# calmiLovesAI/ComputerVision.pytorch

Hardware: AMD Instinct MI355X
Metric: images/sec 640x640 YOLOv8-n train step (higher is better)
Workload: dtype f16; 1 GPU; YOLOv8-n train step (fwd + v8 loss + bwd + Adam), batch 32/GPU, 640x640, nc=80, random init; global_batch=32, parallelism=dp1, launch=eager, exchange=none (1 rank), gpu_max_hw_queues=4

## Files before the change

__graft_entry__.py:

```python
import os
import subprocess
import sys

ROOT = os.path.dirname(os.path.abspath(__file__))
CSRC = os.path.join(ROOT, "computervision.pytorch_amd", "csrc")
LIBDIR = os.path.join(ROOT, "computervision.pytorch_amd", "lib")
LIB = os.path.join(LIBDIR, "libcvx_engine.so")
SOURCES = ["conv_igemm.hip", "conv_igemm_dma.hip", "conv_halo.hip", "conv_tile.hip", "conv_tile_k1.hip", "conv_tile_k2.hip", "conv_gemm.hip", "conv_stem7.hip", "conv_pw.hip", "conv_wgrad.hip", "conv_wgrad_gemm.hip", "conv_wgrad_halo.hip", "conv_wgrad_stream.hip", "conv_wgrad_k3.hip", "bn_act.hip", "stem.hip", "unit_ops.hip", "misc_ops.hip", "loss_v8.hip", "loss_seg.hip", "loss_centernet.hip", "loss_multibox.hip", "loss_yolov7.hip", "preprocess.hip", "augment.hip", "seg_pipeline.hip", "det_eval.hip", "coco_eval.hip", "nms.hip", "centernet_decode.hip", "render.hip", "tiles.hip", "seg_tiles.hip", "seg_tta.hip", "det_tta.hip", "track.hip", "optim.hip", "comm.hip", "engine.hip"]


def _stale(out, deps):
    if not os.path.exists(out):
        return True
    t = os.path.getmtime(out)
    return any(os.path.getmtime(d) > t for d in deps)


def build(force: bool = False) -> None:
    os.makedirs(LIBDIR, exist_ok=True)
    objdir = os.path.join(ROOT, "build", "obj")
    os.makedirs(objdir, exist_ok=True)
    headers = [os.path.join(CSRC, f) for f in os.listdir(CSRC) if f.endswith(".h")] + [os.path.join(ROOT, "include", "cvx_engine.h")]
    hipcc = os.environ.get("HIPCC", "/opt/rocm/bin/hipcc")
    objs, procs = [], []
    for src in SOURCES:
        s = os.path.join(CSRC, src)
        o = os.path.join(objdir, src.replace(".hip", ".o"))
        objs.append(o)
        if force or _stale(o, [s] + headers):
            cmd = [hipcc, "--offload-arch=gfx950", "-O3", "-std=c++17", "-fPIC", "-c", s, "-o", o]
            procs.append((src, subprocess.Popen(cmd, stdout=subprocess.PIPE, stderr=subprocess.STDOUT, text=True)))
    for src, p in procs:
        out, _ = p.communicate()
        if p.returncode != 0:
            raise RuntimeError(f"hipcc failed on {src}:\n{out}")
    if force or procs or _stale(LIB, objs):
        cmd = [hipcc, "--offload-arch=gfx950", "-shared", "-fPIC", "-o", LIB] + objs
        r = subprocess.run(cmd, stdout=subprocess.PIPE, stderr=subprocess.STDOUT, text=True)
        if r.returncode != 0:
            raise RuntimeError("link failed:\n" + r.stdout)
    if ROOT not in sys.path:
        sys.path.insert(0, ROOT)
    import computervision.pytorch_amd as pkg
    pkg._lib.load()


def smoke() -> None:
    if ROOT not in sys.path:
        sys.path.insert(0, ROOT)
    import numpy as np
    import torch
    from computervision.pytorch_amd.model import Yolo8
    from computervision.pytorch_amd.train import FlatAdam, FusedTrainStep, V8DetectionLoss
    from computervision.pytorch_amd import engine as E
    from configs import Yolo8DetConfig
    from oracle import nms_ref, synth
    from oracle import yolov8_ref as O

    assert torch.cuda.is_available(), "smoke() needs the MI355X"
    dev = torch.device("cuda:0")
    cfg = Yolo8DetConfig()
    torch.manual_seed(0)
    model = Yolo8("n", 80).to(dev).train()
    crit = V8DetectionLoss(cfg, model)
    step = FusedTrainStep(model, crit, FlatAdam(model, lr=1e-3))
    x, batch = synth.images(2, 128, 128, seed=1), synth.targets(2, seed=2)
    items = step(x.to(dev), batch).cpu()
    sd = O.init_state_dict("n", 80, seed=0)
    loss_ref, items_ref, _, _ = O.train_step(sd, x, batch, {})
    rel = float((items - items_ref).abs().max() / items_ref.abs().max())
    assert rel < 3e-2, f"loss items differ from the oracle: {items} vs {items_ref}"
    w = model.state_dict()["model.22.cv3.0.2.bias"].cpu()
    assert torch.allclose(w, sd["model.22.cv3.0.2.bias"], atol=2e-3), "post-Adam bias differs from the oracle"
    pred = synth.nms_pred(7, b=1)
    rows, index, counts = E.nms(torch.from_numpy(pred).to(dev), 0.25, 0.7, 300)
    ref_rows, ref_keep = nms_ref.non_max_suppression(pred, 0.25, 0.7, 300)[0]
    k = int(counts[0])
    assert k == len(ref_keep) and np.array_equal(index[0, :k].cpu().numpy().astype(np.int64), ref_keep), "NMS indices differ"
    print(f"smoke ok: loss items {items.tolist()} (oracle {items_ref.tolist()}), nms kept {k}")


if __name__ == "__main__":
    build(force="--force" in sys.argv)
    print("built", LIB)
    if "--smoke" in sys.argv:
        smoke()
```

computervision.pytorch_amd/_lib.py:

```python
from __future__ import annotations

import ctypes as C
import os

import numpy as np

_HERE = os.path.dirname(os.path.abspath(__file__))
LIB_PATH = os.environ.get("CVX_LIB") or os.path.join(_HERE, "lib", "libcvx_engine.so")
ABI_VERSION = 5
SEG_OPTS_KEY_OFFSET = 4096


class CvxError(RuntimeError):
    pass


class BufDesc(C.Structure):
    _fields_ = [("h", C.c_int32), ("w", C.c_int32), ("c", C.c_int32), ("kind", C.c_int32)]


class View(C.Structure):
    _fields_ = [("buf", C.c_int32), ("coff", C.c_int32), ("c", C.c_int32), ("pix_off", C.c_int32)]


class OpDesc(C.Structure):
    _fields_ = [
        ("type", C.c_int32),
        ("in_", View), ("out", View), ("res", View),
        ("ih", C.c_int32), ("iw", C.c_int32), ("oh", C.c_int32), ("ow", C.c_int32),
        ("k", C.c_int32), ("stride", C.c_int32), ("pad", C.c_int32), ("dil", C.c_int32),
        ("act", C.c_int32), ("needs_dgrad", C.c_int32), ("w_cin", C.c_int32),
        ("w_off", C.c_int64), ("gamma_off", C.c_int64), ("beta_off", C.c_int64), ("bias_off", C.c_int64),
        ("rmean_off", C.c_int64), ("rvar_off", C.c_int64),
        ("lane", C.c_int32), ("flags", C.c_int32),
    ]


class SegDims(C.Structure):
    _fields_ = [(k, C.c_int32) for k in ("ld", "batch", "nc", "ih", "iw", "oh", "ow")]


class SegCriterion(C.Structure):
    _fields_ = [("base", C.c_int32), ("focal_alpha", C.c_float), ("focal_gamma", C.c_float), ("class_weight", C.c_void_p),
                ("label_smoothing", C.c_float), ("ignore_index", C.c_int64), ("ohem_theta", C.c_float), ("ohem_min_kept", C.c_int64),
                ("region", C.c_int32), ("base_weight", C.c_double), ("weight", C.c_double), ("alpha", C.c_double), ("beta", C.c_double),
                ("gamma", C.c_double), ("smooth", C.c_double), ("per_image", C.c_int32), ("skip_absent", C.c_int32),
                ("region_class_weight", C.c_void_p)]


BUF_ACT_F16, BUF_PRED_F32 = 0, 1
OP_CONV, OP_MAXPOOL5, OP_UPSAMPLE2, OP_MAXPOOL2, OP_DWCONVT, OP_COPY, OP_MAXPOOL3S2, OP_AVGPOOL, OP_RESIZE, OP_MAXPOOL3S1, OP_L2NORM = 1, 2, 3, 4, 5, 6, 7, 8, 9, 10, 11
OP_DROPOUT = 12
ACT_BN_SILU, ACT_BIAS, ACT_BN_RELU, ACT_BN_LINEAR, ACT_BIAS_RELU, ACT_BIAS_LINEAR = 1, 2, 3, 4, 5, 6
OPF_RES_PRE_ACT = 1
OPF_CONV_BIAS = 2
OPF_RAW_F16 = 4

_P, _I32, _I64, _F, _U64 = C.c_void_p, C.c_int32, C.c_int64, C.c_float, C.c_uint64

EXPERIMENTAL_PROTOTYPES = {
    "cvx_chain_pair_unit": (_I32, [_P, _I32, _I32, _I32, _I32, _P, _P, _P, _P, _P, _P, _I32, _P, _I32, _I32, _I32, C.POINTER(_F), _P]),
    "cvx_chain_conv_unit": (_I32, [_P, _I32, _I32, _I32, _I32, _P, _I32, _I32, _I32, _I32, _P, _P, _I32, _P, _I32, _I32, _I32, C.POINTER(_F), _P]),
    "cvx_chain_detect_unit": (_I32, [_P, _I32, _I32, _I32, _I32, _I32, _I32, _I32, _P, _P, _P, _P, _P, _P, _P, _P, _P, _P, _P, _I32, _I32, _I32,
                                     _I32, _I32, C.POINTER(_F), _P]),
    "cvx_wgrad_time_unit": (_I32, [_P, _P, _I32, _I32, _I32, _I32, _I32, _I32, _I32, _I32, _I32, _I32, _P, _I64, C.POINTER(_F), C.POINTER(_I32), _P]),
}

PROTOTYPES = {
    "cvx_last_error": (C.c_char_p, []),
    "cvx_abi_version": (_I32, []),
    "cvx_engine_create": (_I32, [C.POINTER(_P), C.POINTER(BufDesc), _I32, C.POINTER(OpDesc), _I32, _I32, _I32, _I32, _P]),
    "cvx_engine_destroy": (_I32, [_P]),
    "cvx_engine_bind": (_I32, [_P, _P, _P, _I64, _P, _I64]),
    "cvx_engine_set_bn": (_I32, [_P, _F, _F]),
    "cvx_engine_forward": (_I32, [_P, _P, _I32, _I32, _P]),
    "cvx_engine_backward": (_I32, [_P, _P, _F]),
    "cvx_engine_backward_begin": (_I32, [_P, _P, _F]),
    "cvx_engine_backward_range": (_I32, [_P, _I32, _I32]),
    "cvx_engine_grads_ready": (_I32, [_P, _I32, _I32, _P]),
    "cvx_engine_backward_end": (_I32, [_P]),
    "cvx_engine_workspace_bytes": (_I64, [_P]),
    "cvx_engine_plan_generation": (_I64, [_P]),
    "cvx_engine_debug_copy": (_I32, [_P, _I32, _I32, _P, _I64]),
    "cvx_engine_profile": (_I32, [_P, _I32]),
    "cvx_engine_profile_read": (_I32, [_P, _I32, C.POINTER(C.c_double), C.POINTER(C.c_double), C.POINTER(C.c_double),
                                       C.POINTER(_I64)]),
    "cvx_debug_clock_buffer": (_I32, [_P]),
    "cvx_debug_conv_tile_plan": (_I32, [_I32, _I32, _I32, _I32, _I32, _P]),
    "cvx_debug_conv_dma_plan": (_I32, [_I64, _I32, _I32, _I32, _P]),
    "cvx_debug_conv_halo_plan": (_I32, [_I32, _I32, _I32, _I32, _I32, _P]),
    "cvx_debug_conv_pw_plan": (_I32, [_I64, _I32, _I32, _P]),
    "cvx_debug_conv_grid_div": (_I32, [_I32]),
    "cvx_engine_profile_dump": (_I32, [_P, C.c_char_p]),
    "cvx_pred_level_to_nchw": (_I32, [_P, _I32, _I32, _I32, _I32, _I32, _I32, _P, _P]),
    "cvx_nchw_grad_to_dpred": (_I32, [_P, _I32, _I32, _I32, _I32, _I32, _I32, _F, _P, _P]),
    "cvx_loss_v8_workspace_bytes": (_I64, [_I32, _I32, _I32, _I32]),
    "cvx_loss_v8": (_I32, [_P, _I32, _I32, _I32, _P, _I32, _I32, C.POINTER(_I32), C.POINTER(_F), _I32, _F, _F, _F, _F, _P, _P, _P,
                           _I64, _P]),
    "cvx_loss_v8_strided": (_I32, [_P, _I32, _I32, _I32, _I32, _P, _I32, _I32, C.POINTER(_I32), C.POINTER(_F), _I32, _F, _F, _F, _F, _P, _P, _P,
                                   _I64, _P]),
    "cvx_loss_v8_assignment": (_I32, [_P, _I32, _I32, _I32, _P, _P, _P]),
    "cvx_pack_targets": (_I32, [_P, _P, _P, _I32, _P, _P]),
    "cvx_decode_strided": (_I32, [_P, _I32, _I32, _I32, _I32, C.POINTER(_I32), C.POINTER(_F), _I32, _P, _P]),
    "cvx_adam_step": (_I32, [_P, _P, _P, _P, _I64, _F, _F, _F, _F, _I32, _P, _I32, _P]),
    "cvx_check_finite": (_I32, [_P, _I64, _P, _P]),
    "cvx_adam_step_dev": (_I32, [_P, _P, _P, _P, _I64, _F, _F, _F, _P, _P, _I32, _F, _P]),
    "cvx_ema_update": (_I32, [_P, _P, _I64, _F, _F, _P]),
    "cvx_adam_ema_step_dev": (_I32, [_P, _P, _P, _P, _I64, _F, _F, _F, _P, _P, _I32, _F, _P, _F, _F, _P]),
    "cvx_optim_step": (_I32, [_I32, _P, _P, _P, _P, _I64, _P, _P, _I32, _P, _F, _F, _F, _P, _I32, _F, _P, _P, _F, _F, _P]),
    "cvx_grad_norm_workspace": (_I64, [_I64]),
    "cvx_grad_norm": (_I32, [_P, _I64, _P, _P, _I32, _F, _F, _P, _P, _P, _I64, _P]),
    "cvx_engine_set_stream": (_I32, [_P, _P]),
    "cvx_engine_exchange_stream": (_P, [_P]),
    "cvx_decode": (_I32, [_P, _I32, _I32, _I32, C.POINTER(_I32), C.POINTER(_F), _I32, _P, _P]),
    "cvx_yolo7_decode": (_I32, [_P, _I32, _I32, _I32, _P, _P, _I32, _I32, _I32, _P, _P, _P]),
    "cvx_ssd_decode": (_I32, [_P, _P, _P, _I32, _I32, _I32, _F, _F, _P, _P, _P]),
    "cvx_ssd_decode_max": (_I32, [_P, _P, _P, _I32, _I32, _I32, _F, _F, _P, _P, _P, _P]),
    "cvx_pred_cols_to_nchw": (_I32, [_P, _I32, _I32, _I32, _I32, _I32, _I32, _I32, _P, _I64, _I64, _P]),
    "cvx_nms_workspace_bytes": (_I64, [_I32, _I32]),
    "cvx_nms": (_I32, [_P, _I32, _I32, _I32, _F, _F, _I32, _P, _P, _P, _P, _I64, _P]),
    "cvx_nms_variant": (_I32, [_P, _I32, _I32, _I32, _F, _F, _I32, _I32, _P, _P, _P, _P, _I64, _P]),
    "cvx_centernet_decode_workspace_bytes": (_I64, [_I32, _I32, _I32, _I32]),
    "cvx_centernet_decode": (_I32, [_P, _I32, _I32, _I32, _I32, _I32, _I32, _I32, _I32, _F, _F, _I32, _P, _P, _P, _P, _P, _P, _P, _I64, _P]),
    "cvx_conv2d_nhwc": (_I32, [_P, _I32, _I32, _I32, _I32, _P, _I32, _I32, _I32, _I32, _I32, _I32, _P, _P, _P, _P]),
    "cvx_conv2d_dgrad_nhwc": (_I32, [_P, _I32, _I32, _I32, _I32, _P, _I32, _I32, _I32, _I32, _I32, _P, _P]),
    "cvx_conv2d_wgrad_workspace_bytes": (_I64, [_I32, _I32, _I32, _I32, _I32, _I32]),
    "cvx_conv2d_wgrad_nhwc": (_I32, [_P, _P, _I32, _I32, _I32, _I32, _I32, _I32, _I32, _I32, _I32, _P, _P, _I64, _P]),
    "cvx_bn_silu_train_nhwc": (_I32, [_P, _I32, _I32, _I32, _P, _P, _F, _F, _P, _P, _P, _P, _P, _P, _P, _P]),
    "cvx_bn_silu_bwd_nhwc": (_I32, [_P, _P, _I32, _I32, _I32, _P, _P, _P, _F, _P, _P, _P, _P, _I32, _P]),
    "cvx_letterbox_geometry": (_I32, [_I32, _I32, _I32, _I32, _P, _P, _P, _P, _P]),
    "cvx_letterbox_u8_to_nchw": (_I32, [_P, _I32, _I32, _I32, _I32, _P, _I32, _I32, _P]),
    "cvx_letterbox_batch_u8_to_nchw": (_I32, [_P, _I32, _I32, _I32, _P, _I32, _I32, _P]),
    "cvx_det_to_image": (_I32, [_P, _P, _I32, _I32, _I32, _P, _P, _P, _P, _P]),
    "cvx_draw_detections": (_I32, [_P, _I32, _I32, _I32, _P, _P, _I32, _P, _I32, _I32, _I32, _P]),
    "cvx_seg_overlay": (_I32, [_P, _I32, _I32, _I32, _P, _I32, _I32, _I32, _I32, _I32, _I32, _P, _I32, _P]),
    "cvx_tiles_u8_to_nchw": (_I32, [_P, _I32, _I32, _P, _I32, _I32, _P]),
    "cvx_det_merge_workspace_bytes": (_I64, [_I32]),
    "cvx_det_merge_tiles": (_I32, [_P, _P, _I32, _I32, _P, _P, _I32, _I32, _F, _I32, _I32, _P, _P, _P, _P, _P, _I64, _P]),
    "cvx_track_state_bytes": (_I64, [_I32]),
    "cvx_track_update": (_I32, [_P, _P, _I32, _I32, _P, _I32, _P, _P, _P, _P, _P]),
    "cvx_draw_tracks": (_I32, [_P, _I32, _I32, _I32, _P, _P, _I32, _P, _P, _I32, _I32, _I32, _P]),
    "cvx_seg_stitch": (_I32, [_P, _I32, _I32, _I32, _I32, _I32, _I32, _I32, _P, _P, _I32, _P, _I32, _I32, _I32, _P, _P, _P, _P, _I32, _I32, _I32, _P]),
    "cvx_seg_tta_inputs": (_I32, [_P, _I32, _I32, _I32, _I32, _I32, _I32, _I32, _P, _P]),
    "cvx_seg_fuse": (_I32, [_P, _I32, _I32, _I32, _I32, _I32, _I32, _I32, _P, _P, _P, _P, _P]),
    "cvx_det_tta_inputs": (_I32, [_P, _I32, _I32, _I32, _P, _I32, _F, _P, _P]),
    "cvx_det_fuse_views": (_I32, [_P, _P, _I32, _P, _P, _I32, _I32, _F, _I32, _I32, _I32, _I32, _P, _P, _P, _P, _P, _P, _I64, _P]),
    "cvx_aug_images": (_I32, [_P, _P, _P, _I32, _P, _I32, _I32, _P]),
    "cvx_aug_boxes": (_I32, [_P, _P, _I32, _P, _I32, _I32, _I32, _P, _P, _P]),
    "cvx_aug_images_plain": (_I32, [_P, _P, _I32, _P, _I32, _I32, _P]),
    "cvx_aug_boxes_padded": (_I32, [_P, _P, _P, _I32, _P, _I32, _I32, _I32, _I32, _P, _P, _P, _P]),
    "cvx_aug_warp_mix": (_I32, [_P, _P, _I32, _P, _I32, _I32, _P]),
    "cvx_aug_boxes_warp": (_I32, [_P, _P, _I32, _P, _I32, _I32, _I32, _F, _F, _F, _I32, _P, _I32, _P, _P, _P]),
    "cvx_engine_set_seed": (_I32, [_P, _U64]),
    "cvx_engine_keep_shadows": (_I32, [_P]),
    "cvx_engine_set_fusion": (_I32, [_P, _I32]),
    "cvx_engine_fused_groups": (_I32, [_P]),
    "cvx_centernet_loss_workspace_bytes": (_I64, [_I32, _I32]),
    "cvx_centernet_loss": (_I32, [_P, _I32, _I32, _I32, _I32, _I32, _I32, _P, _P, _P, _P, _P, _I32, _F, _F, _F, _F, _P, _P, _P, _P, _P]),
    "cvx_yolo7_loss_workspace_bytes": (_I64, [_I32, _I32, _I32, _I32]),
    "cvx_yolo7_loss": (_I32, [_P, _I32, _I32, _I32, _P, _P, _P, _P, _I32, _F, _F, _F, _F, _F, _F, _P, _P, _P, _P, _P]),
    "cvx_debug_yolo7_loss_layout": (_I32, [_I32, _I32, _I32, _I32, _P]),
    "cvx_centernet_draw_targets": (_I32, [_P, _P, _I32, _I32, _I32, _I32, _I32, _P, _P, _P, _P, _P, _P]),
    "cvx_ssd_encode_targets": (_I32, [_P, _P, _I32, _I32, _P, _I32, _I32, _F, _F, _F, _P, _P, _P]),
    "cvx_multibox_loss_workspace_bytes": (_I64, [_I32, _I32]),
    "cvx_multibox_loss": (_I32, [_P, _P, _P, _I32, _I32, _I32, _F, _F, _F, _P, _P, _P, _P, _P]),
    "cvx_seg_criterion_workspace_bytes": (_I64, [C.POINTER(SegDims), C.POINTER(SegCriterion), _I32]),
    "cvx_seg_criterion_loss": (_I32, [_P, C.POINTER(SegDims), _P, C.POINTER(SegCriterion), _F, _P, _P, _P, _P, _P, _P, _P]),
    "cvx_seg_criterion_eval": (_I32, [_P, C.POINTER(SegDims), _P, C.POINTER(SegCriterion), _P, _P, _P, _P, _P]),
    "cvx_det_match": (_I32, [_P, _P, _I32, _I32, _I32, _P, _P, _P, _I32, _I32, C.c_double, _I32, _P, _P, _P, _I64, _P, _P, _P]),
    "cvx_det_ap": (_I32, [_P, _P, _P, _P, _I32, C.c_double, _I32, _P, _P, _P, _P]),
    "cvx_coco_match": (_I32, [_P, _P, _I32, _I32, _I32, _P, _I32, _I32, _P, _P, _I32, _I32, _P, _P, _P, _P, _P, _P, _I64, _P, _P, _P]),
    "cvx_coco_accumulate": (_I32, [_P, _P, _P, _P, _P, _I32, _P, _P, _P, _P]),
    "cvx_coco_summarize": (_I32, [_P, _P, _I32, _P, _P]),
    "cvx_seg_pipeline": (_I32, [_P, _I32, _P, _I32, _I32, C.POINTER(_F), C.POINTER(_F), _P, _P, _I32, _I32, _P]),
    "cvx_seg_pipeline_aug": (_I32, [_P, _I32, _P, _I32, _I32, _I32, _I32, C.POINTER(_F), C.POINTER(_F), C.POINTER(_F), _P, _P, _I32, _I32, _P]),
    "cvx_resize_bilinear_nchw_grad_to_rows": (_I32, [_P, _I32, _I32, _I32, _I32, _I32, _I32, _F, _P, _I32, _P]),
    "cvx_maxpool3_train_nhwc": (_I32, [_P, _I32, _I32, _I32, _I32, _I32, _P, _P, _P]),
    "cvx_maxpool3_bwd_nhwc": (_I32, [_P, _P, _I32, _I32, _I32, _I32, _I32, _P, _I32, _P]),
    "cvx_l2norm_bwd_nhwc": (_I32, [_P, _P, _P, _I32, _I32, _I32, _F, _P, _P, _I32, _P]),
    "cvx_nchw_cols_grad_to_pred": (_I32, [_P, _I64, _I64, _I32, _I32, _I32, _I32, _I32, _F, _P, _I32, _I32, _P]),
    "cvx_dwconvt_nhwc": (_I32, [_P, _I32, _I32, _I32, _I32, _I32, _P, _P, _P]),
    "cvx_dwconvt_bwd_nhwc": (_I32, [_P, _P, _I32, _I32, _I32, _I32, _I32, _P, _P, _I32, _P, _F, _P]),
    "cvx_maxpool2_bwd_nhwc": (_I32, [_P, _P, _I32, _I32, _I32, _I32, _I32, _P, _I32, _P]),
    "cvx_avgpool_global_bwd_nhwc": (_I32, [_P, _I32, _I32, _I32, _P, _I32, _P]),
    "cvx_resize_bilinear_bwd_nhwc": (_I32, [_P, _I32, _I32, _I32, _I32, _I32, _I32, _P, _I32, _P]),
    "cvx_dropout_nhwc": (_I32, [_P, _I32, _I32, _I32, _F, _U64, _P, _I32, _P]),
    "cvx_bn_act_train_nhwc": (_I32, [_P, _I32, _I32, _I32, _P, _P, _F, _F, _P, _P, _P, _I32, _I32, _P, _P, _P, _P, _P]),
    "cvx_bn_act_bwd_nhwc": (_I32, [_P, _P, _P, _I32, _I32, _I32, _P, _P, _P, _I32, _I32, _F, _P, _P, _P, _P, _I32, _P]),
    "cvx_maxpool5_nhwc": (_I32, [_P, _I32, _I32, _I32, _I32, _P, _P, _P]),
    "cvx_maxpool5_bwd_nhwc": (_I32, [_P, _P, _I32, _I32, _I32, _I32, _P, _I32, _P]),
    "cvx_resize_bilinear_rows_to_nchw": (_I32, [_P, _I32, _I32, _I32, _I32, _I32, _I32, _I32, _P, _P]),
    "cvx_maxpool_nhwc": (_I32, [_P, _I32, _I32, _I32, _I32, _I32, _I32, _I32, _P, _P]),
    "cvx_avgpool_global_nhwc": (_I32, [_P, _I32, _I32, _I32, _P, _P]),
    "cvx_resize_bilinear_nhwc": (_I32, [_P, _I32, _I32, _I32, _I32, _I32, _I32, _P, _P]),
    "cvx_l2norm_nhwc": (_I32, [_P, _P, _I32, _I32, _I32, _P, _P]),
    "cvx_upsample2_nhwc": (_I32, [_P, _I32, _I32, _I32, _I32, _P, _P]),
    "cvx_upsample2_bwd_nhwc": (_I32, [_P, _I32, _I32, _I32, _I32, _P, _I32, _P]),
    "cvx_stem_train_nchw": (_I32, [_P, _I32, _I32, _I32, _P, _I32, _P, _P, _F, _F, _P, _P, _P, _P, _P, _P, _P]),
    "cvx_stem_eval_nchw": (_I32, [_P, _I32, _I32, _I32, _P, _I32, _P, _P, _P, _P]),
    "cvx_stem_wgrad_nchw": (_I32, [_P, _I32, _I32, _I32, _P, _I32, _P, _P]),
    "cvx_comm_unique_id": (_I32, [_P]),
    "cvx_comm_create": (_I32, [C.POINTER(_P), _P, _I32, _I32, _I32]),
    "cvx_comm_destroy": (_I32, [_P]),
    "cvx_allreduce_f32": (_I32, [_P, _I64, _P, _P]),
    "cvx_allreduce_grads": (_I32, [_P, _P, _P]),
    "cvx_engine_backward_exchange": (_I32, [_P, _P, _F, _P, _P, _I32, _P]),
    "cvx_stem_backward_nchw": (_I32, [_P, _I32, _I32, _I32, _P, _P, _I32, _P, _P, _P, _F, _P, _P, _P, _P]),
    "cvx_stem_backward_recompute_nchw": (_I32, [_P, _I32, _I32, _I32, _P, _P, _I32, _P, _P, _P, _P, _F, _P, _P, _P, _P]),
# ... 49 lines not shown
```

computervision.pytorch_amd/csrc/conv_igemm.h:

```cpp
#pragma once
#include "cvx_common.h"
#include "bn_act.h"
#include "conv_plan.h"

enum {
  CVX_EPI_RAW_STATS = 0,
  CVX_EPI_AFFINE_SILU = 1,
  CVX_EPI_BIAS_F32 = 2,
  CVX_EPI_PLAIN = 3,
};

#define CVX_MAX_TAPS 64

struct ConvParams {
  const half_t* in;
  long long in_bstride;
  int in_ld;
  int IH, IW;
  int Cin;
  const half_t* wt;
  int wt_ld;
  int Cout;
  int B, OH2, OW2;
  int IS;
  int OS, oph, opw;
  int OWr;
  int ntaps;
  const ConvTap* taps;
  int epi;
  int accumulate;
  half_t* out16;
  float* out32;
  long long out_bstride;
  int out_ld;
  const half_t* res;
  long long res_bstride;
  int res_ld;
  const float* scale;
  int act_kind;
  int res_pre;
  const float* shift;
  const float* bias;
  long long* stats;
  int stats_replicas;
  const half_t* zeros;
  int dbg;
  unsigned long long* clk;
  int halo_taps_ok;
  int nphase;
  struct Phase {
    const ConvTap* taps;
    int ntaps, OH2, OW2, oph, opw;
  } phase[4];
  int pointwise;
  unsigned long long halo_pos, halo_wt;
  const half_t* wt_packed;
  int wt_packed_bn, wt_packed_kc;
  int std7x7;
  int std3x3;
  int gemm_variant;
  const half_t* tile_packed;
  int tile_packed_bn;
  int no_tile;
  int ps_cin;
  int raw16;
};

__device__ __forceinline__ void cvx_store_raw4(const ConvParams& p, long long off, const f4& v) {
  if (p.raw16) *reinterpret_cast<h4*>(p.out16 + off) = h4{(half_t)v[0], (half_t)v[1], (half_t)v[2], (half_t)v[3]};
  else *reinterpret_cast<f4*>(p.out32 + off) = v;
}

extern unsigned long long* g_cvx_clk;
extern int g_cvx_grid_div;
int cvx_conv_igemm_launch(const ConvParams& p, hipStream_t stream);
int cvx_conv_igemm_dma_launch(const ConvParams& p, hipStream_t stream);
bool cvx_conv_halo_supported(const ConvParams& p);
int cvx_conv_halo_launch(const ConvParams& p, hipStream_t stream);
bool cvx_conv_stem7_supported(const ConvParams& p);
int cvx_conv_stem7_launch(const ConvParams& p, hipStream_t stream);
struct GemmPackJob {
  const half_t* src;
  half_t* dst;
  const ConvTap* taps;
  int src_ld, rows, Cin, ntaps, BN, kc, nblocks, chunks;
  int blk0, nblk;
};
bool cvx_conv_gemm_plan(const ConvParams& p, GemmPackJob* job, size_t* bytes);
int cvx_conv_gemm_pack_jobs(const GemmPackJob* d_jobs, int njobs, int nblocks, hipStream_t stream);
bool cvx_conv_gemm_shape_ok(const ConvParams& p);
bool cvx_conv_gemm_supported(const ConvParams& p);
int cvx_conv_gemm_launch(const ConvParams& p, hipStream_t stream);
void cvx_conv_gemm_release();
struct TilePackPlan {
  int BN, NB, SPT;
  size_t bytes;
  double cost_us;
};
bool cvx_conv_tile_shape_ok(const ConvParams& p);
bool cvx_conv_tile_supported(const ConvParams& p);
bool cvx_conv_tile_plan(const ConvParams& p, TilePackPlan* out);
int cvx_conv_tile_fill_job(const ConvParams& p, const TilePackPlan& tp, half_t* dst, int blk0, void* job_out);
size_t cvx_conv_tile_job_bytes();
int cvx_conv_tile_pack_jobs(const void* d_jobs, int njobs, int nblocks, hipStream_t stream);
int cvx_conv_tile_launch(const ConvParams& p, hipStream_t stream);
void cvx_conv_tile_release();
bool cvx_conv_pw_supported(const ConvParams& p);
int cvx_conv_pw_launch(const ConvParams& p, hipStream_t stream);

struct WgradParams {
  const half_t* x;
  long long x_bstride;
  int x_ld;
  int IH, IW, Cin;
  const half_t* dy;
  long long dy_bstride;
  int dy_ld;
  int Cout;
  int B, OH, OW;
  int stride;
  int ntaps;
  const ConvTap* taps;
  float* slabs;
  int nsplit;
  int cin_pad16;
  int std3x3;
};
int cvx_conv_wgrad_launch(const WgradParams& p, hipStream_t stream);
void cvx_conv_wgrad_tile(int cout, int jtot, int* co_b, int* j_b);
bool cvx_conv_wgrad_gemm_supported(const WgradParams& p);
void cvx_conv_wgrad_gemm_tile(int cout, int jtot, int* co_b, int* j_b);
int cvx_conv_wgrad_gemm_launch(const WgradParams& p, hipStream_t stream);
bool cvx_conv_wgrad_halo_supported(const WgradParams& p);
void cvx_conv_wgrad_halo_grid(int cout, int cin, int* gx, int* gy);
int cvx_conv_wgrad_halo_tiles(int B, int OH, int OW);
int cvx_conv_wgrad_halo_launch(const WgradParams& p, hipStream_t stream);
bool cvx_conv_wgrad_stream_supported(const WgradParams& p);
int cvx_conv_wgrad_stream_nsplit(const WgradParams& p);
int cvx_conv_wgrad_stream_launch(const WgradParams& p, hipStream_t stream);
bool cvx_conv_wgrad_k3_supported(const WgradParams& p);
int cvx_conv_wgrad_k3_nsplit(const WgradParams& p, bool wide = false);
int cvx_conv_wgrad_k3_launch(const WgradParams& p, hipStream_t stream);
```

computervision.pytorch_amd/csrc/conv_igemm.hip:

```cpp
#include "conv_igemm.h"

unsigned long long* g_cvx_clk = nullptr;
int g_cvx_grid_div = 1;

extern "C" int cvx_debug_conv_grid_div(int32_t div) {
  CVX_CHECK(div >= 1, "the grid divisor is at least 1");
  const int prev = g_cvx_grid_div;
  g_cvx_grid_div = div;
  return prev;
}

int cvx_conv_igemm_launch(const ConvParams& p_in, hipStream_t stream) {
  ConvParams p = p_in;
  p.clk = g_cvx_clk;
  CVX_CHECK(p.Cin % 8 == 0 && p.in_ld % 8 == 0 && p.wt_ld % 8 == 0, "conv: channel counts must be multiples of 8");
  CVX_CHECK(p.Cout % 4 == 0 && p.out_ld % 4 == 0, "conv: Cout/out_ld must be multiples of 4");
  CVX_CHECK(p.ntaps >= 1 && p.ntaps <= CVX_MAX_TAPS, "conv: bad tap count");
  CVX_CHECK(((uintptr_t)p.in % 16) == 0 && ((uintptr_t)p.wt % 16) == 0, "conv: operands must be 16-byte aligned");
  CVX_CHECK(p.zeros && ((uintptr_t)p.zeros % 16) == 0, "conv: needs a 16-byte aligned zero page (padding source of the LDS DMA)");
  CVX_CHECK((long long)p.B * p.OH2 * p.OW2 > 0, "conv: empty output");
  if (p.ps_cin > 0) {
    CVX_CHECK(p.epi == CVX_EPI_PLAIN && p.nphase <= 1 && p.OS == 2 && p.oph == 0 && p.opw == 0 && p.ps_cin % 8 == 0 && p.Cout == 4 * p.ps_cin &&
                  cvx_conv_gemm_shape_ok(p),
              "conv: pixel-shuffle data gradient needs the GEMM-shaped kernel (plain epilogue, 4 phases of ps_cin channels, output stride 2)");
    return cvx_conv_gemm_launch(p, stream);
  }
  if (p.nphase > 1) return cvx_conv_igemm_dma_launch(p, stream);
  if (cvx_conv_stem7_supported(p)) return cvx_conv_stem7_launch(p, stream);
  if (cvx_conv_tile_supported(p)) return cvx_conv_tile_launch(p, stream);
  if (cvx_conv_gemm_supported(p)) return cvx_conv_gemm_launch(p, stream);
  if (cvx_conv_pw_supported(p)) return cvx_conv_pw_launch(p, stream);
  if (cvx_conv_halo_supported(p)) return cvx_conv_halo_launch(p, stream);
  return cvx_conv_igemm_dma_launch(p, stream);
}
```

computervision.pytorch_amd/csrc/conv_tile.h:

```cpp
#pragma once
#include "conv_tile_common.h"

namespace cvx_tile_k {
using namespace cvx_tile;

typedef __attribute__((address_space(3))) void* lds_ptr_t;

constexpr int kTileWaves = 8;

struct TileArgs {
  int TR, tiles_per_img, ntiles, NB;
  int P, pow2, logP, sh, swmask, phmask;
  int SPT, NSTEPS, KSC, NCH, R;
  int CP, PW;
  int PP, PPW;
  int units, Wp;
  unsigned magic_wp, magic_w, magic_p;
  int wring_off, CB, stat_off;
  unsigned in_records;
  const half_t* wpk;
  int dbg;
};

template <int OFF>
__device__ __forceinline__ h8 lds_frag(unsigned a) {
  h8 v;
  asm volatile("ds_read_b128 %0, %1 offset:%2" : "=v"(v) : "v"(a), "n"(OFF));
  return v;
}
template <int NTW>
__device__ __forceinline__ void frag_load_w(h8 (&w)[NTW], unsigned a) {
  if constexpr (NTW >= 1) w[0] = lds_frag<0>(a);
  if constexpr (NTW >= 2) w[1] = lds_frag<1024>(a);
  if constexpr (NTW >= 3) w[2] = lds_frag<2048>(a);
  if constexpr (NTW >= 4) w[3] = lds_frag<3072>(a);
  if constexpr (NTW >= 5) w[4] = lds_frag<4096>(a);
  if constexpr (NTW >= 6) w[5] = lds_frag<5120>(a);
  if constexpr (NTW >= 7) w[6] = lds_frag<6144>(a);
  if constexpr (NTW >= 8) w[7] = lds_frag<7168>(a);
  if constexpr (NTW >= 9) w[8] = lds_frag<8192>(a);
}

__device__ __forceinline__ void wait_vmcnt_dyn(int n) {
#define CVX_WV(N) else if (n == N) wait_vmcnt<N>();
  if (n <= 0 || n > 20) wait_vmcnt<0>();
  CVX_WV(1) CVX_WV(2) CVX_WV(3) CVX_WV(4) CVX_WV(5) CVX_WV(6) CVX_WV(7) CVX_WV(8) CVX_WV(9) CVX_WV(10)
  CVX_WV(11) CVX_WV(12) CVX_WV(13) CVX_WV(14) CVX_WV(15) CVX_WV(16) CVX_WV(17) CVX_WV(18) CVX_WV(19) CVX_WV(20)
#undef CVX_WV
}

}

int cvx_conv_tile_launch_k1(int MT, int NTW, const ConvParams& p, const cvx_tile_k::TileArgs& a, int lds, hipStream_t st);
int cvx_conv_tile_launch_k2(int MT, int NTW, const ConvParams& p, const cvx_tile_k::TileArgs& a, int lds, hipStream_t st);
```

computervision.pytorch_amd/csrc/conv_tile.hip:

```cpp
#include <algorithm>
#include <cstring>
#include <map>
#include <mutex>
#include <vector>

#include "conv_tile.h"

namespace {
using namespace cvx_tile_k;

struct TilePackJob {
  const half_t* src;
  half_t* dst;
  unsigned long long wt_pack;
  int src_ld, rows, Cin, BN, NB, SPT;
  int blk0, nblk;
};
constexpr int TPACK_UNITS = 256 * 8;
__device__ __forceinline__ void tile_pack_units(const TilePackJob& a, long long u0, long long u1) {
  const int nsteps = 9 * a.SPT;
  for (long long u = u0 + threadIdx.x; u < u1; u += blockDim.x) {
    const int sp = (int)(u & 3);
    const long long r0 = u >> 2;
    const int r = (int)(r0 % a.BN);
    const long long r1 = r0 / a.BN;
    const int n = (int)(r1 % nsteps);
    const int nb = (int)(r1 / nsteps);
    const int g = sp ^ ((r >> 1) & 3);
    const int tap = n / a.SPT, s = n - tap * a.SPT;
    const int k = s * 32 + g * 8;
    const int row = nb * a.BN + r;
    h8 v = {0, 0, 0, 0, 0, 0, 0, 0};
    if (row < a.rows && k < a.Cin) v = *reinterpret_cast<const h8*>(a.src + (long long)row * a.src_ld + (int)((a.wt_pack >> (4 * tap)) & 15) * a.Cin + k);
    *reinterpret_cast<h8*>(a.dst + u * 8) = v;
  }
}
__global__ __launch_bounds__(256) void tile_pack_kernel(const TilePackJob a) {
  const long long total = (long long)a.NB * 9 * a.SPT * a.BN * 4;
  const long long u0 = (long long)blockIdx.x * TPACK_UNITS;
  if (u0 < total) tile_pack_units(a, u0, u0 + TPACK_UNITS < total ? u0 + TPACK_UNITS : total);
}
__global__ __launch_bounds__(256) void tile_pack_jobs_kernel(const TilePackJob* jobs, int njobs) {
  int lo = 0, hi = njobs - 1;
  while (lo < hi) {
    const int mid = (lo + hi + 1) >> 1;
    if (jobs[mid].blk0 <= (int)blockIdx.x)
      lo = mid;
    else
      hi = mid - 1;
  }
  const TilePackJob a = jobs[lo];
  const long long total = (long long)a.NB * 9 * a.SPT * a.BN * 4;
  const long long u0 = (long long)((int)blockIdx.x - a.blk0) * TPACK_UNITS;
  if (u0 < total) tile_pack_units(a, u0, u0 + TPACK_UNITS < total ? u0 + TPACK_UNITS : total);
}

constexpr int kMaxMT = 4;
const int kNtwMenu[] = {1, 2, 3, 4, 5, 6, 9};

unsigned magic_of(int d) { return (unsigned)((0x100000000ULL + (unsigned long long)d - 1) / (unsigned long long)d); }

struct Plan {
  int MT, NTW, TR, NB, KSC, NCH, R, SPT, lds, ntiles, tpi, PP, units, CB, wring_off, stat_off;
  double cost;
};

bool plan_tile(const ConvParams& p, Plan* best) {
  const int H = p.IH, W = p.IW, Cin = p.Cin;
  const int P = Cin / 8, SPT = (Cin + 31) / 32, NSTEPS = 9 * SPT;
  const int ctiles = (p.Cout + 15) / 16;
  static const int force_tr = cvx_tune_int("CVX_TILE_TR", 0), force_ntw = cvx_tune_int("CVX_TILE_NTW", 0);
  bool found = false;
  for (int NTW : kNtwMenu) {
    if (force_ntw && NTW != force_ntw) continue;
    if (NTW > ctiles && NTW != kNtwMenu[0]) {
      bool smaller_fits = false;
      for (int q : kNtwMenu) smaller_fits |= q >= ctiles && q < NTW;
      if (smaller_fits) continue;
    }
    const int NB = (ctiles + NTW - 1) / NTW;
    if ((NB - 1) * NTW >= ctiles) continue;
    for (int TR = 1; TR <= H; ++TR) {
      if (force_tr && TR != force_tr) continue;
      const int G = (TR * W + 15) / 16;
      const int MT = (G + kTileWaves - 1) / kTileWaves;
      if (MT > kMaxMT) break;
      if (MT > 4 || MT * NTW * 4 + 3 * (MT + NTW) * 4 > 216) continue;
      const int tpi = (H + TR - 1) / TR;
      const int units = (TR + 2) * (W + 2) * P;
      const int PP = (units + 63) / 64;
      const int patch_bytes = PP * 1024;
      const int stat_bytes = kTileWaves * 16 * NTW * 2 * 4;
      const int budget = 160 * 1024 - patch_bytes - stat_bytes;
      int KSC = 0, R = 0;
      if (NSTEPS * NTW * 1024 <= budget && (NSTEPS * NTW + kTileWaves - 1) / kTileWaves + (PP + kTileWaves - 1) / kTileWaves <= 60) {
        KSC = NSTEPS;
        R = 2;
      } else {
        for (int k = SPT; k >= 1 && !KSC; --k) {
          if (SPT % k) continue;
          const int r = budget / (k * NTW * 1024);
          if (r >= 3 && (k * NTW + kTileWaves - 1) / kTileWaves <= 20) {
            KSC = k;
            R = r > 4 ? 4 : r;
          }
        }
      }
      if (!KSC) continue;
      const int CB = KSC * NTW * 1024;
      const int nslots = R > NSTEPS / KSC ? NSTEPS / KSC : R;
      const int stage_bytes = kTileWaves * MT * 16 * (16 * NTW * 4 + 16);
      const int lds = std::max(patch_bytes + nslots * CB + stat_bytes, stage_bytes);
      if (lds > 160 * 1024) continue;
      const long long wgs = (long long)tpi * p.B * NB;
      const double rounds = (double)((wgs + 255) / 256);
      const double mfma_cyc = (double)NSTEPS * MT * NTW * 16.0 * (kTileWaves / 4);
      const double lds_cyc = (double)NSTEPS * kTileWaves * (MT + NTW) * 6.0;
      const double valu_cyc = (double)NSTEPS * (MT * 3 + NTW * 4 + 8) * 4.0;
      const double loop_us = std::max(std::max(mfma_cyc * 1.15, lds_cyc), valu_cyc + mfma_cyc * 0.5) / 1900.0;
      const double wbytes = (double)NSTEPS * NTW * 1024.0;
      const double load_us = (patch_bytes + CB) / 60e3 + std::max(0.0, (wbytes - CB) / 60e3 - loop_us);
      const double epi_us = 0.6 + MT * NTW * 0.02;
      const double t = rounds * (1.2 + load_us + loop_us + epi_us) + 1.0;
      if (!found || t < best->cost) {
        found = true;
        *best = Plan{MT, NTW, TR, NB, KSC, NSTEPS / KSC, R, SPT, lds, tpi * p.B, tpi, PP, units, CB, patch_bytes, patch_bytes + nslots * CB, t};
      }
    }
  }
  return found;
}

struct PackSlot {
  half_t* buf = nullptr;
  size_t bytes = 0;
};
std::mutex g_pack_mu;
std::map<std::pair<const void*, unsigned long long>, PackSlot> g_pack;

}

bool cvx_conv_tile_shape_ok(const ConvParams& p) {
  if (!p.zeros || !p.halo_taps_ok || p.ntaps != 9) return false;
  if (p.IS != 1 || p.OS != 1 || p.oph != 0 || p.opw != 0) return false;
  if (p.OH2 != p.IH || p.OW2 != p.IW || p.OWr != p.IW) return false;
  if (p.Cin % 8 != 0 || p.Cin < 32 || p.Cin > 512 || p.in_ld % 8 != 0) return false;
  if (p.Cout % 8 != 0 || p.out_ld % 8 != 0 || (p.res && p.res_ld % 8 != 0)) return false;
  if (p.IW > 4000 || p.IH > 4000 || p.IW < 2) return false;
  const long long extent = ((long long)(p.B - 1) * p.in_bstride + ((long long)p.IH * p.IW - 1) * p.in_ld + p.Cin) * 2;
  if (extent >= (1LL << 32) - 65536) return false;
  Plan pl;
  return plan_tile(p, &pl);
}

bool cvx_conv_tile_supported(const ConvParams& p) {
  static const bool off = cvx_tune_set("CVX_NO_TILE");
  if (off || p.no_tile) return false;
  static const int max_w = cvx_tune_int("CVX_TILE_MAXW", 40), max_c = cvx_tune_int("CVX_TILE_MAXC", 144);
  if (p.IW > max_w || p.IH > max_w || p.Cin > max_c) return false;
  return cvx_conv_tile_shape_ok(p);
}

bool cvx_conv_tile_plan(const ConvParams& p, TilePackPlan* out) {
  if (!cvx_conv_tile_shape_ok(p)) return false;
  Plan pl;
  if (!plan_tile(p, &pl)) return false;
  out->BN = 16 * pl.NTW;
  out->NB = pl.NB;
  out->SPT = pl.SPT;
  out->bytes = (size_t)pl.NB * 9 * pl.SPT * pl.NTW * 1024;
  out->cost_us = pl.cost;
  return true;
}

int cvx_conv_tile_pack_jobs(const void* d_jobs, int njobs, int nblocks, hipStream_t stream) {
  if (njobs <= 0 || nblocks <= 0) return 0;
  hipLaunchKernelGGL(tile_pack_jobs_kernel, dim3(nblocks), dim3(256), 0, stream, (const TilePackJob*)d_jobs, njobs);
  CVX_HIP(hipGetLastError());
  return 0;
}

int cvx_conv_tile_fill_job(const ConvParams& p, const TilePackPlan& tp, half_t* dst, int blk0, void* job_out) {
  TilePackJob j;
  memset(&j, 0, sizeof(j));
  j.src = p.wt;
  j.dst = dst;
  j.wt_pack = p.halo_wt;
  j.src_ld = p.wt_ld;
  j.rows = p.Cout;
  j.Cin = p.Cin;
  j.BN = tp.BN;
  j.NB = tp.NB;
  j.SPT = tp.SPT;
  j.blk0 = blk0;
  const long long units = (long long)tp.NB * 9 * tp.SPT * tp.BN * 4;
  j.nblk = (int)((units + TPACK_UNITS - 1) / TPACK_UNITS);
  memcpy(job_out, &j, sizeof(j));
  return j.nblk;
}
size_t cvx_conv_tile_job_bytes() { return sizeof(TilePackJob); }

int cvx_conv_tile_launch(const ConvParams& p, hipStream_t stream) {
  Plan pl;
  CVX_CHECK(plan_tile(p, &pl), "conv_tile: no tiling for this shape");
  const half_t* packed = (p.tile_packed && p.tile_packed_bn == 16 * pl.NTW) ? p.tile_packed : nullptr;
  if (!packed) {
    TilePackPlan tp{16 * pl.NTW, pl.NB, pl.SPT, (size_t)pl.NB * 9 * pl.SPT * pl.NTW * 1024, 0.0};
    half_t* buf = nullptr;
    {
      std::lock_guard<std::mutex> lk(g_pack_mu);
      PackSlot& ps = g_pack[{p.wt, p.halo_wt ^ ((unsigned long long)tp.BN << 52)}];
      if (ps.bytes < tp.bytes) {
        hipStreamCaptureStatus cs = hipStreamCaptureStatusNone;
        (void)hipStreamIsCapturing(stream, &cs);
        CVX_CHECK(cs == hipStreamCaptureStatusNone, "conv_tile: the packed-weight buffer cannot be allocated while the stream is capturing");
        if (ps.buf) CVX_HIP(hipFree(ps.buf));
        CVX_HIP(hipMalloc((void**)&ps.buf, tp.bytes));
        ps.bytes = tp.bytes;
      }
      buf = ps.buf;
    }
    TilePackJob j;
    const int nblk = cvx_conv_tile_fill_job(p, tp, buf, 0, &j);
    hipLaunchKernelGGL(tile_pack_kernel, dim3(nblk), dim3(256), 0, stream, j);
    packed = buf;
  }
  TileArgs a;
  memset(&a, 0, sizeof(a));
  a.TR = pl.TR;
  a.tiles_per_img = pl.tpi;
  a.ntiles = pl.ntiles;
  a.NB = pl.NB;
  a.P = p.Cin / 8;
  a.pow2 = (a.P & (a.P - 1)) == 0 ? 1 : 0;
  a.logP = 0;
  while ((1 << a.logP) < a.P) ++a.logP;
  a.sh = a.P == 4 ? 2 : (a.P == 8 ? 1 : 0);
  a.swmask = a.pow2 ? (a.P >= 16 ? 15 : a.P - 1) : 0;
  a.phmask = a.pow2 ? a.P - 1 : -1;
  a.SPT = pl.SPT;
  a.NSTEPS = 9 * pl.SPT;
  a.KSC = pl.KSC;
  a.NCH = pl.NCH;
  a.R = pl.R;
  a.CP = pl.KSC * pl.NTW;
  a.PW = (a.CP + kTileWaves - 1) / kTileWaves;
  a.PP = pl.PP;
  a.PPW = (pl.PP + kTileWaves - 1) / kTileWaves;
  a.units = pl.units;
  a.Wp = p.IW + 2;
  a.magic_wp = magic_of(a.Wp);
  a.magic_w = magic_of(p.IW);
  a.magic_p = magic_of(a.P);
  a.wring_off = pl.wring_off;
  a.CB = pl.CB;
  a.stat_off = pl.stat_off;
  a.in_records = (unsigned)(((long long)(p.B - 1) * p.in_bstride + ((long long)p.IH * p.IW - 1) * p.in_ld + p.Cin) * 2);
  a.wpk = packed;
  static const int dbg = cvx_tune_int("CVX_TILE_DBG", 0);
  a.dbg = dbg;
  int rc;
  if (pl.MT <= 2)
    rc = cvx_conv_tile_launch_k1(pl.MT, pl.NTW, p, a, pl.lds, stream);
  else
    rc = cvx_conv_tile_launch_k2(pl.MT, pl.NTW, p, a, pl.lds, stream);
  CVX_TRY(rc);
  CVX_HIP(hipGetLastError());
  return 0;
}

extern "C" int cvx_debug_conv_tile_plan(int32_t batch, int32_t h, int32_t w, int32_t cin, int32_t cout, int32_t* out8) {
  CVX_CHECK(out8 && batch > 0 && h > 0 && w > 0, "bad arguments");
  ConvParams p;
  memset(&p, 0, sizeof(p));
  static half_t dummy_zero[8];
  p.zeros = dummy_zero;
  p.halo_taps_ok = 1;
  p.ntaps = 9;
  p.IS = p.OS = 1;
  p.B = batch;
  p.IH = p.OH2 = h;
  p.IW = p.OW2 = p.OWr = w;
  p.Cin = p.in_ld = cin;
  p.in_bstride = (long long)h * w * cin;
  p.Cout = cout;
  if (!cvx_conv_tile_shape_ok(p)) return -1;
  Plan pl;
  if (!plan_tile(p, &pl)) return -1;
  out8[0] = pl.TR;
  out8[1] = pl.MT;
  out8[2] = pl.NTW;
  out8[3] = pl.NB;
  out8[4] = pl.ntiles * pl.NB;
  out8[5] = pl.KSC;
  out8[6] = pl.lds;
  out8[7] = (int)(pl.cost * 100.0);
  return 0;
}

void cvx_conv_tile_release() {
  std::lock_guard<std::mutex> lk(g_pack_mu);
  for (auto& kv : g_pack)
    if (kv.second.buf) (void)hipFree(kv.second.buf);
  g_pack.clear();
}
```

computervision.pytorch_amd/csrc/conv_tile_kernel.inc.h:

```cpp
#include "conv_tile.h"

namespace {
using namespace cvx_tile_k;

template <int MT, int NTW>
__global__ __launch_bounds__(64 * kTileWaves) void conv_tile_kernel(const ConvParams p, const TileArgs a) {
#if defined(__HIP_DEVICE_COMPILE__)
  constexpr int BN = 16 * NTW;
  extern __shared__ __attribute__((aligned(16))) unsigned char smem[];
  const int tid = threadIdx.x;
  const int wave = __builtin_amdgcn_readfirstlane(tid >> 6), lane = tid & 63;
  const int fr = lane & 15, fq = lane >> 4;
  const int xcd = blockIdx.x & 7, seq = blockIdx.x >> 3;
  const int nblk = seq % a.NB;
  const int tile = (seq / a.NB) * 8 + xcd;
  if (tile >= a.ntiles) return;
  clk_mark(p, 0);
  const int b = tile / a.tiles_per_img;
  const int y0 = (tile - b * a.tiles_per_img) * a.TR;
  const int H = p.IH, W = p.IW, Wp = a.Wp, P = a.P;

  const __amdgpu_buffer_rsrc_t rsrc_in = __builtin_amdgcn_make_buffer_rsrc(const_cast<half_t*>(p.in), (short)0, (int)a.in_records, 0x00020000);
  const half_t* wblk = a.wpk + (long long)nblk * a.NSTEPS * (BN * 32);
  const __amdgpu_buffer_rsrc_t rsrc_w = __builtin_amdgcn_make_buffer_rsrc(const_cast<half_t*>(wblk), (short)0, a.NSTEPS * BN * 64, 0x00020000);

  {
    const unsigned img_off = (unsigned)((long long)b * p.in_bstride * 2);
    for (int k = 0; k < a.PPW; ++k) {
      int piece = k * kTileWaves + wave;
      piece = piece < a.PP ? piece : a.PP - 1;
      const unsigned u = (unsigned)(piece * 64 + lane);
      const unsigned q = __umulhi(u, a.magic_p);
      const unsigned phys = u - q * (unsigned)P;
      const unsigned pr = __umulhi(q, a.magic_wp);
      const unsigned pc = q - pr * (unsigned)Wp;
      const unsigned c = phys ^ ((pc >> a.sh) & (unsigned)a.swmask);
      const int y = y0 - 1 + (int)pr, x = (int)pc - 1;
      const bool ok = u < (unsigned)a.units && (unsigned)y < (unsigned)H && (unsigned)x < (unsigned)W;
      const unsigned vo = ok ? img_off + (unsigned)(((y * W + x) * p.in_ld + (int)c * 8) * 2) : 0xffffffffu;
      __builtin_amdgcn_raw_ptr_buffer_load_lds(rsrc_in, (lds_ptr_t)(smem + piece * 1024), 16, vo, 0, 0, 0);
    }
  }
  const unsigned vb = (unsigned)(lane * 16);
  auto issue_chunk = [&](int c, int slot) __attribute__((always_inline)) {
    unsigned char* sb = smem + a.wring_off + slot * a.CB;
    const int base = c * a.CB;
    for (int k = 0; k < a.PW; ++k) {
      int piece = k * kTileWaves + wave;
      piece = piece < a.CP ? piece : a.CP - 1;
      __builtin_amdgcn_raw_ptr_buffer_load_lds(rsrc_w, (lds_ptr_t)(sb + piece * 1024), 16, vb, base + piece * 1024, 0, 0);
    }
  };
  const int npre = a.NCH < a.R - 1 ? a.NCH : a.R - 1;
  for (int c = 0; c < npre; ++c) issue_chunk(c, c);
  clk_mark(p, 1);

  const int rows_here = H - y0 < a.TR ? H - y0 : a.TR;
  const int npix = rows_here * W;
  unsigned S0[MT], S1[MT], S2[MT];
  bool pvalid[MT];
  const unsigned rowpitch = (unsigned)(Wp * P * 16);
#pragma unroll
  for (int i = 0; i < MT; ++i) {
    const int m = (wave * MT + i) * 16 + fr;
    pvalid[i] = m < npix;
    const unsigned mm = pvalid[i] ? (unsigned)m : 0u;
    const unsigned pr = __umulhi(mm, a.magic_w);
    const unsigned pc = mm - pr * (unsigned)W;
    auto s_of = [&](unsigned col) -> unsigned {
      const unsigned sw = (col >> a.sh) & (unsigned)a.swmask;
      const unsigned ph = ((unsigned)fq ^ sw) & (unsigned)a.phmask;
      return (pr + 1u) * rowpitch + ((col * (unsigned)P + ph) << 4);
    };
    S0[i] = s_of(pc);
    S1[i] = s_of(pc + 1u);
    S2[i] = s_of(pc + 2u);
  }

  f4 acc[MT][NTW];
#pragma unroll
  for (int i = 0; i < MT; ++i)
#pragma unroll
    for (int j = 0; j < NTW; ++j) acc[i][j] = f4{0.f, 0.f, 0.f, 0.f};

  const unsigned long long pos_pack = p.halo_pos;
  const unsigned xk_mask = a.pow2 ? 0xffffffffu : 0u, np2_mask = ~xk_mask;
  auto step_xk = [&](int s) -> unsigned { return (unsigned)(s << 6) & xk_mask; };
  auto step_ak = [&](int dh, int s) -> unsigned {
    int c = 4 * s + fq;
    c = c < P ? c : P - 1;
    return (unsigned)(dh * (int)rowpitch) + ((unsigned)((c - fq) << 4) & np2_mask);
  };

#pragma unroll
  for (int i = 0; i < MT; ++i) asm volatile("" ::"v"(S0[i]), "v"(S1[i]), "v"(S2[i]));
#pragma unroll
  for (int i = 0; i < MT; ++i)
#pragma unroll
    for (int j = 0; j < NTW; ++j) asm volatile("" ::"v"(acc[i][j]));
  if (npre <= 1 || (a.dbg & 1)) wait_vmcnt<0>();
  else wait_vmcnt_dyn((npre - 1) * a.PW);
  workgroup_barrier();
  clk_mark(p, 2);
#ifdef CVX_TUNING
  if ((a.dbg & 8) && p.clk) {
    wait_vmcnt<0>();
    workgroup_barrier();
    if (blockIdx.x == 0)
      for (int o = tid * 4; o < a.stat_off; o += 1024) reinterpret_cast<unsigned*>(p.clk)[o >> 2] = *reinterpret_cast<const unsigned*>(smem + o);
    return;
  }
#endif

  h8 xs[3][MT], ws[3][NTW];
  unsigned SC[MT];
  const unsigned lds0 = (unsigned)(unsigned long long)(const __attribute__((address_space(3))) void*)smem;
  const int NSTEPS = a.NSTEPS, SPT = a.SPT, KSC = a.KSC, NCH = a.NCH, CB = a.CB, R = a.R, PWc = a.PW;
  const unsigned wfrag0 = lds0 + (unsigned)a.wring_off + (unsigned)(lds_row_off(fr, fq) * 2);
  int c_tap = 0, c_st = 0, c_inc = 0, c_chunk = 0, c_slot = 0, c_n = 0;
  int dh_cur;
  unsigned xk_c, ak_c, w_c;
  auto set_tap = [&](int t) __attribute__((always_inline)) -> int {
    const int code = (int)(pos_pack >> (4 * t)) & 15;
    const int dwi = code & 3;
    const unsigned m0 = dwi == 0 ? 0xffffffffu : 0u, m1 = dwi == 1 ? 0xffffffffu : 0u, m2 = dwi == 2 ? 0xffffffffu : 0u;
#pragma unroll
    for (int i = 0; i < MT; ++i) SC[i] = (S0[i] & m0) | (S1[i] & m1) | (S2[i] & m2);
    return (code >> 2) - 1;
  };
  dh_cur = set_tap(0);
  xk_c = step_xk(0);
  ak_c = step_ak(dh_cur, 0) + lds0;
  w_c = wfrag0;
  auto advance = [&]() __attribute__((always_inline)) {
    if (c_n + 1 < NSTEPS) {
      ++c_n;
      if (++c_st == SPT) {
        c_st = 0;
        ++c_tap;
        dh_cur = set_tap(c_tap);
      }
      xk_c = step_xk(c_st);
      ak_c = step_ak(dh_cur, c_st) + lds0;
      if (++c_inc == KSC) {
        c_inc = 0;
        const int issued = NCH < c_chunk + R - 1 ? NCH : c_chunk + R - 1;
        if (issued - c_chunk - 2 <= 0) wait_vmcnt<0>();
        else wait_vmcnt_dyn((issued - c_chunk - 2) * PWc);
        workgroup_barrier();
        if (c_chunk + R - 1 < NCH) issue_chunk(c_chunk + R - 1, c_slot == 0 ? R - 1 : c_slot - 1);
        ++c_chunk;
        c_slot = c_slot == R - 1 ? 0 : c_slot + 1;
      }
      w_c = wfrag0 + (unsigned)(c_slot * CB + c_inc * (NTW * 1024));
    }
  };
  frag_load_w<NTW>(ws[0], w_c);
#pragma unroll
  for (int i = 0; i < MT; ++i) xs[0][i] = lds_frag<0>((SC[i] ^ xk_c) + ak_c);
  advance();
  frag_load_w<NTW>(ws[1], w_c);
#pragma unroll
  for (int i = 0; i < MT; ++i) xs[1][i] = lds_frag<0>((SC[i] ^ xk_c) + ak_c);
  asm volatile("s_waitcnt lgkmcnt(0)" ::: "memory");
  constexpr int LW = (MT + NTW) > 15 ? 15 : (MT + NTW);
#if defined(CVX_TILE_ABL)
#define CVX_TILE_DBG_BIT(b) (((CVX_TILE_ABL) & (b)) != 0)
#else
#define CVX_TILE_DBG_BIT(b) false
#endif
#define CVX_TILE_BODY(K, LAST)                                                                                          \
  {                                                                                                                     \
    advance();                                                                                                          \
    if (!CVX_TILE_DBG_BIT(128)) frag_load_w<NTW>(ws[((K) + 2) % 3], w_c);                                                \
    _Pragma("unroll") for (int i = 0; i < MT; ++i) {                                                                    \
      __builtin_amdgcn_sched_barrier(0);                                                                                \
      _Pragma("unroll") for (int j = 0; j < NTW; ++j)                                                                   \
          acc[i][j] = __builtin_amdgcn_mfma_f32_16x16x32_f16(ws[K][j], xs[K][i], acc[i][j], 0, 0, 0);                   \
      if (!CVX_TILE_DBG_BIT(64)) xs[((K) + 2) % 3][i] = lds_frag<0>((SC[i] ^ xk_c) + ak_c);                              \
    }                                                                                                                   \
    __builtin_amdgcn_sched_barrier(0);                                                                                  \
    if (LAST) {                                                                                                         \
      asm volatile("s_waitcnt lgkmcnt(0)" ::: "memory");                                                                \
    } else {                                                                                                            \
      asm volatile("s_waitcnt lgkmcnt(%0)" ::"n"(LW) : "memory");                                                       \
    }                                                                                                                   \
    __builtin_amdgcn_sched_barrier(0);                                                                                  \
  }
  clk_mark(p, 7);
  for (int n = 0; n < NSTEPS; n += 3) {
    CVX_TILE_BODY(0, false)
    CVX_TILE_BODY(1, false)
    CVX_TILE_BODY(2, true)
  }
#undef CVX_TILE_BODY
  clk_mark(p, 3);

  constexpr int RS = BN * 4 + 16;
  constexpr int CPR = BN / 8;
  constexpr int RPI = 64 / CPR;
  constexpr int ROWS = MT * 16;
  const int epi = p.epi;
  f4 st1[NTW], st2[NTW];
  if (epi == CVX_EPI_RAW_STATS) {
#pragma unroll
    for (int j = 0; j < NTW; ++j) {
      st1[j] = st2[j] = f4{0.f, 0.f, 0.f, 0.f};
#pragma unroll
      for (int i = 0; i < MT; ++i)
        if (pvalid[i]) {
#pragma unroll
          for (int r = 0; r < 4; ++r) {
            st1[j][r] += acc[i][j][r];
            st2[j][r] += acc[i][j][r] * acc[i][j][r];
          }
        }
    }
  }
  if (epi == CVX_EPI_RAW_STATS) {
#pragma unroll
    for (int i = 0; i < MT; ++i) {
      if (!pvalid[i]) continue;
      const unsigned m = (unsigned)((wave * MT + i) * 16 + fr);
      const unsigned pr = __umulhi(m, a.magic_w);
      const unsigned pc = m - pr * (unsigned)W;
      const long long dst = (long long)b * p.out_bstride + ((long long)(y0 + (int)pr) * W + (int)pc) * p.out_ld + nblk * BN + fq * 4;
#pragma unroll
      for (int j = 0; j < NTW; ++j)
        if (nblk * BN + j * 16 + fq * 4 < p.Cout) cvx_store_raw4(p, dst + j * 16, acc[i][j]);
    }
  } else {
  __syncthreads();
    unsigned char* wreg = smem + wave * (ROWS * RS);
#pragma unroll
    for (int i = 0; i < MT; ++i)
#pragma unroll
      for (int j = 0; j < NTW; ++j) *reinterpret_cast<f4*>(wreg + (i * 16 + fr) * RS + (j * 16 + fq * 4) * 4) = acc[i][j];
    {
      const int q = lane % CPR, r0 = lane / CPR;
      const int n = nblk * BN + q * 8;
      const bool lane_on = r0 < RPI && n < p.Cout;
      const int act_kind = p.act_kind, res_pre = p.res_pre, accumulate = p.accumulate;
      const half_t* res = p.res;
      float c0[8], c1[8];
#pragma unroll
      for (int k = 0; k < 8; ++k) {
        c0[k] = 1.f;
        c1[k] = 0.f;
      }
      if (lane_on && epi == CVX_EPI_AFFINE_SILU) {
#pragma unroll
        for (int k = 0; k < 8; ++k) {
          c0[k] = p.scale[n + k];
          c1[k] = p.shift[n + k];
        }
      }
      if (lane_on && epi == CVX_EPI_BIAS_F32) {
#pragma unroll
        for (int k = 0; k < 8; ++k) c1[k] = p.bias[n + k];
      }
      const int m_wave = wave * ROWS;
      for (int r = r0; r < ROWS; r += RPI) {
        const int m = m_wave + r;
        if (!lane_on || m >= npix) continue;
        const unsigned pr = __umulhi((unsigned)m, a.magic_w);
        const unsigned pc = (unsigned)m - pr * (unsigned)W;
        const long long pix = (long long)(y0 + (int)pr) * W + (int)pc;
        const f4 lo = *reinterpret_cast<const f4*>(wreg + r * RS + q * 32);
        const f4 hi = *reinterpret_cast<const f4*>(wreg + r * RS + q * 32 + 16);
        float v[8] = {lo[0], lo[1], lo[2], lo[3], hi[0], hi[1], hi[2], hi[3]};
        if (epi == CVX_EPI_BIAS_F32) {
          float* dst = p.out32 + (long long)b * p.out_bstride + pix * p.out_ld + n;
          *reinterpret_cast<f4*>(dst) = f4{v[0] + c1[0], v[1] + c1[1], v[2] + c1[2], v[3] + c1[3]};
          *reinterpret_cast<f4*>(dst + 4) = f4{v[4] + c1[4], v[5] + c1[5], v[6] + c1[6], v[7] + c1[7]};
          continue;
        }
        half_t* dst = p.out16 + (long long)b * p.out_bstride + pix * p.out_ld + n;
        if (epi == CVX_EPI_AFFINE_SILU) {
          float rv[8] = {0.f, 0.f, 0.f, 0.f, 0.f, 0.f, 0.f, 0.f};
          if (res) {
            const h8 rr = *reinterpret_cast<const h8*>(res + (long long)b * p.res_bstride + pix * p.res_ld + n);
#pragma unroll
            for (int k = 0; k < 8; ++k) rv[k] = (float)rr[k];
          }
#pragma unroll
          for (int k = 0; k < 8; ++k) {
            float t = v[k] * c0[k] + c1[k];
            if (res_pre) t += rv[k];
            if (act_kind == 0) t = cvx_silu(t);
            else if (act_kind == 1) t = fmaxf(t, 0.f);
            if (!res_pre) t += rv[k];
            v[k] = t;
          }
        } else if (accumulate) {
          const h8 old = *reinterpret_cast<const h8*>(dst);
#pragma unroll
          for (int k = 0; k < 8; ++k) v[k] += (float)old[k];
        }
        *reinterpret_cast<h8*>(dst) = h8{(half_t)v[0], (half_t)v[1], (half_t)v[2], (half_t)v[3], (half_t)v[4], (half_t)v[5], (half_t)v[6], (half_t)v[7]};
      }
    }
  }
  if (epi == CVX_EPI_RAW_STATS) {
    __syncthreads();
    float* sStat = reinterpret_cast<float*>(smem);
#pragma unroll
    for (int j = 0; j < NTW; ++j)
#pragma unroll
      for (int r = 0; r < 4; ++r) {
        const float s1 = cvx_wave_sum16(st1[j][r]), s2 = cvx_wave_sum16(st2[j][r]);
        if (fr == 0) {
          sStat[(wave * BN + j * 16 + fq * 4 + r) * 2 + 0] = s1;
          sStat[(wave * BN + j * 16 + fq * 4 + r) * 2 + 1] = s2;
        }
      }
    __syncthreads();
    for (int t = tid; t < BN * 2; t += 64 * kTileWaves) {
      const int ch = t >> 1, which = t & 1, nn = nblk * BN + ch;
      if (nn < p.Cout) {
        float v = 0.f;
#pragma unroll
        for (int w = 0; w < kTileWaves; ++w) v += sStat[(w * BN + ch) * 2 + which];
        cvx_fix_atomic_add(p.stats, ((long long)(blockIdx.x % p.stats_replicas) * p.Cout + nn) * 2 + which, v);
      }
    }
  }
  clk_mark(p, 4);
#endif
}


template <int MT, int NTW>
int launch_tile(const ConvParams& p, const TileArgs& a, int lds, hipStream_t stream) {
  static unsigned long long optin_mask = 0;
  CVX_TRY(cvx_lds_optin((const void*)conv_tile_kernel<MT, NTW>, 160 * 1024, &optin_mask));
  const int blocks = ((a.ntiles + 7) / 8) * 8 * a.NB;
  hipLaunchKernelGGL((conv_tile_kernel<MT, NTW>), dim3(blocks), dim3(64 * kTileWaves), lds, stream, p, a);
  return 0;
}
template <int MT>
int launch_tile_n(int NTW, const ConvParams& p, const TileArgs& a, int lds, hipStream_t st) {
  switch (NTW) {
    case 1: return launch_tile<MT, 1>(p, a, lds, st);
    case 2: return launch_tile<MT, 2>(p, a, lds, st);
    case 3: return launch_tile<MT, 3>(p, a, lds, st);
    case 4: return launch_tile<MT, 4>(p, a, lds, st);
    case 5: return launch_tile<MT, 5>(p, a, lds, st);
    case 6: return launch_tile<MT, 6>(p, a, lds, st);
    default: return launch_tile<MT, 9>(p, a, lds, st);
  }
}
}

int CVX_TILE_LAUNCH_FN(int MT, int NTW, const ConvParams& p, const cvx_tile_k::TileArgs& a, int lds, hipStream_t st) {
  if (MT == CVX_TILE_MT_A) return launch_tile_n<CVX_TILE_MT_A>(NTW, p, a, lds, st);
  return launch_tile_n<CVX_TILE_MT_B>(NTW, p, a, lds, st);
}
```

computervision.pytorch_amd/csrc/engine.hip:

```cpp
#include <algorithm>
#include <atomic>
#include <cstdlib>
#include <cstdio>
#include <cstring>
#include <vector>

#include "../../include/cvx_engine.h"
#ifdef CVX_WITH_CHAIN
#include "conv_chain.h"
#endif
#include "bn_act.h"
#include "conv_igemm.h"
#include <map>
#include <mutex>

#include "misc_ops.h"
#include "stem.h"

static unsigned cvx_event_flags() {
  static const bool sysfence = cvx_tune_set("CVX_EVENT_SYSFENCE");
  return hipEventDisableTiming | (sysfence ? 0u : hipEventDisableSystemFence);
}

static thread_local std::string g_last_error;
void cvx_set_error(const std::string& msg) { g_last_error = msg; }
extern "C" const char* cvx_last_error(void) { return g_last_error.c_str(); }
extern "C" int cvx_abi_version(void) { return CVX_ABI_VERSION; }

namespace {

struct PhaseRt {
  const ConvTap* taps = nullptr;
  TapTraits tr;
  int ntaps = 0, oph = 0, opw = 0, OH2 = 0, OW2 = 0;
};
PhaseRt make_phase(const DgradPhase& d, const ConvTap* dev_taps) {
  PhaseRt r;
  r.taps = dev_taps;
  r.tr = cvx_tap_traits(d.taps);
  r.ntaps = (int)d.taps.size();
  r.oph = d.oph;
  r.opw = d.opw;
  r.OH2 = d.OH2;
  r.OW2 = d.OW2;
  return r;
}

struct DgClass {
  PhaseRt ph;
  const half_t* gemm_pk = nullptr;
  int gemm_bn = 0, gemm_kc = 0;
  const half_t* tile_pk = nullptr;
  int tile_bn = 0;
};

struct ConvRt {
  ConvTap* taps_fwd = nullptr;
  TapTraits tr;
  int ntaps = 0;
  DgClass dg[16];
  int ndg = 0;
  long long sh_fwd = 0, sh_dg = -1;
  int cin_g = 0;
  int cin_pad16 = 0;
  int in_accum = 0, res_accum = 0;
  long long sh_ps = -1;
  PsPackDesc ps_desc;
  ConvTap* ps_taps = nullptr;
  bool ps_on = false;
  const half_t* ps_pk = nullptr;
  int ps_bn = 0, ps_kc = 0;
  int slab_blk0 = 0, slab_blk1 = 0;
  bool raw16 = false;
  bool stem = false;
  half_t* ybuf = nullptr;
  half_t* dybuf = nullptr;
  float *mean = nullptr, *invstd = nullptr, *scale = nullptr, *shift = nullptr;
  long long *stat_fwd = nullptr, *stat_bwd = nullptr;
  hipEvent_t ev_dy = nullptr;
  long long slab_off = 0;
  int nsplit = 1;
  const half_t* gemm_fwd = nullptr;
  int gemm_fwd_bn = 0, gemm_fwd_kc = 0;
  const half_t* tile_fwd = nullptr;
  int tile_fwd_bn = 0;
};

struct PoolRt {
  uint8_t* idx = nullptr;
  int in_accum = 0;
};

struct Buf {
  cvx_buf_desc d;
  half_t* act = nullptr;
  half_t* grad = nullptr;
};

}

struct cvx_engine {
  int device = 0;
  hipStream_t stream = nullptr;
  std::vector<Buf> bufs;
  std::vector<cvx_op_desc> ops;
  std::vector<ConvRt> conv;
  std::vector<PoolRt> pool;
  int image_buf = -1, pred_buf = -1;
  float* params = nullptr;
  float* grads = nullptr;
  float* stats = nullptr;
  int64_t n_params = 0, n_stats = 0;
  float bn_eps = 1e-3f, bn_momentum = 0.03f;
  std::vector<void*> static_allocs;
  half_t* shadow = nullptr;
  long long shadow_elems = 0;
  half_t* zero_page = nullptr;
  PackDesc* d_pack = nullptr;
  BlockRef* d_pack_blocks = nullptr;
  int n_pack_blocks = 0;
  int planned_batch = 0;
  bool planned_train = false;
  std::vector<void*> batch_allocs;
  int64_t batch_bytes = 0, static_bytes = 0;
  long long* stat_region = nullptr;
  long long stat_half = 0;
  hipStream_t side = nullptr;
  hipStream_t red = nullptr;
  hipStream_t lane = nullptr;
  hipEvent_t ev_lane_fork = nullptr, ev_lane_join = nullptr, ev_pack = nullptr;
  bool use_lanes = false;
  hipEvent_t ev_head[3] = {nullptr, nullptr, nullptr};
  int head_producer[3] = {-1, -1, -1};
  int head_join_op[3] = {-1, -1, -1};
  bool head_overlap = false;
  float* ytmp_lane = nullptr;
  hipEvent_t ev_red = nullptr;
  hipEvent_t ev_fork = nullptr, ev_join = nullptr;
  bool image_nhwc = false;
  float* ytmp = nullptr;
  const float* last_images = nullptr;
  bool inference_only = false;
  int64_t plan_generation = 0;
  float* slabs = nullptr;
  SlabDesc* d_slab = nullptr;
  BlockRef* d_slab_blocks = nullptr;
  int n_slab_blocks = 0;
  ColsumDesc* d_colsum = nullptr;
  ColsumBlock* d_colsum_blocks = nullptr;
  int n_colsum = 0, n_colsum_blocks = 0, colsum_max_c = 0;
  BnFoldDesc* d_fold = nullptr;
  int n_fold = 0;
  int slab_tail_blocks = 0;
  int slab_tail_op = -1;
  hipEvent_t ev_mid = nullptr;
  hipEvent_t ev_seg[8] = {nullptr, nullptr, nullptr, nullptr, nullptr, nullptr, nullptr, nullptr};
  int ev_seg_next = 0;
  unsigned long long seed = 0, train_pass = 0;
  bool has_bias_act = false;
  bool fwd_train_done = false;
  bool keep_shadows_once = false;
  int shadows_gen = -1;
  bool shadows_train = false;
  bool bwd_slabs_clean = false;
  int last_batch = 0;
  float* last_pred = nullptr;
  bool profile = false;
  std::vector<hipEvent_t> ev_pool;
// ... 20 lines not shown
  half_t* gemm_arena = nullptr;
  GemmPackJob* d_gemm_jobs = nullptr;
  int n_gemm_jobs = 0, n_gemm_fwd_jobs = 0, gemm_blocks = 0, gemm_fwd_blocks = 0;
  half_t* tile_arena = nullptr;
  void* d_tile_jobs = nullptr;
  int n_tile_jobs = 0, n_tile_fwd_jobs = 0, tile_blocks = 0, tile_fwd_blocks = 0;
  struct cvx_bw_state* bw = nullptr;
  std::vector<ProfRec> prof_recs;
};

void cvx_engine_free_bw(cvx_engine* e);

namespace {

int dev_alloc(cvx_engine* e, std::vector<void*>& pool, int64_t& counter, void** out, long long bytes) {
  if (bytes <= 0) bytes = 16;
  bytes = (bytes + 255) & ~255LL;
  CVX_HIP(hipMalloc(out, (size_t)bytes));
  pool.push_back(*out);
  counter += bytes;
  return 0;
}
template <typename T>
int upload(cvx_engine* e, std::vector<void*>& pool, int64_t& counter, T** out, const std::vector<T>& host) {
  void* p = nullptr;
  CVX_TRY(dev_alloc(e, pool, counter, &p, (long long)(host.size() * sizeof(T))));
  if (!host.empty()) CVX_HIP(hipMemcpy(p, host.data(), host.size() * sizeof(T), hipMemcpyHostToDevice));
  *out = (T*)p;
  return 0;
}
void free_pool(std::vector<void*>& pool) {
  for (void* p : pool) (void)hipFree(p);
  pool.clear();
}

inline int round_up(int x, int m) { return (x + m - 1) / m * m; }

enum { PROF_CONV_FWD = 0, PROF_CONV_DGRAD = 1, PROF_CONV_WGRAD = 2, PROF_BN_FWD = 3, PROF_BN_BWD = 4, PROF_MISC = 5, PROF_SLAB_REDUCE = 6 };

struct ProfScope {
  cvx_engine* e;
  hipStream_t st;
  ProfScope(cvx_engine* eng, int cls, double flops, double bytes, hipStream_t stream = nullptr)
      : e(eng->profile ? eng : nullptr), st(stream ? stream : eng->stream) {
    if (!e) return;
    while (e->ev_pool.size() < e->ev_used + 2) {
      hipEvent_t ev;
      if (hipEventCreate(&ev) != hipSuccess) {
        e = nullptr;
        return;
      }
      e->ev_pool.push_back(ev);
    }
    e->prof_recs.push_back({cls, flops, bytes, e->cur_op});
    slot = e->ev_used;
    e->ev_used += 2;
    (void)hipEventRecord(e->ev_pool[slot], st);
  }
  size_t slot = 0;
  ~ProfScope() {
    if (!e) return;
    (void)hipEventRecord(e->ev_pool[slot + 1], st);
  }
};

double conv_flops(const cvx_op_desc& o, int B) { return 2.0 * B * o.oh * o.ow * o.out.c * (double)(o.k * o.k * o.w_cin); }
double conv_bytes(const cvx_op_desc& o, int B) {
  return 2.0 * B * ((double)o.ih * o.iw * o.w_cin + (double)o.oh * o.ow * o.out.c) + 2.0 * o.out.c * o.k * o.k * o.w_cin;
}

ViewDesc make_view(const cvx_engine* e, const cvx_view& v, bool grad) {
  ViewDesc r{nullptr, 0, 0};
  if (v.buf < 0) return r;
  const Buf& b = e->bufs[v.buf];
  half_t* base = grad ? b.grad : b.act;
  r.ld = b.d.c;
  r.bstride = (long long)b.d.h * b.d.w * b.d.c;
  r.p = base + (long long)v.pix_off * b.d.c + v.coff;
  return r;
}

int act_kind(const cvx_op_desc& o) { return o.act == CVX_ACT_BN_SILU ? 0 : ((o.act == CVX_ACT_BN_LINEAR || o.act == CVX_ACT_BIAS_LINEAR) ? 2 : 1); }
float dropout_p(const cvx_op_desc& o) { return (float)o.k / 65536.f; }
unsigned long long dropout_seed(const cvx_engine* e, int op) {
  return e->seed * 0x9E3779B97F4A7C15ULL + (unsigned long long)e->train_pass * 1000003ULL + (unsigned long long)op;
}

struct ConvGeom {
  int B, ih, iw, cin, oh, ow, cout, stride, ntaps;
};
ConvGeom geom_of(const cvx_op_desc& o, int B) { return ConvGeom{B, o.ih, o.iw, o.in.c, o.oh, o.ow, o.out.c, o.stride, o.k * o.k}; }

void fill_conv_fwd(const ConvGeom& g, ViewDesc in, const half_t* wt, const ConvTap* taps, const TapTraits& tr, const half_t* zeros, ConvParams* cp) {
  memset(cp, 0, sizeof(*cp));
  cp->in = in.p;
  cp->in_bstride = in.bstride;
  cp->in_ld = in.ld;
  cp->IH = g.ih;
  cp->IW = g.iw;
  cp->Cin = g.cin;
  cp->wt = wt;
  cp->wt_ld = g.ntaps * g.cin;
  cp->Cout = g.cout;
  cp->B = g.B;
  cp->OH2 = g.oh;
  cp->OW2 = g.ow;
  cp->IS = g.stride;
  cp->OS = 1;
  cp->OWr = g.ow;
  cp->ntaps = g.ntaps;
  cp->taps = taps;
  cp->zeros = zeros;
  cp->halo_taps_ok = tr.halo_ok ? 1 : 0;
  cp->pointwise = tr.pointwise;
  cp->halo_pos = tr.halo_pos;
  cp->halo_wt = tr.halo_wt;
  cp->std7x7 = tr.std7x7;
  cp->std3x3 = tr.std3x3;
}

void fill_conv_dgrad(const ConvGeom& g, const PhaseRt& ph, ViewDesc dy, ViewDesc gin, const half_t* wt_t, const half_t* zeros, int accumulate, ConvParams* cp) {
  memset(cp, 0, sizeof(*cp));
  cp->in = dy.p;
  cp->in_bstride = dy.bstride;
  cp->in_ld = dy.ld;
  cp->IH = g.oh;
  cp->IW = g.ow;
  cp->Cin = g.cout;
  cp->wt = wt_t;
  cp->wt_ld = g.ntaps * g.cout;
  cp->Cout = g.cin;
  cp->B = g.B;
  cp->OH2 = ph.OH2;
  cp->OW2 = ph.OW2;
  cp->IS = 1;
  cp->OS = g.stride;
  cp->oph = ph.oph;
  cp->opw = ph.opw;
  cp->OWr = g.iw;
  cp->ntaps = ph.ntaps;
  cp->taps = ph.taps;
  cp->zeros = zeros;
  cp->halo_taps_ok = ph.tr.halo_ok ? 1 : 0;
  cp->pointwise = ph.tr.pointwise;
  cp->halo_pos = ph.tr.halo_pos;
  cp->halo_wt = ph.tr.halo_wt;
  cp->epi = CVX_EPI_PLAIN;
  cp->accumulate = accumulate;
  cp->out16 = gin.p;
  cp->out_ld = gin.ld;
  cp->out_bstride = gin.bstride;
}
bool phases_mergeable(const DgClass* dg, int n) {
  if (n < 2 || n > 4) return false;
  for (int q = 0; q < n; ++q)
    if (dg[q].ph.OH2 <= 0 || dg[q].ph.OW2 <= 0 || dg[q].ph.ntaps <= 0) return false;
  return true;
}
void set_merged_phases(const DgClass* dg, int n, ConvParams* cp) {
  cp->nphase = n;
  for (int z = 0; z < n; ++z) cp->phase[z] = ConvParams::Phase{dg[z].ph.taps, dg[z].ph.ntaps, dg[z].ph.OH2, dg[z].ph.OW2, dg[z].ph.oph, dg[z].ph.opw};
  cp->halo_taps_ok = 0;
  cp->pointwise = 0;
}

void fill_conv_ps(const ConvGeom& g, ViewDesc dy, ViewDesc gin, const half_t* ps_wt, const ConvTap* window_taps, const half_t* zeros, int accumulate, ConvParams* cp) {
  memset(cp, 0, sizeof(*cp));
  cp->in = dy.p;
  cp->in_bstride = dy.bstride;
  cp->in_ld = dy.ld;
  cp->IH = g.oh;
  cp->IW = g.ow;
  cp->Cin = g.cout;
  cp->wt = ps_wt;
  cp->wt_ld = 4 * g.cout;
  cp->Cout = 4 * g.cin;
  cp->B = g.B;
  cp->OH2 = g.oh;
  cp->OW2 = g.ow;
  cp->IS = 1;
  cp->OS = 2;
  cp->OWr = g.iw;
  cp->ntaps = 4;
  cp->taps = window_taps;
  cp->zeros = zeros;
  cp->epi = CVX_EPI_PLAIN;
  cp->ps_cin = g.cin;
  cp->accumulate = accumulate;
  cp->out16 = gin.p;
  cp->out_ld = gin.ld;
  cp->out_bstride = gin.bstride;
}

void fill_wgrad(const ConvGeom& g, ViewDesc x, ViewDesc dy, const ConvTap* taps, int std3x3, float* slabs, int nsplit, WgradParams* wp) {
  memset(wp, 0, sizeof(*wp));
  wp->x = x.p;
  wp->x_bstride = x.bstride;
  wp->x_ld = x.ld;
  wp->IH = g.ih;
  wp->IW = g.iw;
  wp->Cin = g.cin;
  wp->dy = dy.p;
  wp->dy_bstride = dy.bstride;
  wp->dy_ld = dy.ld;
  wp->Cout = g.cout;
  wp->B = g.B;
  wp->OH = g.oh;
  wp->OW = g.ow;
  wp->stride = g.stride;
  wp->ntaps = g.ntaps;
  wp->taps = taps;
  wp->slabs = slabs;
  wp->nsplit = nsplit;
  wp->cin_pad16 = round_up(g.cin, 16);
  wp->std3x3 = std3x3;
}

ViewDesc dense_dy(const cvx_op_desc& o, half_t* p = nullptr) { return ViewDesc{p, (long long)o.oh * o.ow * o.out.c, o.out.c}; }
ViewDesc dy_view(const cvx_engine* e, int i, half_t* dpred) {
  const cvx_op_desc& o = e->ops[i];
  if (o.act != CVX_ACT_BIAS) return dense_dy(o, e->conv[i].dybuf);
  const Buf& pb = e->bufs[e->pred_buf];
  return ViewDesc{dpred ? dpred + (long long)o.out.pix_off * pb.d.c + o.out.coff : nullptr, (long long)pb.d.h * pb.d.w * pb.d.c, pb.d.c};
}
void fill_wgrad(const cvx_engine* e, int i, int B, ViewDesc dy, float* slabs, int nsplit, WgradParams* wp) {
  const ConvRt& c = e->conv[i];
  const ViewDesc x = c.stem ? ViewDesc{nullptr, 0, 0} : make_view(e, e->ops[i].in, false);
  fill_wgrad(geom_of(e->ops[i], B), x, dy, c.taps_fwd, c.tr.std3x3, slabs, nsplit, wp);
}

int build_static(cvx_engine* e) {
  const int nops = (int)e->ops.size();
  e->conv.assign(nops, ConvRt());
  e->pool.assign(nops, PoolRt());
  std::vector<PackDesc> packs;
  std::vector<BlockRef> pblocks;
  long long sh = 0;
  for (int i = 0; i < nops; ++i) {
    const cvx_op_desc& o = e->ops[i];
    CVX_CHECK(o.in.buf >= 0 && o.in.buf < (int)e->bufs.size() && o.out.buf >= 0 && o.out.buf < (int)e->bufs.size(), "op view buffer index");
    CVX_CHECK(o.type >= CVX_OP_CONV && o.type <= CVX_OP_DROPOUT, "unknown op type");
    if (o.type == CVX_OP_CONV && (o.act == CVX_ACT_BIAS_RELU || o.act == CVX_ACT_BIAS_LINEAR) && o.res.buf >= 0) e->inference_only = true;
    if (o.type == CVX_OP_CONV && o.res.buf >= 0 && o.act != CVX_ACT_BIAS) {
      const bool pre = (o.flags & CVX_OPF_RES_PRE_ACT) != 0;
      if (o.act == CVX_ACT_BN_RELU && !pre) e->inference_only = true;
    }
    if (o.type == CVX_OP_DROPOUT) CVX_CHECK(o.k >= 0 && o.k < 65536, "dropout: k = drop probability in units of 2^-16");
    if (o.type == CVX_OP_CONV && (o.act == CVX_ACT_BIAS_RELU || o.act == CVX_ACT_BIAS_LINEAR)) e->has_bias_act = true;
    if (o.type != CVX_OP_CONV) {
      CVX_CHECK(o.in.c % 8 == 0 && o.in.coff % 8 == 0 && o.out.coff % 8 == 0 && o.in.c == o.out.c, "pool / resample / copy views: equal, 8-aligned channel slices");
      continue;
    }
    ConvRt& c = e->conv[i];
    const int T = o.k * o.k;
    CVX_CHECK(T <= CVX_MAX_TAPS, "kernel too large");
    if (o.in.buf == e->image_buf) {
      c.stem = o.w_cin == 3 && o.k == 3 && o.stride == 2 && o.pad == 1 && o.dil == 1 && o.act == CVX_ACT_BN_SILU && !o.needs_dgrad &&
               o.res.buf < 0 && o.out.c % 16 == 0 && o.out.c <= 80 && o.ih % 2 == 0 && o.iw % 2 == 0;
      if (!c.stem) {
        CVX_CHECK(o.w_cin == 3 && !o.needs_dgrad, "an op that reads the image needs 3 stored input channels and no data gradient");
        e->image_nhwc = true;
      }
    }
    CVX_CHECK(o.in.c % 8 == 0 && o.out.c % 8 == 0 && o.in.coff % 8 == 0 && o.out.coff % 8 == 0, "conv views must be 8-channel aligned");
    CVX_CHECK(o.w_cin <= o.in.c && o.w_cin > o.in.c - 8, "w_cin vs view channels");
    CVX_CHECK(o.oh == cvx_conv_out_size(o.ih, o.k, o.stride, o.pad, o.dil) && o.ow == cvx_conv_out_size(o.iw, o.k, o.stride, o.pad, o.dil),
              "conv output size does not follow from (ih, iw, k, stride, pad, dil)");
    c.cin_g = o.in.c;
    c.cin_pad16 = round_up(o.in.c, 16);
    c.ntaps = T;
    const std::vector<ConvTap> taps = cvx_conv_fwd_taps(o.k, o.pad, o.dil);
    CVX_TRY(upload(e, e->static_allocs, e->static_bytes, &c.taps_fwd, taps));
    c.tr = cvx_tap_traits(taps);
    PackDesc pd;
// ... 461 lines not shown
  e->n_colsum = e->n_colsum_blocks = e->colsum_max_c = 0;
  if (training) {
    const Buf& pb = e->bufs[e->pred_buf];
    const long long A = (long long)pb.d.h * pb.d.w;
    std::vector<ColsumDesc> cds;
    std::vector<ColsumBlock> cbs;
    for (size_t i = 0; i < e->ops.size(); ++i) {
      const cvx_op_desc& o = e->ops[i];
      if (o.type != CVX_OP_CONV || o.act != CVX_ACT_BIAS) continue;
      ColsumDesc d;
      d.off = (long long)o.out.pix_off * pb.d.c + o.out.coff;
      d.bstride = A * pb.d.c;
      d.ld = pb.d.c;
      d.hw = o.oh * o.ow;
      d.M = (long long)B * d.hw;
      d.C = o.out.c;
      d.rows_per_block = cvx_stream_rows_per_block(d.M, d.C, 32);
      d.part = e->conv[i].stat_bwd;
      d.dbias_off = o.bias_off;
      const int nb = (int)((d.M + d.rows_per_block - 1) / d.rows_per_block);
      for (int b = 0; b < nb; ++b) cbs.push_back(ColsumBlock{(int)cds.size(), b});
      if (d.C > e->colsum_max_c) e->colsum_max_c = d.C;
      cds.push_back(d);
    }
    CVX_TRY(upload(e, e->batch_allocs, e->batch_bytes, &e->d_colsum, cds));
    CVX_TRY(upload(e, e->batch_allocs, e->batch_bytes, &e->d_colsum_blocks, cbs));
    e->n_colsum = (int)cds.size();
    e->n_colsum_blocks = (int)cbs.size();
  }
  if (training) {
    CVX_TRY(dev_alloc(e, e->batch_allocs, e->batch_bytes, &p, slab_total * 4));
    e->slabs = (float*)p;
    CVX_TRY(upload(e, e->batch_allocs, e->batch_bytes, &e->d_slab, sdescs));
    CVX_TRY(upload(e, e->batch_allocs, e->batch_bytes, &e->d_slab_blocks, sblocks));
    e->n_slab_blocks = (int)sblocks.size();
  }
  e->planned_batch = B;
  e->planned_train = training;
  CVX_TRY(plan_fused_groups(e, B));
  CVX_TRY(plan_gemm_packs(e, B, training));
  CVX_TRY(plan_tile_packs(e, B, training));
  return 0;
}

void fill_conv_fwd(const cvx_engine* e, int i, int B, ConvParams* cp) {
  const ConvRt& c = e->conv[i];
  fill_conv_fwd(geom_of(e->ops[i], B), make_view(e, e->ops[i].in, false), e->shadow + c.sh_fwd, c.taps_fwd, c.tr, e->zero_page, cp);
  cp->wt_packed = c.gemm_fwd;
  cp->wt_packed_bn = c.gemm_fwd_bn;
  cp->wt_packed_kc = c.gemm_fwd_kc;
  cp->tile_packed = c.tile_fwd;
  cp->tile_packed_bn = c.tile_fwd_bn;
}

void free_gemm_packs(cvx_engine* e) {
  if (e->gemm_arena) (void)hipFree(e->gemm_arena);
  if (e->d_gemm_jobs) (void)hipFree(e->d_gemm_jobs);
  e->gemm_arena = nullptr;
  e->d_gemm_jobs = nullptr;
  e->n_gemm_jobs = e->n_gemm_fwd_jobs = e->gemm_blocks = e->gemm_fwd_blocks = 0;
  for (auto& c : e->conv) {
    c.gemm_fwd = nullptr;
    c.gemm_fwd_bn = c.gemm_fwd_kc = 0;
    c.ps_on = false;
    c.ps_pk = nullptr;
    c.ps_bn = c.ps_kc = 0;
    for (auto& d : c.dg) {
      d.gemm_pk = nullptr;
      d.gemm_bn = d.gemm_kc = 0;
    }
  }
}

void fill_conv_dgrad(const cvx_engine* e, int i, int q, int B, ViewDesc dy, ConvParams* cp) {
  const ConvRt& c = e->conv[i];
  const DgClass& dc = c.dg[q];
  fill_conv_dgrad(geom_of(e->ops[i], B), dc.ph, dy, make_view(e, e->ops[i].in, true), e->shadow + c.sh_dg, e->zero_page, c.in_accum, cp);
  cp->wt_packed = dc.gemm_pk;
  cp->wt_packed_bn = dc.gemm_bn;
  cp->wt_packed_kc = dc.gemm_kc;
  cp->tile_packed = dc.tile_pk;
  cp->tile_packed_bn = dc.tile_bn;
}
void fill_conv_ps(const cvx_engine* e, int i, int B, ViewDesc dy, ConvParams* cp) {
  const ConvRt& c = e->conv[i];
  fill_conv_ps(geom_of(e->ops[i], B), dy, make_view(e, e->ops[i].in, true), e->shadow + c.sh_ps, c.ps_taps, e->zero_page, c.in_accum, cp);
  cp->wt_packed = c.ps_pk;
  cp->wt_packed_bn = c.ps_bn;
  cp->wt_packed_kc = c.ps_kc;
}

constexpr int kPsRef = 1000;
int plan_gemm_packs(cvx_engine* e, int B, bool training) {
  free_gemm_packs(e);
  struct Ref {
    int op, q;
  };
  std::vector<GemmPackJob> jobs;
  std::vector<Ref> refs;
  std::vector<size_t> offs;
  size_t total = 0;
  int blocks = 0;
  auto add = [&](const ConvParams& cp, int op, int q) {
    GemmPackJob j;
    size_t bytes = 0;
    if (!cvx_conv_gemm_plan(cp, &j, &bytes)) return;
    j.blk0 = blocks;
    blocks += j.nblk;
    offs.push_back(total);
    total += (bytes + 255) / 256 * 256;
    jobs.push_back(j);
    refs.push_back(Ref{op, q});
  };
  for (size_t i = 0; i < e->ops.size(); ++i) {
    if (e->ops[i].type != CVX_OP_CONV || e->conv[i].stem) continue;
    ConvParams cp;
    fill_conv_fwd(e, (int)i, B, &cp);
    add(cp, (int)i, -1);
  }
  const int n_fwd = (int)jobs.size(), fwd_blocks = blocks;
  if (training) {
    for (size_t i = 0; i < e->ops.size(); ++i) {
      const cvx_op_desc& o = e->ops[i];
      const ConvRt& c = e->conv[i];
      if (o.type != CVX_OP_CONV || c.stem || !o.needs_dgrad || c.sh_dg < 0 || c.ndg != 1) continue;
      if (c.dg[0].ph.OH2 <= 0 || c.dg[0].ph.OW2 <= 0 || c.dg[0].ph.ntaps <= 0) continue;
      ConvParams cp;
      fill_conv_dgrad(e, (int)i, 0, B, dense_dy(e->ops[i]), &cp);
      add(cp, (int)i, 0);
    }
    static const bool ps_off = cvx_tune_set("CVX_NO_PS_DGRAD");
    for (size_t i = 0; i < e->ops.size() && !ps_off; ++i) {
      const cvx_op_desc& o = e->ops[i];
      ConvRt& c = e->conv[i];
      if (o.type != CVX_OP_CONV || c.stem || !o.needs_dgrad || c.sh_ps < 0 || c.ndg != 4) continue;
      ConvParams cp;
      fill_conv_ps(e, (int)i, B, dense_dy(e->ops[i]), &cp);
      if (!cvx_conv_gemm_supported(cp)) continue;
      const size_t before = jobs.size();
      add(cp, (int)i, kPsRef);
      c.ps_on = jobs.size() > before;
    }
  }
  if (jobs.empty()) return 0;
  CVX_HIP(hipMalloc((void**)&e->gemm_arena, total));
  for (size_t k = 0; k < jobs.size(); ++k) {
    jobs[k].dst = reinterpret_cast<half_t*>(reinterpret_cast<char*>(e->gemm_arena) + offs[k]);
    ConvRt& c = e->conv[refs[k].op];
    if (refs[k].q < 0) {
      c.gemm_fwd = jobs[k].dst;
      c.gemm_fwd_bn = jobs[k].BN;
      c.gemm_fwd_kc = jobs[k].kc;
    } else if (refs[k].q == kPsRef) {
      c.ps_pk = jobs[k].dst;
      c.ps_bn = jobs[k].BN;
      c.ps_kc = jobs[k].kc;
    } else {
      c.dg[refs[k].q].gemm_pk = jobs[k].dst;
      c.dg[refs[k].q].gemm_bn = jobs[k].BN;
      c.dg[refs[k].q].gemm_kc = jobs[k].kc;
    }
  }
  CVX_HIP(hipMalloc((void**)&e->d_gemm_jobs, jobs.size() * sizeof(GemmPackJob)));
  CVX_HIP(hipMemcpy(e->d_gemm_jobs, jobs.data(), jobs.size() * sizeof(GemmPackJob), hipMemcpyHostToDevice));
  e->n_gemm_jobs = (int)jobs.size();
  e->n_gemm_fwd_jobs = n_fwd;
  e->gemm_blocks = blocks;
  e->gemm_fwd_blocks = fwd_blocks;
  return 0;
}

void free_tile_packs(cvx_engine* e) {
  if (e->tile_arena) (void)hipFree(e->tile_arena);
  if (e->d_tile_jobs) (void)hipFree(e->d_tile_jobs);
  e->tile_arena = nullptr;
  e->d_tile_jobs = nullptr;
  e->n_tile_jobs = e->n_tile_fwd_jobs = e->tile_blocks = e->tile_fwd_blocks = 0;
  for (auto& c : e->conv) {
    c.tile_fwd = nullptr;
    c.tile_fwd_bn = 0;
    for (auto& d : c.dg) {
      d.tile_pk = nullptr;
      d.tile_bn = 0;
    }
  }
}

int plan_tile_packs(cvx_engine* e, int B, bool training) {
  free_tile_packs(e);
  struct Ref {
    int op, q;
    TilePackPlan tp;
    ConvParams cp;
  };
  std::vector<Ref> refs;
  std::vector<size_t> offs;
  size_t total = 0;
  auto add = [&](const ConvParams& cp, int op, int q) {
    TilePackPlan tp;
    if (!cvx_conv_tile_supported(cp) || !cvx_conv_tile_plan(cp, &tp)) return;
    offs.push_back(total);
    total += (tp.bytes + 255) / 256 * 256;
    refs.push_back(Ref{op, q, tp, cp});
  };
  for (size_t i = 0; i < e->ops.size(); ++i) {
    if (e->ops[i].type != CVX_OP_CONV || e->conv[i].stem) continue;
    ConvParams cp;
    fill_conv_fwd(e, (int)i, B, &cp);
    add(cp, (int)i, -1);
  }
  const int n_fwd = (int)refs.size();
  if (training) {
    for (size_t i = 0; i < e->ops.size(); ++i) {
      const cvx_op_desc& o = e->ops[i];
      const ConvRt& c = e->conv[i];
      if (o.type != CVX_OP_CONV || c.stem || !o.needs_dgrad || c.sh_dg < 0 || c.ndg != 1) continue;
      if (c.dg[0].ph.OH2 <= 0 || c.dg[0].ph.OW2 <= 0 || c.dg[0].ph.ntaps <= 0) continue;
      ConvParams cp;
      fill_conv_dgrad(e, (int)i, 0, B, dense_dy(e->ops[i]), &cp);
      add(cp, (int)i, 0);
    }
  }
  if (refs.empty()) return 0;
  CVX_HIP(hipMalloc((void**)&e->tile_arena, total));
  const size_t jb = cvx_conv_tile_job_bytes();
  std::vector<unsigned char> jobs(refs.size() * jb);
  int blocks = 0, fwd_blocks = 0;
  for (size_t k = 0; k < refs.size(); ++k) {
    half_t* dst = reinterpret_cast<half_t*>(reinterpret_cast<char*>(e->tile_arena) + offs[k]);
    blocks += cvx_conv_tile_fill_job(refs[k].cp, refs[k].tp, dst, blocks, jobs.data() + k * jb);
    if ((int)k + 1 == n_fwd) fwd_blocks = blocks;
    ConvRt& c = e->conv[refs[k].op];
    if (refs[k].q < 0) {
      c.tile_fwd = dst;
      c.tile_fwd_bn = refs[k].tp.BN;
    } else {
      c.dg[refs[k].q].tile_pk = dst;
      c.dg[refs[k].q].tile_bn = refs[k].tp.BN;
    }
  }
  if (n_fwd == 0) fwd_blocks = 0;
  CVX_HIP(hipMalloc(&e->d_tile_jobs, jobs.size()));
  CVX_HIP(hipMemcpy(e->d_tile_jobs, jobs.data(), jobs.size(), hipMemcpyHostToDevice));
  e->n_tile_jobs = (int)refs.size();
  e->n_tile_fwd_jobs = n_fwd;
  e->tile_blocks = blocks;
  e->tile_fwd_blocks = fwd_blocks;
  return 0;
}

}

namespace {
struct AuxStreams {
  hipStream_t side = nullptr, red = nullptr, lane = nullptr, xchg = nullptr;
};
std::mutex g_aux_mu;
std::map<int, AuxStreams> g_aux;
template <typename Make>
hipError_t shared_stream(int device, hipStream_t AuxStreams::*which, hipStream_t* out, Make make) {
  std::lock_guard<std::mutex> lk(g_aux_mu);
  AuxStreams& a = g_aux[device];
  if (!(a.*which)) {
    hipStream_t s = nullptr;
    const hipError_t rc = make(&s);
    if (rc != hipSuccess) return rc;
    a.*which = s;
  }
  *out = a.*which;
  return hipSuccess;
}
}

static std::atomic<int> g_live_engines{0};

extern "C" int cvx_engine_create(cvx_engine** out, const cvx_buf_desc* bufs, int32_t nbufs, const cvx_op_desc* ops, int32_t nops,
                                 int32_t image_buf, int32_t pred_buf, int32_t device, void* hip_stream) {
  CVX_CHECK(out && bufs && ops && nbufs > 0 && nops > 0, "null arguments");
  CVX_HIP(hipSetDevice(device));
  cvx_engine* e = new cvx_engine();
  e->device = device;
  e->stream = (hipStream_t)hip_stream;
  e->bufs.resize(nbufs);
  for (int i = 0; i < nbufs; ++i) e->bufs[i].d = bufs[i];
  e->ops.assign(ops, ops + nops);
  e->image_buf = image_buf;
  e->pred_buf = pred_buf;
  if (!(image_buf >= 0 && image_buf < nbufs && bufs[image_buf].c == 8 && pred_buf >= 0 && pred_buf < nbufs &&
        bufs[pred_buf].kind == CVX_BUF_PRED_F32)) {
    delete e;
    CVX_FAIL("image_buf must be an 8-channel fp16 buffer and pred_buf a PRED_F32 buffer");
  }
  int rc = build_static(e);
  if (rc == 0) {
    static const bool side_prio = cvx_tune_int("CVX_SIDE_PRIO", 1) != 0;
    int prio_least = 0, prio_greatest = 0;
    (void)hipDeviceGetStreamPriorityRange(&prio_least, &prio_greatest);
    hipError_t side_rc;
    static const int side_cus = cvx_tune_int("CVX_SIDE_CUS", 0);
    side_rc = shared_stream(e->device, &AuxStreams::side, &e->side, [&](hipStream_t* s) {
      if (side_cus > 0) {
        uint32_t mask[8] = {0, 0, 0, 0, 0, 0, 0, 0};
        for (int c = 0; c < side_cus && c < 256; ++c) mask[c >> 5] |= 1u << (c & 31);
        return hipExtStreamCreateWithCUMask(s, 8, mask);
      }
      return side_prio ? hipStreamCreateWithPriority(s, hipStreamNonBlocking, prio_least) : hipStreamCreateWithFlags(s, hipStreamNonBlocking);
    });
    static const bool red_own = cvx_tune_int("CVX_RED_OWN_STREAM", 0) != 0;
    if (side_rc == hipSuccess && !red_own) e->red = e->side;
    else if (side_rc == hipSuccess)
      side_rc = shared_stream(e->device, &AuxStreams::red, &e->red, [&](hipStream_t* s) {
        return side_prio ? hipStreamCreateWithPriority(s, hipStreamNonBlocking, prio_least) : hipStreamCreateWithFlags(s, hipStreamNonBlocking);
      });
    if (side_rc != hipSuccess || hipEventCreateWithFlags(&e->ev_red, cvx_event_flags()) != hipSuccess ||
        hipEventCreateWithFlags(&e->ev_fork, cvx_event_flags()) != hipSuccess ||
        hipEventCreateWithFlags(&e->ev_join, cvx_event_flags()) != hipSuccess ||
        hipEventCreateWithFlags(&e->ev_mid, cvx_event_flags()) != hipSuccess) {
      cvx_set_error("cvx_engine_create: could not create the side stream / events");
// ... 375 lines not shown
    if (o.type == CVX_OP_MAXPOOL3S2) {
      ProfScope ps(e, PROF_MISC, 0, 2.0 * B * (o.ih * o.iw + o.oh * o.ow) * o.in.c, st);
      CVX_CHECK(o.oh == (o.ih - 1) / 2 + 1 && o.ow == (o.iw - 1) / 2 + 1, "maxpool3s2: output size must be floor((i - 1) / 2) + 1");
      CVX_TRY(cvx_maxpool3(make_view(e, o.in, false), make_view(e, o.out, false), B, o.ih, o.iw, o.in.c, 2, training ? e->pool[i].idx : nullptr, st));
      continue;
    }
    if (o.type == CVX_OP_MAXPOOL3S1) {
      ProfScope ps(e, PROF_MISC, 0, 4.0 * B * o.ih * o.iw * o.in.c, st);
      CVX_CHECK(o.oh == o.ih && o.ow == o.iw, "maxpool3s1: same-size output");
      CVX_TRY(cvx_maxpool3(make_view(e, o.in, false), make_view(e, o.out, false), B, o.ih, o.iw, o.in.c, 1, training ? e->pool[i].idx : nullptr, st));
      continue;
    }
    if (o.type == CVX_OP_L2NORM) {
      ProfScope ps(e, PROF_MISC, 0, 4.0 * B * o.ih * o.iw * o.in.c, st);
      CVX_TRY(cvx_l2norm(make_view(e, o.in, false), make_view(e, o.out, false), e->params + o.gamma_off, B, o.ih * o.iw, o.in.c, st));
      continue;
    }
    if (o.type == CVX_OP_AVGPOOL) {
      ProfScope ps(e, PROF_MISC, 0, 2.0 * B * o.ih * o.iw * o.in.c, st);
      CVX_CHECK(o.oh == 1 && o.ow == 1, "avgpool: global pooling only (1x1 output)");
      CVX_TRY(cvx_avgpool_global(make_view(e, o.in, false), make_view(e, o.out, false), B, o.ih * o.iw, o.in.c, st));
      continue;
    }
    if (o.type == CVX_OP_RESIZE) {
      ProfScope ps(e, PROF_MISC, 0, 2.0 * B * (o.ih * o.iw + o.oh * o.ow) * o.in.c, st);
      CVX_TRY(cvx_resize_bilinear(make_view(e, o.in, false), make_view(e, o.out, false), B, o.ih, o.iw, o.oh, o.ow, o.in.c, st));
      continue;
    }
    if (o.type == CVX_OP_DROPOUT) {
      ProfScope ps(e, PROF_MISC, 0, 4.0 * B * o.ih * o.iw * o.in.c, st);
      CVX_TRY(cvx_dropout(make_view(e, o.in, false), make_view(e, o.out, false), B, o.ih * o.iw, o.in.c, training ? dropout_p(o) : 0.f,
                          dropout_seed(e, (int)i), 0, st));
      continue;
    }
    ConvRt& c = e->conv[i];
    const long long M = (long long)B * o.oh * o.ow;
    const int C = o.out.c;
    if (c.stem) {
      const StemParams sp{images, B, ib.d.h, ib.d.w, o.oh, o.ow, e->params + o.w_off, C};
      const double img_bytes = 12.0 * B * ib.d.h * ib.d.w;
      ViewDesc outv = make_view(e, o.out, false);
      if (training) {
        {
          ProfScope ps(e, PROF_CONV_FWD, conv_flops(o, B), img_bytes, st);
          CVX_TRY(cvx_stem_stats(sp, c.stat_fwd, st));
        }
        ProfScope ps(e, PROF_CONV_FWD, conv_flops(o, B), img_bytes + 4.0 * M * C, st);
        BnTrainArgs ta{c.stat_fwd,           e->params + o.gamma_off, e->params + o.beta_off, c.mean, c.invstd, e->stats + o.rmean_off,
                       e->stats + o.rvar_off, e->bn_eps,       e->bn_momentum};
        const bool keep_xhat = cvx_stem_keeps_xhat(sp, make_view(e, o.out, true), c.nsplit);
        CVX_TRY(cvx_stem_apply_train(sp, ta, outv, keep_xhat ? c.ybuf : nullptr, st));
      } else {
        ProfScope ps(e, PROF_CONV_FWD, conv_flops(o, B), img_bytes + 2.0 * M * C, st);
        CVX_TRY(cvx_stem_apply_eval(sp, c.scale, c.shift, outv, st));
      }
      continue;
    }
    ConvParams cp;
    fill_conv_fwd(e, (int)i, B, &cp);
    if (o.act == CVX_ACT_BIAS) {
      cp.epi = CVX_EPI_BIAS_F32;
      cp.bias = e->params + o.bias_off;
      cp.out32 = pred + (long long)o.out.pix_off * pb.d.c + o.out.coff;
      cp.out_ld = pb.d.c;
      cp.out_bstride = A * pb.d.c;
      ProfScope ps(e, PROF_CONV_FWD, conv_flops(o, B), conv_bytes(o, B) + 2.0 * M * C, st);
      CVX_TRY(cvx_conv_igemm_launch(cp, st));
      continue;
    }
    ViewDesc outv = make_view(e, o.out, false);
    ViewDesc resv = make_view(e, o.res, false);
    if (training && o.act != CVX_ACT_BIAS_RELU && o.act != CVX_ACT_BIAS_LINEAR) {
      cp.epi = CVX_EPI_RAW_STATS;
      cp.out32 = ytmp;
      cp.out_ld = C;
      cp.out_bstride = (long long)o.oh * o.ow * C;
      if (c.raw16) {
        cp.raw16 = 1;
        cp.out32 = nullptr;
        cp.out16 = c.ybuf;
      }
      cp.stats = c.stat_fwd;
      cp.stats_replicas = cvx_stat_replicas(C);
      {
        ProfScope ps(e, PROF_CONV_FWD, conv_flops(o, B), conv_bytes(o, B) + (c.raw16 ? 0.0 : 2.0 * M * C), st);
        CVX_TRY(cvx_conv_igemm_launch(cp, st));
      }
      ProfScope ps(e, PROF_BN_FWD, 0, (c.raw16 ? 4.0 : resv.p ? 10.0 : 8.0) * M * C, st);
      BnTrainArgs ta{c.stat_fwd,           e->params + o.gamma_off, e->params + o.beta_off, c.mean, c.invstd, e->stats + o.rmean_off,
                     e->stats + o.rvar_off, e->bn_eps,       e->bn_momentum};
      if (o.flags & CVX_OPF_CONV_BIAS) ta.cbias = e->params + o.bias_off;
      if (c.raw16) CVX_TRY(cvx_bn_silu_apply_raw16(c.ybuf, M, C, o.oh * o.ow, ta, outv, st));
      else CVX_TRY(cvx_bn_act_apply(ytmp, M, C, o.oh * o.ow, ta, outv, resv, act_kind(o), (o.flags & CVX_OPF_RES_PRE_ACT) ? 1 : 0, c.ybuf, st));
    } else {
      cp.epi = CVX_EPI_AFFINE_SILU;
      cp.act_kind = act_kind(o);
      cp.res_pre = (o.flags & CVX_OPF_RES_PRE_ACT) ? 1 : 0;
      cp.scale = c.scale;
      cp.shift = c.shift;
      cp.out16 = outv.p;
      cp.out_ld = outv.ld;
      cp.out_bstride = outv.bstride;
      cp.res = resv.p;
      cp.res_ld = resv.ld;
      cp.res_bstride = resv.bstride;
      ProfScope ps(e, PROF_CONV_FWD, conv_flops(o, B), conv_bytes(o, B), st);
      CVX_TRY(cvx_conv_igemm_launch(cp, st));
    }
  }
  if (lane_used) {
    CVX_HIP(hipEventRecord(e->ev_lane_join, e->lane));
    CVX_HIP(hipStreamWaitEvent(main_st, e->ev_lane_join, 0));
  }
  e->cur_op = -1;
  e->fwd_train_done = training != 0;
  e->last_batch = B;
  return 0;
}

struct PendingWgrad {
  WgradParams wp;
  bool stem;
  StemParams sp;
  ViewDesc gout;
  BnCoef coef;
  const long long* part;
  float inv_scale;
  float *dgamma, *dbeta;
  double flops, bytes;
  int op;
  float* dw = nullptr;
};
struct cvx_bw_state {
  half_t* dpred = nullptr;
  float inv_scale = 1.f;
  int B = 0;
  bool active = false;
  int wg_batch = 1;
  int next_op = -1;
  bool lane_pending = false;
  int lane_join_op = -1;
  hipStream_t pending_stream = nullptr;
  std::vector<PendingWgrad> pending;
};
static cvx_bw_state& bw_of(cvx_engine* e) {
  if (!e->bw) e->bw = new cvx_bw_state();
  return *e->bw;
}

namespace {

int flush_wgrads(cvx_engine* e, hipEvent_t ev, hipStream_t producer) {
  cvx_bw_state& w = bw_of(e);
  if (w.pending.empty()) return 0;
  CVX_HIP(hipEventRecord(ev, producer));
  CVX_HIP(hipStreamWaitEvent(e->side, ev, 0));
  for (const PendingWgrad& g : w.pending) {
    e->cur_op = g.op;
    if (g.stem) {
      ProfScope ps(e, PROF_CONV_WGRAD, g.flops, g.bytes, producer);
      CVX_TRY(cvx_stem_backward_fold(g.sp, g.wp.dy , g.gout, g.coef, g.part, g.inv_scale, g.dgamma, g.dbeta, g.dw, g.wp.slabs, g.wp.nsplit, producer));
      continue;
    }
    static const bool skip = cvx_tune_int("CVX_TUNE_SKIP_WGRAD", 0) != 0;
    if (skip) continue;
    ProfScope ps(e, PROF_CONV_WGRAD, g.flops, g.bytes, e->side);
    CVX_TRY(cvx_conv_wgrad_launch(g.wp, e->side));
// ... 123 lines not shown
    }
    if (o.type == CVX_OP_MAXPOOL3S2 || o.type == CVX_OP_MAXPOOL3S1) {
      ProfScope ps(e, PROF_MISC, 0, (2.0 * o.ih * o.iw + 3.0 * o.oh * o.ow) * B * o.in.c, st);
      CVX_TRY(cvx_maxpool3_bwd(make_view(e, o.out, true), make_view(e, o.in, true), B, o.ih, o.iw, o.in.c, o.type == CVX_OP_MAXPOOL3S2 ? 2 : 1,
                               e->pool[i].idx, e->pool[i].in_accum, st));
      return 0;
    }
    if (o.type == CVX_OP_AVGPOOL) {
      ProfScope ps(e, PROF_MISC, 0, (e->pool[i].in_accum ? 4.0 : 2.0) * B * o.ih * o.iw * o.in.c, st);
      CVX_TRY(cvx_avgpool_global_bwd(make_view(e, o.out, true), make_view(e, o.in, true), B, o.ih * o.iw, o.in.c, e->pool[i].in_accum, st));
      return 0;
    }
    if (o.type == CVX_OP_RESIZE) {
      ProfScope ps(e, PROF_MISC, 0, 2.0 * B * (o.ih * o.iw + o.oh * o.ow) * o.in.c, st);
      CVX_TRY(cvx_resize_bilinear_bwd(make_view(e, o.out, true), make_view(e, o.in, true), B, o.ih, o.iw, o.oh, o.ow, o.in.c, e->pool[i].in_accum,
                                      st));
      return 0;
    }
    if (o.type == CVX_OP_DROPOUT) {
      ProfScope ps(e, PROF_MISC, 0, 4.0 * B * o.ih * o.iw * o.in.c, st);
      CVX_TRY(cvx_dropout(make_view(e, o.out, true), make_view(e, o.in, true), B, o.ih * o.iw, o.in.c, dropout_p(o), dropout_seed(e, i),
                          e->pool[i].in_accum, st));
      return 0;
    }
    CVX_CHECK(o.type == CVX_OP_CONV, "op without a backward pass");
    ConvRt& c = e->conv[i];
    const long long M = (long long)B * o.oh * o.ow;
    const int C = o.out.c;
    const int hw = o.oh * o.ow;
    const ViewDesc dyv = dy_view(e, i, w.dpred);
    if (o.act == CVX_ACT_BIAS_RELU || o.act == CVX_ACT_BIAS_LINEAR) {
      ProfScope ps(e, PROF_BN_BWD, 0, 6.0 * M * C, st);
      CVX_TRY(cvx_bias_act_bwd(make_view(e, o.out, true), make_view(e, o.out, false), o.act == CVX_ACT_BIAS_RELU ? 1 : 0, M, C, hw, c.dybuf, c.stat_bwd,
                               w.inv_scale, e->grads + o.bias_off, st));
    } else if (o.act != CVX_ACT_BIAS) {
      ViewDesc gout = make_view(e, o.out, true);
      ViewDesc gres = make_view(e, o.res, true);
      BnCoef k{c.invstd, e->params + o.gamma_off, e->params + o.beta_off, c.raw16 ? c.mean : nullptr};
      const bool pre = (o.flags & CVX_OPF_RES_PRE_ACT) != 0 && o.res.buf >= 0;
      const BnActKind ak{act_kind(o), pre ? 1 : 0, act_kind(o) == 0 && pre ? make_view(e, o.res, false) : ViewDesc{nullptr, 0, 0}};
      ProfScope ps(e, PROF_BN_BWD, 0, (c.stem ? 4.0 : (gres.p ? 14.0 : 10.0)) * M * C, st);
      static const bool tune_skip_reduce = cvx_tune_int("CVX_TUNE_SKIP_BN_REDUCE", 0) != 0;
      int one = 1;
      if (!c.stem && !c.raw16 && st == e->stream && !tune_skip_reduce)
        one = cvx_bn_bwd_fused(c.ybuf, M, C, hw, k, c.stat_bwd, reinterpret_cast<unsigned long long*>(c.stat_bwd + (long long)cvx_stat_replicas(C) * C * CVX_STAT_WORDS),
                               w.inv_scale, e->grads + o.gamma_off, e->grads + o.beta_off, gout, ak, c.dybuf, gres, c.res_accum, st);
      if (one < 0) return one;
      bool stem_onepass = false;
      if (c.stem && e->last_images) {
        const Buf& ib = e->bufs[e->image_buf];
        stem_onepass = cvx_stem_backward_onepass_ok(StemParams{e->last_images, B, ib.d.h, ib.d.w, o.oh, o.ow, e->params + o.w_off, C}, c.ybuf, gout, c.nsplit);
      }
      if (one == 1 && !tune_skip_reduce && !stem_onepass) CVX_TRY(cvx_bn_bwd_reduce(c.ybuf, M, C, hw, k, gout, ak, c.stat_bwd, st));
      if (one == 1 && !c.stem)
        CVX_TRY(cvx_bn_bwd_apply(c.ybuf, M, C, hw, k, c.stat_bwd, w.inv_scale, e->grads + o.gamma_off, e->grads + o.beta_off, gout, ak, c.dybuf,
                                 gres, c.res_accum, st));
    }
    auto queue_wgrad = [&]() -> int {
      WgradParams wp;
      fill_wgrad(e, i, B, dyv, e->slabs + c.slab_off, c.nsplit, &wp);
      PendingWgrad pw{wp, c.stem, StemParams{}, ViewDesc{nullptr, 0, 0}, BnCoef{nullptr, nullptr, nullptr}, nullptr, 0.f, nullptr, nullptr,
                      conv_flops(o, B), conv_bytes(o, B) + 4.0 * c.nsplit * C * c.ntaps * c.cin_pad16, i};
      if (c.stem) {
        const Buf& ib = e->bufs[e->image_buf];
        CVX_CHECK(e->last_images, "the stem's weight gradient needs the images of the training forward");
        pw.sp = StemParams{e->last_images, B, ib.d.h, ib.d.w, o.oh, o.ow, e->params + o.w_off, C};
        pw.bytes = 12.0 * B * ib.d.h * ib.d.w + 4.0 * M * C + 4.0 * c.nsplit * C * 144;
        pw.wp.dy = c.ybuf;
        pw.gout = make_view(e, o.out, true);
        pw.coef = BnCoef{c.invstd, e->params + o.gamma_off, e->params + o.beta_off, c.mean};
        pw.part = c.stat_bwd;
        pw.inv_scale = w.inv_scale;
        pw.dgamma = e->grads + o.gamma_off;
        pw.dbeta = e->grads + o.beta_off;
        pw.dw = e->grads + o.w_off;
      }
      w.pending.push_back(pw);
      if ((int)w.pending.size() >= w.wg_batch || i <= e->slab_tail_op || e->slab_tail_op < 0) CVX_TRY(flush_wgrads(e, c.ev_dy, st));
      return 0;
    };
    static const int wgrad_early = cvx_tune_int("CVX_WGRAD_EARLY", 1);
    const bool wgrad_first = !c.stem && (wgrad_early >= 2 || (wgrad_early == 1 && e->slab_tail_op >= 0 && i <= e->slab_tail_op));
    if (wgrad_first) CVX_TRY(queue_wgrad());
    if (o.needs_dgrad) {
      ViewDesc gin = make_view(e, o.in, true);
      static const bool merge_off = cvx_tune_set("CVX_NO_PHASE_MERGE");
      const bool merged = !merge_off && phases_mergeable(c.dg, c.ndg);
      bool empty_phase = false;
      for (int q = 0; q < c.ndg; ++q) empty_phase |= c.dg[q].ph.OH2 > 0 && c.dg[q].ph.OW2 > 0 && c.dg[q].ph.ntaps == 0;
      if (empty_phase && !c.in_accum) CVX_TRY(cvx_zero_slice(gin, B, o.ih * o.iw, o.in.c, st));
      if (c.ps_on) {
        ConvParams cp;
        fill_conv_ps(e, i, B, dyv, &cp);
        const double fl = 2.0 * B * o.oh * o.ow * (double)o.in.c * c.ntaps * C;
        ProfScope ps(e, PROF_CONV_DGRAD, fl, conv_bytes(o, B) + (c.in_accum ? 2.0 * B * o.ih * o.iw * o.in.c : 0.0), st);
        CVX_TRY(cvx_conv_igemm_launch(cp, st));
      }
      for (int q = 0; q < c.ndg && !c.ps_on; ++q) {
        if (merged && q > 0) break;
        const DgClass& dc = c.dg[q];
        if (dc.ph.OH2 <= 0 || dc.ph.OW2 <= 0 || dc.ph.ntaps == 0) continue;
        ConvParams cp;
        fill_conv_dgrad(e, i, q, B, dyv, &cp);
        double fl = 2.0 * B * dc.ph.OH2 * dc.ph.OW2 * (double)o.in.c * dc.ph.ntaps * C;
        double by = (conv_bytes(o, B) + (c.in_accum ? 2.0 * B * o.ih * o.iw * o.in.c : 0.0)) / c.ndg;
        if (merged) {
          set_merged_phases(c.dg, c.ndg, &cp);
          fl = 0;
          for (int z = 0; z < c.ndg; ++z) fl += 2.0 * B * c.dg[z].ph.OH2 * c.dg[z].ph.OW2 * (double)o.in.c * c.dg[z].ph.ntaps * C;
          by *= c.ndg;
        }
        ProfScope ps(e, PROF_CONV_DGRAD, fl, by, st);
        CVX_TRY(cvx_conv_igemm_launch(cp, st));
      }
    }
    if (!wgrad_first) CVX_TRY(queue_wgrad());
  return 0;
}

}

extern "C" int cvx_engine_backward(cvx_engine* e, const void* dpred_f16, float loss_scale) {
  CVX_TRY(backward_begin(e, dpred_f16, loss_scale));
  cvx_bw_state& w = bw_of(e);
  hipStream_t st = e->stream;
  const float inv_scale = w.inv_scale;
  hipStream_t rs = e->red;
  static const int chunk_convs = cvx_tune_int("CVX_SLAB_CHUNK", 6);
  double slab_bytes = 0;
  int chunk_hi = -1, in_chunk = 0;
  auto reduce_chunk = [&](int lo, int hi, bool first, hipStream_t on) -> int {
    const int blk0 = e->conv[lo].slab_blk0, blk1 = e->conv[hi].slab_blk1;
    if (blk1 <= blk0) return 0;
    ProfScope ps(e, PROF_SLAB_REDUCE, 0, first ? slab_bytes + 8.0 * e->n_params : 0.0, on);
    return cvx_reduce_slabs(e->slabs, e->grads, inv_scale, e->d_slab, e->d_slab_blocks + blk0, blk1 - blk0, on);
  };
  for (size_t i = 0; i < e->ops.size(); ++i)
    if (e->ops[i].type == CVX_OP_CONV) slab_bytes += 4.0 * e->conv[i].nsplit * e->ops[i].out.c * e->conv[i].ntaps * e->conv[i].cin_pad16;
  bool first = true;
  int lo_conv = -1;
  for (int i = (int)e->ops.size() - 1; i >= 0; --i) {
    CVX_TRY(backward_op(e, i));
    if (e->ops[i].type != CVX_OP_CONV) continue;
    if (chunk_hi < 0) chunk_hi = i;
    lo_conv = i;
    ++in_chunk;
    if (in_chunk >= chunk_convs && w.pending.empty() && i > 1) {
      if (rs != e->side) {
        CVX_HIP(hipEventRecord(e->ev_mid, e->side));
        CVX_HIP(hipStreamWaitEvent(rs, e->ev_mid, 0));
      }
      CVX_TRY(reduce_chunk(i, chunk_hi, first, rs));
      first = false;
      chunk_hi = -1;
      in_chunk = 0;
    }
  }
  w.active = false;
  CVX_TRY(join_lane(e));
  CVX_TRY(flush_wgrads(e, e->ev_fork, st));
  e->cur_op = -1;
  static const bool tail_on_main = cvx_tune_int("CVX_TAIL_REDUCE_MAIN", 0) != 0;
  if (tail_on_main) {
    CVX_HIP(hipEventRecord(e->ev_red, rs));
    if (rs != e->side) {
      CVX_HIP(hipEventRecord(e->ev_join, e->side));
      CVX_HIP(hipStreamWaitEvent(st, e->ev_join, 0));
    }
    CVX_HIP(hipStreamWaitEvent(st, e->ev_red, 0));
    if (chunk_hi >= 0) CVX_TRY(reduce_chunk(lo_conv, chunk_hi, first, st));
    return 0;
  }
  if (rs != e->side) {
    CVX_HIP(hipEventRecord(e->ev_join, e->side));
    CVX_HIP(hipStreamWaitEvent(rs, e->ev_join, 0));
  }
  if (chunk_hi >= 0) CVX_TRY(reduce_chunk(lo_conv, chunk_hi, first, rs));
  CVX_HIP(hipEventRecord(e->ev_red, rs));
  CVX_HIP(hipStreamWaitEvent(st, e->ev_red, 0));
  return 0;
}
// ... 133 lines not shown
    if (hipEventElapsedTime(&t, e->ev_pool[2 * r], e->ev_pool[2 * r + 1]) != hipSuccess) t = -1.f;
    const auto& rec = e->prof_recs[r];
    fprintf(f, "%d,%d,%.0f,%.0f,%.6f\n", rec.cls, rec.op, rec.flops, rec.bytes, t);
  }
  fclose(f);
  e->ev_used = 0;
  e->prof_recs.clear();
  return 0;
}

extern "C" int cvx_pred_level_to_nchw(const float* pred, int32_t batch, int32_t anchors, int32_t no, int32_t a_off, int32_t h, int32_t w,
                                      float* out_nchw, void* hip_stream) {
  return cvx_pred_to_nchw(pred, batch, anchors, no, a_off, h, w, out_nchw, (hipStream_t)hip_stream);
}
extern "C" int cvx_nchw_grad_to_dpred(const float* grad_nchw, int32_t batch, int32_t anchors, int32_t no, int32_t a_off, int32_t h, int32_t w,
                                      float scale, void* dpred_f16, void* hip_stream) {
  return cvx_nchw_to_pred_f16(grad_nchw, batch, anchors, no, a_off, h, w, scale, (half_t*)dpred_f16, (hipStream_t)hip_stream);
}
extern "C" int cvx_engine_set_stream(cvx_engine* e, void* hip_stream) {
  CVX_CHECK(e, "null engine");
  e->stream = (hipStream_t)hip_stream;
  return 0;
}
extern "C" void* cvx_engine_exchange_stream(cvx_engine* e) {
  if (!e) return nullptr;
  static const bool own = cvx_tune_int("CVX_XCHG_OWN_STREAM", 0) != 0;
  if (!own) return (void*)e->side;
  int prio_least = 0, prio_greatest = 0;
  (void)hipDeviceGetStreamPriorityRange(&prio_least, &prio_greatest);
  hipStream_t s = nullptr;
  if (shared_stream(e->device, &AuxStreams::xchg, &s, [&](hipStream_t* out) { return hipStreamCreateWithPriority(out, hipStreamNonBlocking, prio_least); }) !=
      hipSuccess) {
    (void)hipGetLastError();
    cvx_set_error("cvx_engine_exchange_stream: could not create the stream");
    return nullptr;
  }
  return (void*)s;
}

namespace {
struct DevTemps {
  std::vector<void*> ptrs;
  DevTemps() = default;
  DevTemps(const DevTemps&) = delete;
  DevTemps& operator=(const DevTemps&) = delete;
  ~DevTemps() {
    for (void* p : ptrs) (void)hipFree(p);
  }
  template <typename T>
  int alloc(T** out, size_t bytes) {
    void* p = nullptr;
    CVX_HIP(hipMalloc(&p, bytes));
    ptrs.push_back(p);
    *out = (T*)p;
    return 0;
  }
  int taps(const std::vector<ConvTap>& host, const ConvTap** dev, const half_t** zeros = nullptr) {
    const size_t tb = ((host.size() * sizeof(ConvTap) + 255) / 256) * 256;
    char* p = nullptr;
    CVX_TRY(alloc(&p, tb + 256));
    CVX_HIP(hipMemset(p, 0, tb + 256));
    CVX_HIP(hipMemcpy(p, host.data(), host.size() * sizeof(ConvTap), hipMemcpyHostToDevice));
    *dev = reinterpret_cast<const ConvTap*>(p);
    if (zeros) *zeros = reinterpret_cast<const half_t*>(p + tb);
    return 0;
  }
};
ViewDesc dense_view(const void* p, long long pixels, int c) { return ViewDesc{(half_t*)p, pixels * c, c}; }
long long unit_wgrad_splits(long long M) { return std::min<long long>(std::max<long long>(1, M / 256), 64); }
}

extern "C" int cvx_conv2d_nhwc(const void* x_f16, int32_t batch, int32_t ih, int32_t iw, int32_t cin, const void* w_f16, int32_t cout,
                               int32_t k, int32_t stride, int32_t pad, int32_t dil, int32_t mode, const float* scale_or_bias,
                               const float* shift, void* out, void* hip_stream) {
  CVX_CHECK(x_f16 && w_f16 && out && k * k <= CVX_MAX_TAPS && stride >= 1 && dil >= 1, "bad arguments");
  hipStream_t st = (hipStream_t)hip_stream;
  const bool force_gemm = (mode & 0x100) != 0;
  const int gemm_variant = (mode >> 9) & 15;
  const bool force_tile = (mode & 0x2000) != 0;
  const bool no_tile = (mode & 0x4000) != 0;
  const bool force_dma = (mode & 0x8000) != 0;
  const bool force_halo = (mode & 0x10000) != 0;
  const bool force_pw = (mode & 0x20000) != 0;
  mode &= 0xff;
  const int oh = cvx_conv_out_size(ih, k, stride, pad, dil), ow = cvx_conv_out_size(iw, k, stride, pad, dil);
  const std::vector<ConvTap> taps = cvx_conv_fwd_taps(k, pad, dil);
  DevTemps tmp;
  const ConvTap* dt = nullptr;
  const half_t* zeros = nullptr;
  CVX_TRY(tmp.taps(taps, &dt, &zeros));
  ConvParams cp;
  fill_conv_fwd(ConvGeom{batch, ih, iw, cin, oh, ow, cout, stride, k * k}, dense_view(x_f16, (long long)ih * iw, cin), (const half_t*)w_f16, dt,
                cvx_tap_traits(taps), zeros, &cp);
  cp.out_ld = cout;
  cp.out_bstride = (long long)oh * ow * cout;
  if (mode == 0) {
    cp.epi = CVX_EPI_PLAIN;
    cp.out16 = (half_t*)out;
  } else if (mode == 1) {
    cp.epi = CVX_EPI_AFFINE_SILU;
    cp.scale = scale_or_bias;
    cp.shift = shift;
    cp.out16 = (half_t*)out;
  } else if (mode == 2) {
    cp.epi = CVX_EPI_BIAS_F32;
    cp.bias = scale_or_bias;
    cp.out32 = (float*)out;
  } else {
    CVX_CHECK(shift, "mode 3 needs the statistics slab (cvx_stat_replicas(cout) * cout * 4 64-bit words, zeroed) in `shift`");
    cp.epi = CVX_EPI_RAW_STATS;
    cp.out32 = (float*)out;
    cp.stats = (long long*)shift;
    cp.stats_replicas = cvx_stat_replicas(cout);
  }
  int rc;
  cp.gemm_variant = gemm_variant;
  if (force_gemm) {
    CVX_CHECK(cvx_conv_gemm_shape_ok(cp), "shape outside the GEMM-shaped kernel (cin % 8, cout % 4)");
    rc = cvx_conv_gemm_launch(cp, st);
  } else if (force_tile) {
    CVX_CHECK(cvx_conv_tile_shape_ok(cp), "shape outside the row-band kernel (3x3 stride 1, cin % 8, cin >= 32)");
    cp.clk = g_cvx_clk;
    rc = cvx_conv_tile_launch(cp, st);
  } else if (force_dma) {
    CVX_CHECK(cin % 8 == 0 && cout % 4 == 0 && oh > 0 && ow > 0 && batch > 0, "shape outside the ring kernel (cin % 8, cout % 4, a non-empty output)");
    CVX_CHECK(((uintptr_t)x_f16 % 16) == 0 && ((uintptr_t)w_f16 % 16) == 0, "conv: operands must be 16-byte aligned");
    cp.clk = g_cvx_clk;
    rc = cvx_conv_igemm_dma_launch(cp, st);
  } else if (force_halo || force_pw) {
    CVX_CHECK(cin % 8 == 0 && cout % 4 == 0 && oh > 0 && ow > 0 && batch > 0, "shape outside the kernel (cin % 8, cout % 4, a non-empty output)");
    CVX_CHECK(((uintptr_t)x_f16 % 16) == 0 && ((uintptr_t)w_f16 % 16) == 0, "conv: operands must be 16-byte aligned");
    cp.clk = g_cvx_clk;
    if (force_halo) {
      CVX_CHECK(cvx_conv_halo_supported(cp), "shape outside the halo kernel (3x3, stride 1, pad 1, dilation 1, cin 16 / 32 / 64 / 80 / 128 / 144)");
      rc = cvx_conv_halo_launch(cp, st);
    } else {
      CVX_CHECK(cvx_conv_pw_supported(cp), "shape outside the pointwise kernel (1x1, stride 1, pad 0, cin <= 512)");
      rc = cvx_conv_pw_launch(cp, st);
    }
  } else {
    cp.no_tile = no_tile ? 1 : 0;
    rc = cvx_conv_igemm_launch(cp, st);
  }
  (void)hipStreamSynchronize(st);
  return rc;
}

extern "C" int cvx_conv2d_dgrad_nhwc(const void* dy_f16, int32_t batch, int32_t ih, int32_t iw, int32_t cin, const void* wt_f16, int32_t cout,
                                     int32_t k, int32_t stride, int32_t pad, int32_t dil, void* dx_f16, void* hip_stream) {
  CVX_CHECK(dy_f16 && wt_f16 && dx_f16 && k * k <= CVX_MAX_TAPS && stride >= 1 && stride <= 4, "bad arguments");
  hipStream_t st = (hipStream_t)hip_stream;
  const int oh = cvx_conv_out_size(ih, k, stride, pad, dil), ow = cvx_conv_out_size(iw, k, stride, pad, dil);
  const ConvGeom g{batch, ih, iw, cin, oh, ow, cout, stride, k * k};
  const ViewDesc dy = dense_view(dy_f16, (long long)oh * ow, cout), dx = dense_view(dx_f16, (long long)ih * iw, cin);
  const std::vector<DgradPhase> phases = cvx_conv_dgrad_phases(k, stride, pad, dil, ih, iw);
  const PsDgrad ps = cvx_conv_ps_dgrad(k, stride, pad, dil, ih, iw, phases);
  if (ps.qualifies && cout % 32 == 0 && cin % 8 == 0) {
    DevTemps tmp;
    const ConvTap* dt = nullptr;
    const half_t* zeros = nullptr;
    CVX_TRY(tmp.taps(cvx_conv_ps_window_taps(), &dt, &zeros));
    ConvParams cp;
    fill_conv_ps(g, dy, dx, nullptr, dt, zeros, 0, &cp);
    if (cvx_conv_gemm_supported(cp)) {
      half_t* psw = nullptr;
      CVX_CHECK(tmp.alloc(&psw, (size_t)16 * cin * cout * 2) == 0, "dgrad: out of memory for the pixel-shuffle weights");
      cp.wt = psw;
      PsPackDesc pd{0, 0, cin, k * k, cout, {}};
      for (int q = 0; q < 16; ++q) pd.wtap[q] = ps.wtap[q];
      int rc = cvx_pack_ps_weights((const half_t*)wt_f16, psw, pd, st);
      if (rc == 0) rc = cvx_conv_igemm_launch(cp, st);
      (void)hipStreamSynchronize(st);
      return rc;
    }
  }
  if (phases.size() >= 2 && phases.size() <= 4) {
    DevTemps tmp;
    DgClass dg[4];
    const half_t* zeros = nullptr;
    for (size_t q = 0; q < phases.size(); ++q) {
      const ConvTap* dt = nullptr;
      if (!phases[q].taps.empty()) CVX_TRY(tmp.taps(phases[q].taps, &dt, &zeros));
      dg[q].ph = make_phase(phases[q], dt);
    }
    if (phases_mergeable(dg, (int)phases.size())) {
      ConvParams cp;
      fill_conv_dgrad(g, dg[0].ph, dy, dx, (const half_t*)wt_f16, zeros, 0, &cp);
      set_merged_phases(dg, (int)phases.size(), &cp);
      const int rc = cvx_conv_igemm_launch(cp, st);
      (void)hipStreamSynchronize(st);
      return rc;
    }
  }
  int rc = 0;
  for (size_t q = 0; q < phases.size() && rc == 0; ++q) {
    const DgradPhase& d = phases[q];
    if (d.OH2 <= 0 || d.OW2 <= 0) continue;
    CVX_CHECK(!d.taps.empty(), "dgrad phase without taps");
    DevTemps tmp;
    const ConvTap* dt = nullptr;
    const half_t* zeros = nullptr;
    CVX_TRY(tmp.taps(d.taps, &dt, &zeros));
    ConvParams cp;
    fill_conv_dgrad(g, make_phase(d, dt), dy, dx, (const half_t*)wt_f16, zeros, 0, &cp);
    rc = cvx_conv_igemm_launch(cp, st);
    (void)hipStreamSynchronize(st);
  }
  return rc;
}

extern "C" int64_t cvx_conv2d_wgrad_workspace_bytes(int32_t batch, int32_t oh, int32_t ow, int32_t cin, int32_t cout, int32_t k) {
  return unit_wgrad_splits((long long)batch * oh * ow) * cout * k * k * round_up(cin, 16) * 4 + 4096;
}

extern "C" int cvx_conv2d_wgrad_nhwc(const void* x_f16, const void* dy_f16, int32_t batch, int32_t ih, int32_t iw, int32_t cin, int32_t cout,
                                     int32_t k, int32_t stride, int32_t pad, int32_t dil, float* dw, void* workspace, int64_t workspace_bytes,
                                     void* hip_stream) {
  CVX_CHECK(x_f16 && dy_f16 && dw && workspace && k * k <= CVX_MAX_TAPS, "bad arguments");
  hipStream_t st = (hipStream_t)hip_stream;
  const int oh = cvx_conv_out_size(ih, k, stride, pad, dil), ow = cvx_conv_out_size(iw, k, stride, pad, dil);
  CVX_CHECK(workspace_bytes >= cvx_conv2d_wgrad_workspace_bytes(batch, oh, ow, cin, cout, k), "workspace too small");
  const std::vector<ConvTap> taps = cvx_conv_fwd_taps(k, pad, dil);
  DevTemps tmp;
  const ConvTap* dt = nullptr;
  CVX_TRY(tmp.taps(taps, &dt));
  WgradParams wp;
// ... 61 lines not shown
```

include/cvx_engine.h:

```cpp
#ifndef CVX_ENGINE_H
#define CVX_ENGINE_H
#include <stdint.h>
#ifdef __cplusplus
extern "C" {
#endif

#define CVX_ABI_VERSION 5

const char* cvx_last_error(void);
int cvx_abi_version(void);

enum { CVX_BUF_ACT_F16 = 0, CVX_BUF_PRED_F32 = 1 };
typedef struct {
  int32_t h, w, c;
  int32_t kind;
} cvx_buf_desc;

typedef struct {
  int32_t buf;
  int32_t coff;
  int32_t c;
  int32_t pix_off;
} cvx_view;

enum { CVX_OP_CONV = 1, CVX_OP_MAXPOOL5 = 2, CVX_OP_UPSAMPLE2 = 3,
       CVX_OP_MAXPOOL2 = 4,
       CVX_OP_DWCONVT = 5,
       CVX_OP_COPY = 6,
       CVX_OP_MAXPOOL3S2 = 7,
       CVX_OP_AVGPOOL = 8,
       CVX_OP_RESIZE = 9,
       CVX_OP_MAXPOOL3S1 = 10,
       CVX_OP_L2NORM = 11,
       CVX_OP_DROPOUT = 12 };
enum { CVX_ACT_BN_SILU = 1, CVX_ACT_BIAS = 2,
       CVX_ACT_BN_RELU = 3,
       CVX_ACT_BN_LINEAR = 4,
       CVX_ACT_BIAS_RELU = 5,
       CVX_ACT_BIAS_LINEAR = 6 };
#define CVX_OPF_RES_PRE_ACT 1
#define CVX_OPF_CONV_BIAS 2
#define CVX_OPF_RAW_F16 4

typedef struct {
  int32_t type;
  cvx_view in, out, res;
  int32_t ih, iw, oh, ow;
  int32_t k, stride, pad, dil;
  int32_t act;
  int32_t needs_dgrad;
  int32_t w_cin;
  int64_t w_off;
  int64_t gamma_off, beta_off;
  int64_t bias_off;
  int64_t rmean_off, rvar_off;
  int32_t lane;
  int32_t flags;
} cvx_op_desc;

typedef struct cvx_engine cvx_engine;

int cvx_engine_create(cvx_engine** out, const cvx_buf_desc* bufs, int32_t nbufs, const cvx_op_desc* ops, int32_t nops,
                      int32_t image_buf, int32_t pred_buf, int32_t device, void* hip_stream);
int cvx_engine_destroy(cvx_engine* e);

int cvx_engine_bind(cvx_engine* e, float* params, float* grads, int64_t n_params, float* stats, int64_t n_stats);

int cvx_engine_set_stream(cvx_engine* e, void* hip_stream);
void* cvx_engine_exchange_stream(cvx_engine* e);

int cvx_engine_set_bn(cvx_engine* e, float eps, float momentum);
int cvx_engine_keep_shadows(cvx_engine* e);
int cvx_engine_set_fusion(cvx_engine* e, int32_t enable);
int32_t cvx_engine_fused_groups(const cvx_engine* e);

int cvx_engine_set_seed(cvx_engine* e, uint64_t seed);

int cvx_engine_forward(cvx_engine* e, const float* images, int32_t batch, int32_t training, float* pred);

int cvx_engine_backward(cvx_engine* e, const void* dpred_f16, float loss_scale);

int cvx_engine_debug_copy(cvx_engine* e, int32_t buf, int32_t which, void* dst, int64_t bytes);

int cvx_engine_backward_begin(cvx_engine* e, const void* dpred_f16, float loss_scale);
int cvx_engine_backward_range(cvx_engine* e, int32_t op_hi, int32_t op_lo);
int cvx_engine_grads_ready(cvx_engine* e, int32_t op_hi, int32_t op_lo, void* hip_stream);
int cvx_engine_backward_end(cvx_engine* e);

int cvx_engine_profile(cvx_engine* e, int32_t enable);
int cvx_engine_profile_read(cvx_engine* e, int32_t n_classes, double* ms, double* flops, double* bytes, int64_t* launches);
int cvx_engine_profile_dump(cvx_engine* e, const char* path);

int cvx_debug_clock_buffer(void* buf);

int cvx_debug_conv_tile_plan(int32_t batch, int32_t h, int32_t w, int32_t cin, int32_t cout, int32_t* out8);
int cvx_debug_conv_dma_plan(int64_t pixels, int32_t cin, int32_t cout, int32_t ntaps, int32_t* out4);
int cvx_debug_conv_halo_plan(int32_t batch, int32_t h, int32_t w, int32_t cin, int32_t cout, int32_t* out4);
int cvx_debug_conv_pw_plan(int64_t pixels, int32_t cin, int32_t cout, int32_t* out4);
int cvx_debug_conv_grid_div(int32_t div);

int64_t cvx_engine_workspace_bytes(const cvx_engine* e);
int64_t cvx_engine_plan_generation(const cvx_engine* e);

int cvx_pred_level_to_nchw(const float* pred, int32_t batch, int32_t anchors, int32_t no, int32_t a_off, int32_t h, int32_t w,
                           float* out_nchw, void* hip_stream);
int cvx_nchw_grad_to_dpred(const float* grad_nchw, int32_t batch, int32_t anchors, int32_t no, int32_t a_off, int32_t h, int32_t w,
                           float scale, void* dpred_f16, void* hip_stream);

int64_t cvx_loss_v8_workspace_bytes(int32_t batch, int32_t anchors, int32_t nc, int32_t max_targets_per_image);
int cvx_loss_v8(const float* pred, int32_t batch, int32_t anchors, int32_t nc, const float* targets, int32_t n_targets,
                int32_t max_targets_per_image, const int32_t* level_hw, const float* strides, int32_t n_levels, float gain_box,
                float gain_cls, float gain_dfl, float loss_scale, float* loss_items, void* dpred_f16, void* workspace,
                int64_t workspace_bytes, void* hip_stream);
int cvx_loss_v8_strided(const float* pred, int32_t pred_ld, int32_t batch, int32_t anchors, int32_t nc, const float* targets,
                        int32_t n_targets, int32_t max_targets_per_image, const int32_t* level_hw, const float* strides, int32_t n_levels,
                        float gain_box, float gain_cls, float gain_dfl, float loss_scale, float* loss_items, void* dpred_f16,
                        void* workspace, int64_t workspace_bytes, void* hip_stream);

int cvx_loss_v8_assignment(const void* workspace, int32_t batch, int32_t anchors, int32_t max_targets_per_image, int32_t* gt_index,
                           float* norm_score, void* hip_stream);
int cvx_pack_targets(const float* batch_idx, const float* cls, const float* bboxes, int32_t n, float* rows, void* hip_stream);

int cvx_letterbox_geometry(int32_t h, int32_t w, int32_t H, int32_t W, int32_t* new_h, int32_t* new_w, int32_t* top, int32_t* left, double* scale);
int cvx_letterbox_u8_to_nchw(const uint8_t* image_hwc, int32_t h, int32_t w, int32_t letterbox, int32_t swap_rb, float* out_chw, int32_t H,
                             int32_t W, void* hip_stream);
typedef struct cvx_letterbox_job {
  const uint8_t* src;
  int32_t h, w, out, reserved;
} cvx_letterbox_job;
int cvx_letterbox_batch_u8_to_nchw(const cvx_letterbox_job* jobs, int32_t n_jobs, int32_t letterbox, int32_t swap_rb, float* out_nchw, int32_t H,
                                   int32_t W, void* hip_stream);

int cvx_adam_step(float* params, float* grads, float* exp_avg, float* exp_avg_sq, int64_t n, float lr, float beta1, float beta2,
                  float eps, int32_t step, const int32_t* found_inf, int32_t zero_grad, void* hip_stream);
int cvx_check_finite(const float* grads, int64_t n, int32_t* found_inf, void* hip_stream);
int cvx_adam_step_dev(float* params, float* grads, float* exp_avg, float* exp_avg_sq, int64_t n, float beta1, float beta2, float eps,
                      float* state, const int32_t* found_inf, int32_t zero_grad, float grad_scale, void* hip_stream);

int cvx_ema_update(float* ema, const float* src, int64_t n, float d, float one_minus_d, void* hip_stream);
int cvx_adam_ema_step_dev(float* params, float* grads, float* exp_avg, float* exp_avg_sq, int64_t n, float beta1, float beta2, float eps,
                          float* state, const int32_t* found_inf, int32_t zero_grad, float grad_scale, float* ema, float d, float one_minus_d,
                          void* hip_stream);

enum { CVX_OPTIM_SGD = 0, CVX_OPTIM_ADAM = 1 };
#define CVX_OPTIM_MAX_GROUPS 16
#define CVX_OPTIM_GROUP_FLOATS 8
#define CVX_OPTIM_UNMAPPED 255
int cvx_optim_step(int32_t kind, float* params, float* grads, float* buf1, float* buf2, int64_t n, const uint8_t* group_map, float* group_state,
                   int32_t n_groups, float* state, float beta1, float beta2, float eps, const int32_t* found_inf, int32_t zero_grad,
                   float grad_scale, const float* clip_state, float* ema, float d, float one_minus_d, void* hip_stream);
int64_t cvx_grad_norm_workspace(int64_t n);
int cvx_grad_norm(const float* grads, int64_t n, const uint8_t* group_map, const float* group_state, int32_t n_groups, float grad_scale,
                  float max_norm, float* clip_state, int32_t* found_inf, float* workspace, int64_t workspace_floats, void* hip_stream);

int cvx_decode(const float* pred, int32_t batch, int32_t anchors, int32_t nc, const int32_t* level_hw, const float* strides,
               int32_t n_levels, float* y, void* hip_stream);
int cvx_decode_strided(const float* pred, int32_t pred_ld, int32_t batch, int32_t anchors, int32_t nc, const int32_t* level_hw,
                       const float* strides, int32_t n_levels, float* y, void* hip_stream);
int cvx_ssd_decode(const float* loc, const float* conf, const float* priors, int32_t batch, int32_t anchors, int32_t num_classes_plus_bg,
                   float variance_xy, float variance_wh, float* boxes, float* prob, void* hip_stream);
int cvx_ssd_decode_max(const float* loc, const float* conf, const float* priors, int32_t B, int32_t A, int32_t num_classes_plus_bg,
                       float variance_xy, float variance_wh, float* boxes, float* prob, float* class_max, void* hip_stream);
int cvx_pred_cols_to_nchw(const float* rows, int32_t ld, int32_t col0, int32_t c, int32_t batch, int32_t anchors, int32_t a_off, int32_t hw,
                          float* out, int64_t out_bstride, int64_t out_off, void* hip_stream);
int cvx_yolo7_decode(const float* pred, int32_t pred_ld, int32_t batch, int32_t nc, const int32_t* level_hw, const float* anchors_wh,
                     int32_t n_levels, int32_t input_h, int32_t input_w, float* dec, float* y, void* hip_stream);
enum { CVX_NMS_TV0141_CUDA = 0,
       CVX_NMS_TV0141_CPU = 1,
       CVX_NMS_OFFSET = 2,
       CVX_NMS_VANILLA = 3 };
#define CVX_NMS_BOXES_XYXY 0x100
int64_t cvx_nms_workspace_bytes(int32_t batch, int32_t anchors);
int cvx_nms(const float* y, int32_t batch, int32_t anchors, int32_t nc, float conf_thres, float iou_thres, int32_t max_det,
            float* out_rows, int32_t* out_index, int32_t* counts, void* workspace, int64_t workspace_bytes, void* hip_stream);
int cvx_nms_variant(const float* y, int32_t batch, int32_t anchors, int32_t nc, float conf_thres, float iou_thres, int32_t max_det,
                    int32_t variant, float* out_rows, int32_t* out_index, int32_t* counts, void* workspace, int64_t workspace_bytes,
                    void* hip_stream);

int64_t cvx_centernet_decode_workspace_bytes(int32_t batch, int32_t h, int32_t w, int32_t nc);
int cvx_centernet_decode(const float* pred, int32_t pred_ld, int32_t batch, int32_t h, int32_t w, int32_t nc, int32_t reg_col, int32_t wh_col,
                         int32_t k, float conf, float nms_thr, int32_t use_nms, float* boxes, float* scores, int32_t* classes,
                         int32_t* topk_index, int32_t* keep, int32_t* counts, void* workspace, int64_t workspace_bytes, void* hip_stream);

int cvx_conv2d_nhwc(const void* x_f16, int32_t batch, int32_t ih, int32_t iw, int32_t cin, const void* w_f16, int32_t cout, int32_t k,
                    int32_t stride, int32_t pad, int32_t dil, int32_t mode, const float* scale_or_bias, const float* shift, void* out,
                    void* hip_stream);
int cvx_conv2d_dgrad_nhwc(const void* dy_f16, int32_t batch, int32_t ih, int32_t iw, int32_t cin, const void* wt_f16, int32_t cout,
                          int32_t k, int32_t stride, int32_t pad, int32_t dil, void* dx_f16, void* hip_stream);
int64_t cvx_conv2d_wgrad_workspace_bytes(int32_t batch, int32_t oh, int32_t ow, int32_t cin, int32_t cout, int32_t k);
int cvx_conv2d_wgrad_nhwc(const void* x_f16, const void* dy_f16, int32_t batch, int32_t ih, int32_t iw, int32_t cin, int32_t cout,
                          int32_t k, int32_t stride, int32_t pad, int32_t dil, float* dw, void* workspace, int64_t workspace_bytes,
                          void* hip_stream);


int cvx_bn_silu_train_nhwc(const float* y_f32, int32_t batch, int32_t hw, int32_t c, const float* gamma, const float* beta, float eps,
                           float momentum, float* running_mean, float* running_var, const void* res_f16, void* out_f16, void* xhat_f16,
                           float* mean, float* invstd, void* hip_stream);
int cvx_bn_silu_bwd_nhwc(const void* xhat_f16, const void* gout_f16, int32_t batch, int32_t hw, int32_t c, const float* gamma,
                         const float* beta, const float* invstd, float inv_scale, float* dgamma, float* dbeta, void* dy_f16, void* gres_f16,
                         int32_t res_accumulate, void* hip_stream);
int cvx_bn_act_train_nhwc(const float* y_f32, int32_t batch, int32_t hw, int32_t c, const float* gamma, const float* beta, float eps,
                          float momentum, float* running_mean, float* running_var, const void* res_f16, int32_t act, int32_t res_pre,
                          void* out_f16, void* xhat_f16, float* mean, float* invstd, void* hip_stream);
int cvx_bn_act_bwd_nhwc(const void* xhat_f16, const void* gout_f16, const void* out_f16, int32_t batch, int32_t hw, int32_t c,
                        const float* gamma, const float* beta, const float* invstd, int32_t act, int32_t res_pre, float inv_scale,
                        float* dgamma, float* dbeta, void* dy_f16, void* gres_f16, int32_t res_accumulate, void* hip_stream);
int cvx_maxpool5_nhwc(const void* x_f16, int32_t batch, int32_t h, int32_t w, int32_t c, void* out_f16, uint8_t* argmax, void* hip_stream);
int cvx_maxpool5_bwd_nhwc(const void* gout_f16, const uint8_t* argmax, int32_t batch, int32_t h, int32_t w, int32_t c, void* gin_f16,
                          int32_t accumulate, void* hip_stream);
int cvx_maxpool_nhwc(const void* x_f16, int32_t batch, int32_t h, int32_t w, int32_t c, int32_t kernel, int32_t stride, int32_t ceil_mode,
                     void* out_f16, void* hip_stream);
int cvx_avgpool_global_nhwc(const void* x_f16, int32_t batch, int32_t hw, int32_t c, void* out_f16, void* hip_stream);
int cvx_resize_bilinear_nhwc(const void* x_f16, int32_t batch, int32_t ih, int32_t iw, int32_t c, int32_t oh, int32_t ow, void* out_f16,
                             void* hip_stream);
int cvx_l2norm_nhwc(const void* x_f16, const float* weight, int32_t batch, int32_t hw, int32_t c, void* out_f16, void* hip_stream);
int cvx_resize_bilinear_rows_to_nchw(const float* rows_f32, int32_t ld, int32_t batch, int32_t c, int32_t ih, int32_t iw, int32_t oh, int32_t ow,
                                     float* out_nchw, void* hip_stream);
#define CVX_SEG_OPTS_KEY_OFFSET 4096
#define CVX_SEG_DIMS_BYTES 28
#define CVX_SEG_CRITERION_BYTES 128
typedef struct cvx_seg_dims {
  int32_t ld, batch, nc, ih, iw, oh, ow;
} cvx_seg_dims;
typedef struct cvx_seg_criterion {
  int32_t base;
  float focal_alpha, focal_gamma;
  const float* class_weight;
  float label_smoothing;
  int64_t ignore_index;
  float ohem_theta;
  int64_t ohem_min_kept;
  int32_t region;
  double base_weight, weight, alpha, beta, gamma, smooth;
  int32_t per_image, skip_absent;
  const float* region_class_weight;
} cvx_seg_criterion;
int64_t cvx_seg_criterion_workspace_bytes(const cvx_seg_dims* dims, const cvx_seg_criterion* crit, int32_t for_eval);
int cvx_seg_criterion_loss(const float* rows_f32, const cvx_seg_dims* dims, const int64_t* target, const cvx_seg_criterion* crit, float loss_scale,
                           float* loss_out, void* dpred_f16, int32_t* bad_target, double* stats_out, double* region_stats_out, void* workspace,
                           void* hip_stream);
int cvx_seg_criterion_eval(const float* rows_f32, const cvx_seg_dims* dims, const int64_t* target, const cvx_seg_criterion* crit, int64_t* confusion,
                           float* loss_out, double* region_stats_out, void* workspace, void* hip_stream);
int cvx_det_match(const float* rows, const int32_t* counts, int32_t batch, int32_t max_det, int32_t box_mode, const float* box_map,
                  const int32_t* gt, const int32_t* gt_counts, int32_t max_gt, int32_t nc, double min_overlap, int32_t quantize,
                  float* rec_score, int32_t* rec_class, int32_t* rec_flag, int64_t capacity, int64_t* state, int64_t* gt_per_class,
                  void* hip_stream);
int cvx_det_ap(const float* score, const int32_t* flag, const int64_t* seg_off, const int64_t* gt_per_class, int32_t nc,
               double score_threshold, int32_t quantize, double* prec, double* rec, double* stats, void* hip_stream);
int cvx_coco_match(const float* rows, const int32_t* counts, int32_t batch, int32_t max_det, int32_t box_mode, const float* box_map,
                   int32_t truncate, int32_t quantize, const double* gt, const int32_t* gt_counts, int32_t max_gt, int32_t nc,
                   const double* iou_thrs, float* rec_score, int32_t* rec_class, int32_t* rec_rank, int64_t* rec_matched, int64_t* rec_ignored,
                   int64_t capacity, int64_t* state, int64_t* npig, void* hip_stream);
int cvx_coco_accumulate(const int32_t* rank, const int64_t* matched, const int64_t* ignored, const int64_t* seg_off, const int64_t* npig,
                        int32_t nc, const double* rec_thrs, double* precision, double* recall, void* hip_stream);
int cvx_coco_summarize(const double* precision, const double* recall, int32_t nc, double* stats, void* hip_stream);
int64_t cvx_centernet_loss_workspace_bytes(int32_t batch, int32_t anchors);
int cvx_centernet_loss(const float* rows_f32, int32_t ld, int32_t batch, int32_t anchors, int32_t nc, int32_t col_a, int32_t col_b,
                       const float* heat_true, const float* true_a, const float* true_b, const float* mask, const int64_t* indices,
                       int32_t max_objects, float hm_weight, float a_weight, float b_weight, float loss_scale, float* loss_items, void* dpred_f16,
                       int32_t* bad_index, void* workspace, void* hip_stream);
int64_t cvx_multibox_loss_workspace_bytes(int32_t batch, int32_t anchors);
int cvx_multibox_loss(const float* loc, const float* conf, const float* y_true, int32_t batch, int32_t anchors, int32_t nc1, float neg_pos_ratio,
                      float alpha, float grad_scale, float* loss_items, float* dloc, float* dconf, void* workspace, void* hip_stream);
int64_t cvx_yolo7_loss_workspace_bytes(int32_t batch, int32_t anchors, int32_t ld, int32_t n_targets);
int cvx_yolo7_loss(const float* rows_f32, int32_t ld, int32_t batch, int32_t nc, const int32_t* level_hw, const float* anchors_px, const float* strides,
                   const float* targets, int32_t n_targets, float img_size, float box_ratio, float obj_ratio, float cls_ratio, float label_smoothing,
                   float loss_scale, float* loss_items, void* dpred_f16, int32_t* bad, void* workspace, void* hip_stream);
int cvx_debug_yolo7_loss_layout(int32_t batch, int32_t anchors, int32_t ld, int32_t n_targets, int64_t* offsets);
int cvx_centernet_draw_targets(const float* labels, const int32_t* counts, int32_t batch, int32_t max_boxes, int32_t fh, int32_t fw, int32_t nc,
                               float* heatmap, float* reg, float* wh, float* reg_mask, float* indices, void* hip_stream);
int cvx_ssd_encode_targets(const float* labels, const int32_t* counts, int32_t batch, int32_t max_boxes, const float* priors, int32_t anchors, int32_t nc1,
// ... 177 lines not shown
```

Before: 5660 images/sec.

## Extend row-band tile conv kernel to stride-2 forward and four-phase data gradient

Generalizes the row-band tiled 3x3 convolution kernel with compile-time variants for stride-2 forward and a four-phase stride-2 data gradient. Cost-model gates choose these over the existing ring/DMA and pixel-shuffle GEMM paths when enough pixels are involved. The engine pre-packs weights for the new dgrad path and routes it at backward time. The aim is better patch and weight reuse in LDS for YOLOv8's downsampling convs. The risks are planner heuristics picking a slower route and extra weight-pack memory.

```diff
diff --git a/__graft_entry__.py b/__graft_entry__.py
--- a/__graft_entry__.py
+++ b/__graft_entry__.py
@@ -6,7 +6,7 @@
 CSRC = os.path.join(ROOT, "computervision.pytorch_amd", "csrc")
 LIBDIR = os.path.join(ROOT, "computervision.pytorch_amd", "lib")
 LIB = os.path.join(LIBDIR, "libcvx_engine.so")
-SOURCES = ["conv_igemm.hip", "conv_igemm_dma.hip", "conv_halo.hip", "conv_tile.hip", "conv_tile_k1.hip", "conv_tile_k2.hip", "conv_gemm.hip", "conv_stem7.hip", "conv_pw.hip", "conv_wgrad.hip", "conv_wgrad_gemm.hip", "conv_wgrad_halo.hip", "conv_wgrad_stream.hip", "conv_wgrad_k3.hip", "bn_act.hip", "stem.hip", "unit_ops.hip", "misc_ops.hip", "loss_v8.hip", "loss_seg.hip", "loss_centernet.hip", "loss_multibox.hip", "loss_yolov7.hip", "preprocess.hip", "augment.hip", "seg_pipeline.hip", "det_eval.hip", "coco_eval.hip", "nms.hip", "centernet_decode.hip", "render.hip", "tiles.hip", "seg_tiles.hip", "seg_tta.hip", "det_tta.hip", "track.hip", "optim.hip", "comm.hip", "engine.hip"]
+SOURCES = ["conv_igemm.hip", "conv_igemm_dma.hip", "conv_halo.hip", "conv_tile.hip", "conv_tile_k1.hip", "conv_tile_k2.hip", "conv_tile_s2_k1.hip", "conv_tile_s2_k2.hip", "conv_tile_dg_k1.hip", "conv_tile_dg_k2.hip", "conv_gemm.hip", "conv_stem7.hip", "conv_pw.hip", "conv_wgrad.hip", "conv_wgrad_gemm.hip", "conv_wgrad_halo.hip", "conv_wgrad_stream.hip", "conv_wgrad_k3.hip", "bn_act.hip", "stem.hip", "unit_ops.hip", "misc_ops.hip", "loss_v8.hip", "loss_seg.hip", "loss_centernet.hip", "loss_multibox.hip", "loss_yolov7.hip", "preprocess.hip", "augment.hip", "seg_pipeline.hip", "det_eval.hip", "coco_eval.hip", "nms.hip", "centernet_decode.hip", "render.hip", "tiles.hip", "seg_tiles.hip", "seg_tta.hip", "det_tta.hip", "track.hip", "optim.hip", "comm.hip", "engine.hip"]
 
 
 def _stale(out, deps):
diff --git a/computervision.pytorch_amd/_lib.py b/computervision.pytorch_amd/_lib.py
--- a/computervision.pytorch_amd/_lib.py
+++ b/computervision.pytorch_amd/_lib.py
@@ -7,7 +7,7 @@
 
 _HERE = os.path.dirname(os.path.abspath(__file__))
 LIB_PATH = os.environ.get("CVX_LIB") or os.path.join(_HERE, "lib", "libcvx_engine.so")
-ABI_VERSION = 5
+ABI_VERSION = 6
 SEG_OPTS_KEY_OFFSET = 4096
 
 
@@ -87,6 +87,8 @@
                                        C.POINTER(_I64)]),
     "cvx_debug_clock_buffer": (_I32, [_P]),
     "cvx_debug_conv_tile_plan": (_I32, [_I32, _I32, _I32, _I32, _I32, _P]),
+    "cvx_debug_conv_tile_s2_plan": (_I32, [_I32, _I32, _I32, _I32, _I32, _I32, _P]),
+    "cvx_debug_conv_tile_rows": (_I32, [_I32]),
     "cvx_debug_conv_dma_plan": (_I32, [_I64, _I32, _I32, _I32, _P]),
     "cvx_debug_conv_halo_plan": (_I32, [_I32, _I32, _I32, _I32, _I32, _P]),
     "cvx_debug_conv_pw_plan": (_I32, [_I64, _I32, _I32, _P]),
@@ -124,6 +126,7 @@
     "cvx_centernet_decode": (_I32, [_P, _I32, _I32, _I32, _I32, _I32, _I32, _I32, _I32, _F, _F, _I32, _P, _P, _P, _P, _P, _P, _P, _I64, _P]),
     "cvx_conv2d_nhwc": (_I32, [_P, _I32, _I32, _I32, _I32, _P, _I32, _I32, _I32, _I32, _I32, _I32, _P, _P, _P, _P]),
     "cvx_conv2d_dgrad_nhwc": (_I32, [_P, _I32, _I32, _I32, _I32, _P, _I32, _I32, _I32, _I32, _I32, _P, _P]),
+    "cvx_conv2d_dgrad_mode_nhwc": (_I32, [_P, _I32, _I32, _I32, _I32, _P, _I32, _I32, _I32, _I32, _I32, _I32, _P, _P]),
     "cvx_conv2d_wgrad_workspace_bytes": (_I64, [_I32, _I32, _I32, _I32, _I32, _I32]),
     "cvx_conv2d_wgrad_nhwc": (_I32, [_P, _P, _I32, _I32, _I32, _I32, _I32, _I32, _I32, _I32, _I32, _P, _P, _I64, _P]),
     "cvx_bn_silu_train_nhwc": (_I32, [_P, _I32, _I32, _I32, _P, _P, _F, _F, _P, _P, _P, _P, _P, _P, _P, _P]),
diff --git a/computervision.pytorch_amd/csrc/conv_igemm.h b/computervision.pytorch_amd/csrc/conv_igemm.h
--- a/computervision.pytorch_amd/csrc/conv_igemm.h
+++ b/computervision.pytorch_amd/csrc/conv_igemm.h
@@ -64,6 +64,8 @@
   int no_tile;
   int ps_cin;
   int raw16;
+  int tile_dg, OHr;
+  unsigned tile_dg_taps, tile_dg_phase;
 };
 
 __device__ __forceinline__ void cvx_store_raw4(const ConvParams& p, long long off, const f4& v) {
diff --git a/computervision.pytorch_amd/csrc/conv_igemm.hip b/computervision.pytorch_amd/csrc/conv_igemm.hip
--- a/computervision.pytorch_amd/csrc/conv_igemm.hip
+++ b/computervision.pytorch_amd/csrc/conv_igemm.hip
@@ -25,6 +25,10 @@
               "conv: pixel-shuffle data gradient needs the GEMM-shaped kernel (plain epilogue, 4 phases of ps_cin channels, output stride 2)");
     return cvx_conv_gemm_launch(p, stream);
   }
+  if (p.tile_dg) {
+    CVX_CHECK(p.epi == CVX_EPI_PLAIN && p.nphase <= 1 && cvx_conv_tile_shape_ok(p), "conv: the four-phase data gradient needs the row-band kernel (3x3 / stride 2 / pad 1, plain epilogue)");
+    return cvx_conv_tile_launch(p, stream);
+  }
   if (p.nphase > 1) return cvx_conv_igemm_dma_launch(p, stream);
   if (cvx_conv_stem7_supported(p)) return cvx_conv_stem7_launch(p, stream);
   if (cvx_conv_tile_supported(p)) return cvx_conv_tile_launch(p, stream);
diff --git a/computervision.pytorch_amd/csrc/conv_tile.h b/computervision.pytorch_amd/csrc/conv_tile.h
--- a/computervision.pytorch_amd/csrc/conv_tile.h
+++ b/computervision.pytorch_amd/csrc/conv_tile.h
@@ -7,6 +7,7 @@
 typedef __attribute__((address_space(3))) void* lds_ptr_t;
 
 constexpr int kTileWaves = 8;
+constexpr int kTileS1 = 0, kTileS2 = 1, kTileDg = 2;
 
 struct TileArgs {
   int TR, tiles_per_img, ntiles, NB;
@@ -19,6 +20,8 @@
   int wring_off, CB, stat_off;
   unsigned in_records;
   const half_t* wpk;
+  int OHr;
+  unsigned dg_taps, dg_phase;
   int dbg;
 };
 
@@ -53,3 +56,7 @@
 
 int cvx_conv_tile_launch_k1(int MT, int NTW, const ConvParams& p, const cvx_tile_k::TileArgs& a, int lds, hipStream_t st);
 int cvx_conv_tile_launch_k2(int MT, int NTW, const ConvParams& p, const cvx_tile_k::TileArgs& a, int lds, hipStream_t st);
+int cvx_conv_tile_launch_s2_k1(int MT, int NTW, const ConvParams& p, const cvx_tile_k::TileArgs& a, int lds, hipStream_t st);
+int cvx_conv_tile_launch_s2_k2(int MT, int NTW, const ConvParams& p, const cvx_tile_k::TileArgs& a, int lds, hipStream_t st);
+int cvx_conv_tile_launch_dg_k1(int MT, int NTW, const ConvParams& p, const cvx_tile_k::TileArgs& a, int lds, hipStream_t st);
+int cvx_conv_tile_launch_dg_k2(int MT, int NTW, const ConvParams& p, const cvx_tile_k::TileArgs& a, int lds, hipStream_t st);
diff --git a/computervision.pytorch_amd/csrc/conv_tile.hip b/computervision.pytorch_amd/csrc/conv_tile.hip
--- a/computervision.pytorch_amd/csrc/conv_tile.hip
+++ b/computervision.pytorch_amd/csrc/conv_tile.hip
@@ -60,16 +60,20 @@
 
 unsigned magic_of(int d) { return (unsigned)((0x100000000ULL + (unsigned long long)d - 1) / (unsigned long long)d); }
 
+int g_tile_rows = 0;
+
 struct Plan {
   int MT, NTW, TR, NB, KSC, NCH, R, SPT, lds, ntiles, tpi, PP, units, CB, wring_off, stat_off;
   double cost;
 };
 
 bool plan_tile(const ConvParams& p, Plan* best) {
-  const int H = p.IH, W = p.IW, Cin = p.Cin;
+  const bool s2 = p.IS == 2, dg = p.tile_dg != 0;
+  const int H = s2 ? p.OH2 : p.IH, W = s2 ? p.OW2 : p.IW, Cin = p.Cin;
   const int P = Cin / 8, SPT = (Cin + 31) / 32, NSTEPS = 9 * SPT;
   const int ctiles = (p.Cout + 15) / 16;
-  static const int force_tr = cvx_tune_int("CVX_TILE_TR", 0), force_ntw = cvx_tune_int("CVX_TILE_NTW", 0);
+  static const int env_tr = cvx_tune_int("CVX_TILE_TR", 0), force_ntw = cvx_tune_int("CVX_TILE_NTW", 0);
+  const int force_tr = g_tile_rows > 0 ? g_tile_rows : env_tr;
   bool found = false;
   for (int NTW : kNtwMenu) {
     if (force_ntw && NTW != force_ntw) continue;
@@ -87,10 +91,10 @@
       if (MT > kMaxMT) break;
       if (MT > 4 || MT * NTW * 4 + 3 * (MT + NTW) * 4 > 216) continue;
       const int tpi = (H + TR - 1) / TR;
-      const int units = (TR + 2) * (W + 2) * P;
+      const int units = s2 ? (2 * TR + 1) * 2 * (W + 1) * P : (dg ? (TR + 1) * (W + 1) * P : (TR + 2) * (W + 2) * P);
       const int PP = (units + 63) / 64;
       const int patch_bytes = PP * 1024;
-      const int stat_bytes = kTileWaves * 16 * NTW * 2 * 4;
+      const int stat_bytes = dg ? 0 : kTileWaves * 16 * NTW * 2 * 4;
       const int budget = 160 * 1024 - patch_bytes - stat_bytes;
       int KSC = 0, R = 0;
       if (NSTEPS * NTW * 1024 <= budget && (NSTEPS * NTW + kTileWaves - 1) / kTileWaves + (PP + kTileWaves - 1) / kTileWaves <= 60) {
@@ -109,7 +113,7 @@
       if (!KSC) continue;
       const int CB = KSC * NTW * 1024;
       const int nslots = R > NSTEPS / KSC ? NSTEPS / KSC : R;
-      const int stage_bytes = kTileWaves * MT * 16 * (16 * NTW * 4 + 16);
+      const int stage_bytes = dg ? 0 : kTileWaves * MT * 16 * (16 * NTW * 4 + 16);
       const int lds = std::max(patch_bytes + nslots * CB + stat_bytes, stage_bytes);
       if (lds > 160 * 1024) continue;
       const long long wgs = (long long)tpi * p.B * NB;
@@ -120,8 +124,13 @@
       const double loop_us = std::max(std::max(mfma_cyc * 1.15, lds_cyc), valu_cyc + mfma_cyc * 0.5) / 1900.0;
       const double wbytes = (double)NSTEPS * NTW * 1024.0;
       const double load_us = (patch_bytes + CB) / 60e3 + std::max(0.0, (wbytes - CB) / 60e3 - loop_us);
-      const double epi_us = 0.6 + MT * NTW * 0.02;
-      const double t = rounds * (1.2 + load_us + loop_us + epi_us) + 1.0;
+      const double epi_us = dg ? 4 * (0.3 + MT * NTW * 0.03) : 0.6 + MT * NTW * 0.02;
+      double t = rounds * (1.2 + load_us + loop_us + epi_us) + 1.0;
+      if (s2) {
+        const double req_mb = (double)wgs * (patch_bytes + wbytes) / 1e6;
+        const double out_mb = 2.0 * p.B * H * W * p.Cout / 1e6;
+        t += 0.19 * req_mb + 0.5 * out_mb;
+      }
       if (!found || t < best->cost) {
         found = true;
         *best = Plan{MT, NTW, TR, NB, KSC, NSTEPS / KSC, R, SPT, lds, tpi * p.B, tpi, PP, units, CB, patch_bytes, patch_bytes + nslots * CB, t};
@@ -142,8 +151,16 @@
 
 bool cvx_conv_tile_shape_ok(const ConvParams& p) {
   if (!p.zeros || !p.halo_taps_ok || p.ntaps != 9) return false;
-  if (p.IS != 1 || p.OS != 1 || p.oph != 0 || p.opw != 0) return false;
-  if (p.OH2 != p.IH || p.OW2 != p.IW || p.OWr != p.IW) return false;
+  if (p.tile_dg) {
+    if (p.IS != 1 || p.OS != 2 || p.oph != 0 || p.opw != 0 || p.epi != CVX_EPI_PLAIN) return false;
+    if (p.OH2 != p.IH || p.OW2 != p.IW || p.IH != (p.OHr - 1) / 2 + 1 || p.IW != (p.OWr - 1) / 2 + 1) return false;
+  } else if ((p.IS != 1 && p.IS != 2) || p.OS != 1 || p.oph != 0 || p.opw != 0) {
+    return false;
+  } else if (p.IS == 2) {
+    if (p.OH2 != (p.IH - 1) / 2 + 1 || p.OW2 != (p.IW - 1) / 2 + 1 || p.OWr != p.OW2 || p.OW2 < 2) return false;
+  } else if (p.OH2 != p.IH || p.OW2 != p.IW || p.OWr != p.IW) {
+    return false;
+  }
   if (p.Cin % 8 != 0 || p.Cin < 32 || p.Cin > 512 || p.in_ld % 8 != 0) return false;
   if (p.Cout % 8 != 0 || p.out_ld % 8 != 0 || (p.res && p.res_ld % 8 != 0)) return false;
   if (p.IW > 4000 || p.IH > 4000 || p.IW < 2) return false;
@@ -153,10 +170,32 @@
   return plan_tile(p, &pl);
 }
 
+constexpr long long kS2MinPixels = 16384;
 bool cvx_conv_tile_supported(const ConvParams& p) {
   static const bool off = cvx_tune_set("CVX_NO_TILE");
   if (off || p.no_tile) return false;
   static const int max_w = cvx_tune_int("CVX_TILE_MAXW", 40), max_c = cvx_tune_int("CVX_TILE_MAXC", 144);
+  if (p.tile_dg) {
+    static const int route = cvx_tune_int("CVX_TILE_S2", 2);
+    if (route == 0) return false;
+    if (route == 2 && (p.Cout < 32 || (long long)p.B * p.IH * p.IW < kS2MinPixels)) return false;
+    Plan pl;
+    if (!cvx_conv_tile_shape_ok(p) || !plan_tile(p, &pl)) return false;
+    if (route == 1) return true;
+    const double ps_us = 27.0 + 0.43 * 2.0 * p.B * p.OHr * p.OWr * p.Cout / 1e6;
+    const double w_mb = (double)pl.ntiles * pl.NB * 9 * pl.SPT * pl.NTW * 1024.0 / 1e6;
+    return pl.cost + 14.0 + 0.3 * w_mb < ps_us;
+  }
+  if (p.IS == 2) {
+    static const int route = cvx_tune_int("CVX_TILE_S2", 2);
+    if (route == 0 || p.Cin > max_c) return false;
+    if (route == 2 && (long long)p.B * p.OH2 * p.OW2 < kS2MinPixels) return false;
+    Plan pl;
+    if (!cvx_conv_tile_shape_ok(p) || !plan_tile(p, &pl)) return false;
+    if (route == 1) return true;
+    const double ring_us = 12.0 + 9.0 * p.B * p.OH2 * p.OW2 * p.Cin * 2.0 / 3.0e6;
+    return pl.cost < 0.9 * ring_us;
+  }
   if (p.IW > max_w || p.IH > max_w || p.Cin > max_c) return false;
   return cvx_conv_tile_shape_ok(p);
 }
@@ -248,9 +287,13 @@
   a.PP = pl.PP;
   a.PPW = (pl.PP + kTileWaves - 1) / kTileWaves;
   a.units = pl.units;
-  a.Wp = p.IW + 2;
+  const bool s2 = p.IS == 2, dg = p.tile_dg != 0;
+  a.OHr = p.OHr;
+  a.dg_taps = p.tile_dg_taps;
+  a.dg_phase = p.tile_dg_phase;
+  a.Wp = s2 ? p.OW2 + 1 : (dg ? p.IW + 1 : p.IW + 2);
   a.magic_wp = magic_of(a.Wp);
-  a.magic_w = magic_of(p.IW);
+  a.magic_w = magic_of(s2 ? p.OW2 : p.IW);
   a.magic_p = magic_of(a.P);
   a.wring_off = pl.wring_off;
   a.CB = pl.CB;
@@ -260,10 +303,12 @@
   static const int dbg = cvx_tune_int("CVX_TILE_DBG", 0);
   a.dbg = dbg;
   int rc;
-  if (pl.MT <= 2)
-    rc = cvx_conv_tile_launch_k1(pl.MT, pl.NTW, p, a, pl.lds, stream);
+  if (dg)
+    rc = pl.MT <= 2 ? cvx_conv_tile_launch_dg_k1(pl.MT, pl.NTW, p, a, pl.lds, stream) : cvx_conv_tile_launch_dg_k2(pl.MT, pl.NTW, p, a, pl.lds, stream);
+  else if (pl.MT <= 2)
+    rc = s2 ? cvx_conv_tile_launch_s2_k1(pl.MT, pl.NTW, p, a, pl.lds, stream) : cvx_conv_tile_launch_k1(pl.MT, pl.NTW, p, a, pl.lds, stream);
   else
-    rc = cvx_conv_tile_launch_k2(pl.MT, pl.NTW, p, a, pl.lds, stream);
+    rc = s2 ? cvx_conv_tile_launch_s2_k2(pl.MT, pl.NTW, p, a, pl.lds, stream) : cvx_conv_tile_launch_k2(pl.MT, pl.NTW, p, a, pl.lds, stream);
   CVX_TRY(rc);
   CVX_HIP(hipGetLastError());
   return 0;
@@ -298,6 +343,62 @@
   return 0;
 }
 
+extern "C" int cvx_debug_conv_tile_rows(int32_t rows) {
+  CVX_CHECK(rows >= 0, "rows per tile: 0 (the planner's choice) or a positive count");
+  const int prev = g_tile_rows;
+  g_tile_rows = rows;
+  return prev;
+}
+
+extern "C" int cvx_debug_conv_tile_s2_plan(int32_t batch, int32_t ih, int32_t iw, int32_t cin, int32_t cout, int32_t dgrad, int32_t* out12) {
+  CVX_CHECK(out12 && batch > 0 && ih > 0 && iw > 0, "bad arguments");
+  ConvParams p;
+  memset(&p, 0, sizeof(p));
+  static half_t dummy_zero[8];
+  p.zeros = dummy_zero;
+  p.halo_taps_ok = 1;
+  p.ntaps = 9;
+  p.IS = 2;
+  p.OS = 1;
+  p.B = batch;
+  p.IH = ih;
+  p.IW = iw;
+  p.OH2 = (ih - 1) / 2 + 1;
+  p.OW2 = p.OWr = (iw - 1) / 2 + 1;
+  p.Cin = p.in_ld = cin;
+  p.in_bstride = (long long)ih * iw * cin;
+  p.Cout = p.out_ld = cout;
+  if (dgrad) {
+    p.IS = 1;
+    p.OS = 2;
+    p.OHr = ih;
+    p.OWr = iw;
+    p.IH = p.OH2;
+    p.IW = p.OW2;
+    p.Cin = p.in_ld = cout;
+    p.in_bstride = (long long)p.IH * p.IW * cout;
+    p.Cout = p.out_ld = cin;
+    p.epi = CVX_EPI_PLAIN;
+    p.tile_dg = 1;
+  }
+  if (!cvx_conv_tile_shape_ok(p)) return -1;
+  Plan pl;
+  if (!plan_tile(p, &pl)) return -1;
+  out12[0] = pl.TR;
+  out12[1] = pl.MT;
+  out12[2] = pl.NTW;
+  out12[3] = pl.NB;
+  out12[4] = pl.ntiles * pl.NB;
+  out12[5] = pl.KSC;
+  out12[6] = pl.lds;
+  out12[7] = (int)(pl.cost * 100.0);
+  out12[8] = pl.PP * 1024;
+  out12[9] = pl.wring_off;
+  out12[10] = pl.stat_off - pl.wring_off;
+  out12[11] = pl.stat_off;
+  return 0;
+}
+
 void cvx_conv_tile_release() {
   std::lock_guard<std::mutex> lk(g_pack_mu);
   for (auto& kv : g_pack)
diff --git a/computervision.pytorch_amd/csrc/conv_tile_dg_k1.hip b/computervision.pytorch_amd/csrc/conv_tile_dg_k1.hip
--- /dev/null
+++ b/computervision.pytorch_amd/csrc/conv_tile_dg_k1.hip
@@ -0,0 +1,5 @@
+#define CVX_TILE_MT_A 1
+#define CVX_TILE_MT_B 2
+#define CVX_TILE_KIND kTileDg
+#define CVX_TILE_LAUNCH_FN cvx_conv_tile_launch_dg_k1
+#include "conv_tile_kernel.inc.h"
diff --git a/computervision.pytorch_amd/csrc/conv_tile_dg_k2.hip b/computervision.pytorch_amd/csrc/conv_tile_dg_k2.hip
--- /dev/null
+++ b/computervision.pytorch_amd/csrc/conv_tile_dg_k2.hip
@@ -0,0 +1,5 @@
+#define CVX_TILE_MT_A 3
+#define CVX_TILE_MT_B 4
+#define CVX_TILE_KIND kTileDg
+#define CVX_TILE_LAUNCH_FN cvx_conv_tile_launch_dg_k2
+#include "conv_tile_kernel.inc.h"
diff --git a/computervision.pytorch_amd/csrc/conv_tile_kernel.inc.h b/computervision.pytorch_amd/csrc/conv_tile_kernel.inc.h
--- a/computervision.pytorch_amd/csrc/conv_tile_kernel.inc.h
+++ b/computervision.pytorch_amd/csrc/conv_tile_kernel.inc.h
@@ -1,12 +1,17 @@
 #include "conv_tile.h"
+
+#ifndef CVX_TILE_KIND
+#define CVX_TILE_KIND kTileS1
+#endif
 
 namespace {
 using namespace cvx_tile_k;
 
-template <int MT, int NTW>
+template <int MT, int NTW, int KIND>
 __global__ __launch_bounds__(64 * kTileWaves) void conv_tile_kernel(const ConvParams p, const TileArgs a) {
 #if defined(__HIP_DEVICE_COMPILE__)
   constexpr int BN = 16 * NTW;
+  constexpr bool S2 = KIND == kTileS2, DG = KIND == kTileDg;
   extern __shared__ __attribute__((aligned(16))) unsigned char smem[];
   const int tid = threadIdx.x;
   const int wave = __builtin_amdgcn_readfirstlane(tid >> 6), lane = tid & 63;
@@ -18,7 +23,8 @@
   clk_mark(p, 0);
   const int b = tile / a.tiles_per_img;
   const int y0 = (tile - b * a.tiles_per_img) * a.TR;
-  const int H = p.IH, W = p.IW, Wp = a.Wp, P = a.P;
+  const int H = S2 ? p.OH2 : p.IH, W = S2 ? p.OW2 : p.IW, Wp = a.Wp, P = a.P;
+  const int Hin = p.IH, Win = p.IW;
 
   const __amdgpu_buffer_rsrc_t rsrc_in = __builtin_amdgcn_make_buffer_rsrc(const_cast<half_t*>(p.in), (short)0, (int)a.in_records, 0x00020000);
   const half_t* wblk = a.wpk + (long long)nblk * a.NSTEPS * (BN * 32);
@@ -35,9 +41,10 @@
       const unsigned pr = __umulhi(q, a.magic_wp);
       const unsigned pc = q - pr * (unsigned)Wp;
       const unsigned c = phys ^ ((pc >> a.sh) & (unsigned)a.swmask);
-      const int y = y0 - 1 + (int)pr, x = (int)pc - 1;
-      const bool ok = u < (unsigned)a.units && (unsigned)y < (unsigned)H && (unsigned)x < (unsigned)W;
-      const unsigned vo = ok ? img_off + (unsigned)(((y * W + x) * p.in_ld + (int)c * 8) * 2) : 0xffffffffu;
+      const int y = S2 ? 2 * y0 - 1 + (int)(pr >> 1) : (DG ? y0 + (int)pr : y0 - 1 + (int)pr);
+      const int x = S2 ? 2 * (int)pc + (int)(pr & 1u) - 1 : (DG ? (int)pc : (int)pc - 1);
+      const bool ok = u < (unsigned)a.units && (unsigned)y < (unsigned)Hin && (unsigned)x < (unsigned)Win;
+      const unsigned vo = ok ? img_off + (unsigned)(((y * Win + x) * p.in_ld + (int)c * 8) * 2) : 0xffffffffu;
       __builtin_amdgcn_raw_ptr_buffer_load_lds(rsrc_in, (lds_ptr_t)(smem + piece * 1024), 16, vo, 0, 0, 0);
     }
   }
@@ -57,9 +64,10 @@
 
   const int rows_here = H - y0 < a.TR ? H - y0 : a.TR;
   const int npix = rows_here * W;
-  unsigned S0[MT], S1[MT], S2[MT];
+  unsigned S0[MT], S1[MT], S2_[MT];
   bool pvalid[MT];
-  const unsigned rowpitch = (unsigned)(Wp * P * 16);
+  const unsigned planepitch = (unsigned)(Wp * P * 16);
+  const unsigned rowpitch = S2 ? 2u * planepitch : planepitch;
 #pragma unroll
   for (int i = 0; i < MT; ++i) {
     const int m = (wave * MT + i) * 16 + fr;
@@ -67,14 +75,15 @@
     const unsigned mm = pvalid[i] ? (unsigned)m : 0u;
     const unsigned pr = __umulhi(mm, a.magic_w);
     const unsigned pc = mm - pr * (unsigned)W;
-    auto s_of = [&](unsigned col) -> unsigned {
+    auto s_of = [&](unsigned col, unsigned plane) -> unsigned {
       const unsigned sw = (col >> a.sh) & (unsigned)a.swmask;
       const unsigned ph = ((unsigned)fq ^ sw) & (unsigned)a.phmask;
-      return (pr + 1u) * rowpitch + ((col * (unsigned)P + ph) << 4);
+      const unsigned row = S2 ? (2u * pr + 1u) * rowpitch + plane * planepitch : (DG ? pr * rowpitch : (pr + 1u) * rowpitch);
+      return row + ((col * (unsigned)P + ph) << 4);
     };
-    S0[i] = s_of(pc);
-    S1[i] = s_of(pc + 1u);
-    S2[i] = s_of(pc + 2u);
+    S0[i] = s_of(pc, 0u);
+    S1[i] = S2 ? s_of(pc, 1u) : (DG ? s_of(pc, 0u) : s_of(pc + 1u, 0u));
+    S2_[i] = (S2 || DG) ? s_of(pc + 1u, 0u) : s_of(pc + 2u, 0u);
   }
 
   f4 acc[MT][NTW];
@@ -93,7 +102,7 @@
   };
 
 #pragma unroll
-  for (int i = 0; i < MT; ++i) asm volatile("" ::"v"(S0[i]), "v"(S1[i]), "v"(S2[i]));
+  for (int i = 0; i < MT; ++i) asm volatile("" ::"v"(S0[i]), "v"(S1[i]), "v"(S2_[i]));
 #pragma unroll
   for (int i = 0; i < MT; ++i)
 #pragma unroll
@@ -125,7 +134,7 @@
     const int dwi = code & 3;
     const unsigned m0 = dwi == 0 ? 0xffffffffu : 0u, m1 = dwi == 1 ? 0xffffffffu : 0u, m2 = dwi == 2 ? 0xffffffffu : 0u;
 #pragma unroll
-    for (int i = 0; i < MT; ++i) SC[i] = (S0[i] & m0) | (S1[i] & m1) | (S2[i] & m2);
+    for (int i = 0; i < MT; ++i) SC[i] = (S0[i] & m0) | (S1[i] & m1) | (S2_[i] & m2);
     return (code >> 2) - 1;
   };
   dh_cur = set_tap(0);
@@ -145,7 +154,7 @@
       if (++c_inc == KSC) {
         c_inc = 0;
         const int issued = NCH < c_chunk + R - 1 ? NCH : c_chunk + R - 1;
-        if (issued - c_chunk - 2 <= 0) wait_vmcnt<0>();
+        if (DG || issued - c_chunk - 2 <= 0) wait_vmcnt<0>();
         else wait_vmcnt_dyn((issued - c_chunk - 2) * PWc);
         workgroup_barrier();
         if (c_chunk + R - 1 < NCH) issue_chunk(c_chunk + R - 1, c_slot == 0 ? R - 1 : c_slot - 1);
@@ -187,14 +196,56 @@
     }                                                                                                                   \
     __builtin_amdgcn_sched_barrier(0);                                                                                  \
   }
+  int dg_q = 0, dg_end = DG ? (a.dg_taps & 15) * SPT : -1;
+  auto dg_flush = [&]() __attribute__((always_inline)) {
+    asm volatile("s_waitcnt lgkmcnt(0)" ::: "memory");
+    const int ph = (a.dg_phase >> (2 * dg_q + 1)) & 1, pw = (a.dg_phase >> (2 * dg_q)) & 1;
+    const int accumulate = p.accumulate;
+#pragma unroll
+    for (int i = 0; i < MT; ++i) {
+      const unsigned m = (unsigned)((wave * MT + i) * 16 + fr);
+      const unsigned pr = __umulhi(m, a.magic_w);
+      const unsigned pc = m - pr * (unsigned)W;
+      const int oy = 2 * (y0 + (int)pr) + ph, ox = 2 * (int)pc + pw;
+      const bool ok = pvalid[i] && oy < a.OHr && ox < p.OWr;
+      half_t* dst = p.out16 + (long long)b * p.out_bstride + ((long long)oy * p.OWr + ox) * p.out_ld + nblk * BN + fq * 4;
+#pragma unroll
+      for (int j = 0; j < NTW; ++j) {
+        if (ok && nblk * BN + j * 16 + fq * 4 < p.Cout) {
+          f4 v = acc[i][j];
+          if (accumulate) {
+            const h4 old = *reinterpret_cast<const h4*>(dst + j * 16);
+#pragma unroll
+            for (int r = 0; r < 4; ++r) v[r] += (float)old[r];
+          }
+          *reinterpret_cast<h4*>(dst + j * 16) = h4{(half_t)v[0], (half_t)v[1], (half_t)v[2], (half_t)v[3]};
+        }
+        acc[i][j] = f4{0.f, 0.f, 0.f, 0.f};
+      }
+    }
+    ++dg_q;
+    dg_end = ((a.dg_taps >> (4 * dg_q)) & 15) * SPT;
+  };
+#define CVX_TILE_DG_END(K)                       \
+  if constexpr (DG) {                            \
+    if (n + (K) + 1 == dg_end) dg_flush();       \
+  }
   clk_mark(p, 7);
   for (int n = 0; n < NSTEPS; n += 3) {
     CVX_TILE_BODY(0, false)
+    CVX_TILE_DG_END(0)
     CVX_TILE_BODY(1, false)
+    CVX_TILE_DG_END(1)
     CVX_TILE_BODY(2, true)
+    CVX_TILE_DG_END(2)
   }
 #undef CVX_TILE_BODY
+#undef CVX_TILE_DG_END
   clk_mark(p, 3);
+  if constexpr (DG) {
+    clk_mark(p, 4);
+    return;
+  }
 
   constexpr int RS = BN * 4 + 16;
   constexpr int CPR = BN / 8;
@@ -333,9 +384,9 @@
 template <int MT, int NTW>
 int launch_tile(const ConvParams& p, const TileArgs& a, int lds, hipStream_t stream) {
   static unsigned long long optin_mask = 0;
-  CVX_TRY(cvx_lds_optin((const void*)conv_tile_kernel<MT, NTW>, 160 * 1024, &optin_mask));
+  CVX_TRY(cvx_lds_optin((const void*)conv_tile_kernel<MT, NTW, CVX_TILE_KIND>, 160 * 1024, &optin_mask));
   const int blocks = ((a.ntiles + 7) / 8) * 8 * a.NB;
-  hipLaunchKernelGGL((conv_tile_kernel<MT, NTW>), dim3(blocks), dim3(64 * kTileWaves), lds, stream, p, a);
+  hipLaunchKernelGGL((conv_tile_kernel<MT, NTW, CVX_TILE_KIND>), dim3(blocks), dim3(64 * kTileWaves), lds, stream, p, a);
   return 0;
 }
 template <int MT>
diff --git a/computervision.pytorch_amd/csrc/conv_tile_s2_k1.hip b/computervision.pytorch_amd/csrc/conv_tile_s2_k1.hip
--- /dev/null
+++ b/computervision.pytorch_amd/csrc/conv_tile_s2_k1.hip
@@ -0,0 +1,5 @@
+#define CVX_TILE_MT_A 1
+#define CVX_TILE_MT_B 2
+#define CVX_TILE_KIND kTileS2
+#define CVX_TILE_LAUNCH_FN cvx_conv_tile_launch_s2_k1
+#include "conv_tile_kernel.inc.h"
diff --git a/computervision.pytorch_amd/csrc/conv_tile_s2_k2.hip b/computervision.pytorch_amd/csrc/conv_tile_s2_k2.hip
--- /dev/null
+++ b/computervision.pytorch_amd/csrc/conv_tile_s2_k2.hip
@@ -0,0 +1,5 @@
+#define CVX_TILE_MT_A 3
+#define CVX_TILE_MT_B 4
+#define CVX_TILE_KIND kTileS2
+#define CVX_TILE_LAUNCH_FN cvx_conv_tile_launch_s2_k2
+#include "conv_tile_kernel.inc.h"
diff --git a/computervision.pytorch_amd/csrc/engine.hip b/computervision.pytorch_amd/csrc/engine.hip
--- a/computervision.pytorch_amd/csrc/engine.hip
+++ b/computervision.pytorch_amd/csrc/engine.hip
@@ -84,6 +84,9 @@
   int gemm_fwd_bn = 0, gemm_fwd_kc = 0;
   const half_t* tile_fwd = nullptr;
   int tile_fwd_bn = 0;
+  bool tdg_on = false;
+  const half_t* tdg_pk = nullptr;
+  int tdg_bn = 0;
 };
 
 struct PoolRt {
@@ -270,6 +273,10 @@
 
 int act_kind(const cvx_op_desc& o) { return o.act == CVX_ACT_BN_SILU ? 0 : ((o.act == CVX_ACT_BN_LINEAR || o.act == CVX_ACT_BIAS_LINEAR) ? 2 : 1); }
 float dropout_p(const cvx_op_desc& o) { return (float)o.k / 65536.f; }
+bool tune_skip_s2(const cvx_op_desc& o) {
+  static const bool skip = cvx_tune_int("CVX_TUNE_SKIP_S2", 0) != 0;
+  return skip && o.type == CVX_OP_CONV && o.k == 3 && o.stride == 2 && o.in.c >= 32;
+}
 unsigned long long dropout_seed(const cvx_engine* e, int op) {
   return e->seed * 0x9E3779B97F4A7C15ULL + (unsigned long long)e->train_pass * 1000003ULL + (unsigned long long)op;
 }
@@ -378,6 +385,52 @@
   cp->out16 = gin.p;
   cp->out_ld = gin.ld;
   cp->out_bstride = gin.bstride;
+}
+
+bool fill_conv_tile_dg(const ConvGeom& g, int k, int pad, int dil, ViewDesc dy, ViewDesc gin, const half_t* wt_t, const half_t* zeros, int accumulate, ConvParams* cp) {
+  memset(cp, 0, sizeof(*cp));
+  if (k != 3 || g.stride != 2 || pad != 1 || dil != 1 || g.ntaps != 9 || g.ih < 2 || g.iw < 2) return false;
+  const std::vector<DgradPhase> phases = cvx_conv_dgrad_phases(k, g.stride, pad, dil, g.ih, g.iw);
+  std::vector<ConvTap> order;
+  for (size_t q = 0; q < phases.size(); ++q) {
+    order.insert(order.end(), phases[q].taps.begin(), phases[q].taps.end());
+    cp->tile_dg_taps |= (unsigned)order.size() << (4 * q);
+    cp->tile_dg_phase |= (unsigned)(phases[q].oph * 2 + phases[q].opw) << (2 * q);
+  }
+  if (phases.size() != 4) return false;
+  if (order.size() != 9) return false;
+  for (const ConvTap& t : order)
+    if (t.dh < 0 || t.dh > 1 || t.dw < 0 || t.dw > 1) return false;
+  unsigned long long pos = 0, wt = 0;
+  if (!cvx_halo_pack_taps(order.data(), 9, &pos, &wt)) return false;
+  cp->in = dy.p;
+  cp->in_bstride = dy.bstride;
+  cp->in_ld = dy.ld;
+  cp->IH = g.oh;
+  cp->IW = g.ow;
+  cp->Cin = g.cout;
+  cp->wt = wt_t;
+  cp->wt_ld = g.ntaps * g.cout;
+  cp->Cout = g.cin;
+  cp->B = g.B;
+  cp->OH2 = g.oh;
+  cp->OW2 = g.ow;
+  cp->IS = 1;
+  cp->OS = 2;
+  cp->OWr = g.iw;
+  cp->OHr = g.ih;
+  cp->ntaps = 9;
+  cp->zeros = zeros;
+  cp->halo_taps_ok = 1;
+  cp->halo_pos = pos;
+  cp->halo_wt = wt;
+  cp->epi = CVX_EPI_PLAIN;
+  cp->accumulate = accumulate;
+  cp->out16 = gin.p;
+  cp->out_ld = gin.ld;
+  cp->out_bstride = gin.bstride;
+  cp->tile_dg = 1;
+  return true;
 }
 
 void fill_wgrad(const ConvGeom& g, ViewDesc x, ViewDesc dy, const ConvTap* taps, int std3x3, float* slabs, int nsplit, WgradParams* wp) {
@@ -1005,6 +1058,20 @@
   cp->tile_packed = dc.tile_pk;
   cp->tile_packed_bn = dc.tile_bn;
 }
+bool fill_conv_tile_dg(const cvx_engine* e, int i, int B, ViewDesc dy, ConvParams* cp) {
+  const ConvRt& c = e->conv[i];
+  const cvx_op_desc& o = e->ops[i];
+  if (c.sh_dg < 0 || c.ndg != 4) return false;
+  if (!fill_conv_tile_dg(geom_of(o, B), o.k, o.pad, o.dil, dy, make_view(e, o.in, true), e->shadow + c.sh_dg, e->zero_page, c.in_accum, cp)) return false;
+  cp->tile_packed = c.tdg_pk;
+  cp->tile_packed_bn = c.tdg_bn;
+  return true;
+}
+bool tile_dg_wanted(const cvx_engine* e, int i, int B) {
+  const cvx_op_desc& o = e->ops[i];
+  ConvParams cp;
+  return o.type == CVX_OP_CONV && !e->conv[i].stem && o.needs_dgrad && fill_conv_tile_dg(e, i, B, dense_dy(o), &cp) && cvx_conv_tile_supported(cp);
+}
 void fill_conv_ps(const cvx_engine* e, int i, int B, ViewDesc dy, ConvParams* cp) {
   const ConvRt& c = e->conv[i];
   fill_conv_ps(geom_of(e->ops[i], B), dy, make_view(e, e->ops[i].in, true), e->shadow + c.sh_ps, c.ps_taps, e->zero_page, c.in_accum, cp);
@@ -1057,6 +1124,7 @@
       const cvx_op_desc& o = e->ops[i];
       ConvRt& c = e->conv[i];
       if (o.type != CVX_OP_CONV || c.stem || !o.needs_dgrad || c.sh_ps < 0 || c.ndg != 4) continue;
+      if (tile_dg_wanted(e, (int)i, B)) continue;
       ConvParams cp;
       fill_conv_ps(e, (int)i, B, dense_dy(e->ops[i]), &cp);
       if (!cvx_conv_gemm_supported(cp)) continue;
@@ -1102,6 +1170,9 @@
   for (auto& c : e->conv) {
     c.tile_fwd = nullptr;
     c.tile_fwd_bn = 0;
+    c.tdg_on = false;
+    c.tdg_pk = nullptr;
+    c.tdg_bn = 0;
     for (auto& d : c.dg) {
       d.tile_pk = nullptr;
       d.tile_bn = 0;
@@ -1109,6 +1180,7 @@
   }
 }
 
+constexpr int kTileDgRef = 1001;
 int plan_tile_packs(cvx_engine* e, int B, bool training) {
   free_tile_packs(e);
   struct Ref {
@@ -1143,6 +1215,12 @@
       fill_conv_dgrad(e, (int)i, 0, B, dense_dy(e->ops[i]), &cp);
       add(cp, (int)i, 0);
     }
+    for (size_t i = 0; i < e->ops.size(); ++i) {
+      if (!tile_dg_wanted(e, (int)i, B)) continue;
+      ConvParams cp;
+      fill_conv_tile_dg(e, (int)i, B, dense_dy(e->ops[i]), &cp);
+      add(cp, (int)i, kTileDgRef);
+    }
   }
   if (refs.empty()) return 0;
   CVX_HIP(hipMalloc((void**)&e->tile_arena, total));
@@ -1157,6 +1235,10 @@
     if (refs[k].q < 0) {
       c.tile_fwd = dst;
       c.tile_fwd_bn = refs[k].tp.BN;
+    } else if (refs[k].q == kTileDgRef) {
+      c.tdg_on = true;
+      c.tdg_pk = dst;
+      c.tdg_bn = refs[k].tp.BN;
     } else {
       c.dg[refs[k].q].tile_pk = dst;
       c.dg[refs[k].q].tile_bn = refs[k].tp.BN;
@@ -1698,7 +1780,7 @@
       }
       cp.stats = c.stat_fwd;
       cp.stats_replicas = cvx_stat_replicas(C);
-      {
+      if (!tune_skip_s2(o)) {
         ProfScope ps(e, PROF_CONV_FWD, conv_flops(o, B), conv_bytes(o, B) + (c.raw16 ? 0.0 : 2.0 * M * C), st);
         CVX_TRY(cvx_conv_igemm_launch(cp, st));
       }
@@ -1988,21 +2070,27 @@
     static const int wgrad_early = cvx_tune_int("CVX_WGRAD_EARLY", 1);
     const bool wgrad_first = !c.stem && (wgrad_early >= 2 || (wgrad_early == 1 && e->slab_tail_op >= 0 && i <= e->slab_tail_op));
     if (wgrad_first) CVX_TRY(queue_wgrad());
-    if (o.needs_dgrad) {
+    if (o.needs_dgrad && !tune_skip_s2(o)) {
       ViewDesc gin = make_view(e, o.in, true);
       static const bool merge_off = cvx_tune_set("CVX_NO_PHASE_MERGE");
       const bool merged = !merge_off && phases_mergeable(c.dg, c.ndg);
       bool empty_phase = false;
       for (int q = 0; q < c.ndg; ++q) empty_phase |= c.dg[q].ph.OH2 > 0 && c.dg[q].ph.OW2 > 0 && c.dg[q].ph.ntaps == 0;
       if (empty_phase && !c.in_accum) CVX_TRY(cvx_zero_slice(gin, B, o.ih * o.iw, o.in.c, st));
-      if (c.ps_on) {
+      if (c.tdg_on) {
+        ConvParams cp;
+        CVX_CHECK(fill_conv_tile_dg(e, i, B, dyv, &cp), "the four-phase data gradient was planned for an op it does not fit");
+        const double fl = 2.0 * B * o.oh * o.ow * (double)o.in.c * c.ntaps * C;
+        ProfScope ps(e, PROF_CONV_DGRAD, fl, conv_bytes(o, B) + (c.in_accum ? 2.0 * B * o.ih * o.iw * o.in.c : 0.0), st);
+        CVX_TRY(cvx_conv_igemm_launch(cp, st));
+      } else if (c.ps_on) {
         ConvParams cp;
         fill_conv_ps(e, i, B, dyv, &cp);
         const double fl = 2.0 * B * o.oh * o.ow * (double)o.in.c * c.ntaps * C;
         ProfScope ps(e, PROF_CONV_DGRAD, fl, conv_bytes(o, B) + (c.in_accum ? 2.0 * B * o.ih * o.iw * o.in.c : 0.0), st);
         CVX_TRY(cvx_conv_igemm_launch(cp, st));
       }
-      for (int q = 0; q < c.ndg && !c.ps_on; ++q) {
+      for (int q = 0; q < c.ndg && !c.ps_on && !c.tdg_on; ++q) {
         if (merged && q > 0) break;
         const DgClass& dc = c.dg[q];
         if (dc.ph.OH2 <= 0 || dc.ph.OW2 <= 0 || dc.ph.ntaps == 0) continue;
@@ -2302,6 +2390,8 @@
   const bool force_dma = (mode & 0x8000) != 0;
   const bool force_halo = (mode & 0x10000) != 0;
   const bool force_pw = (mode & 0x20000) != 0;
+  const bool raw_f16 = (mode & 0x40000) != 0;
+  const bool res_inplace = (mode & 0x80000) != 0;
   mode &= 0xff;
   const int oh = cvx_conv_out_size(ih, k, stride, pad, dil), ow = cvx_conv_out_size(iw, k, stride, pad, dil);
   const std::vector<ConvTap> taps = cvx_conv_fwd_taps(k, pad, dil);
@@ -2322,6 +2412,11 @@
     cp.scale = scale_or_bias;
     cp.shift = shift;
     cp.out16 = (half_t*)out;
+    if (res_inplace) {
+      cp.res = (const half_t*)out;
+      cp.res_ld = cp.out_ld;
+      cp.res_bstride = cp.out_bstride;
+    }
   } else if (mode == 2) {
     cp.epi = CVX_EPI_BIAS_F32;
     cp.bias = scale_or_bias;
@@ -2332,6 +2427,11 @@
     cp.out32 = (float*)out;
     cp.stats = (long long*)shift;
     cp.stats_replicas = cvx_stat_replicas(cout);
+    if (raw_f16) {
+      cp.raw16 = 1;
+      cp.out32 = nullptr;
+      cp.out16 = (half_t*)out;
+    }
   }
   int rc;
   cp.gemm_variant = gemm_variant;
@@ -2339,7 +2439,7 @@
     CVX_CHECK(cvx_conv_gemm_shape_ok(cp), "shape outside the GEMM-shaped kernel (cin % 8, cout % 4)");
     rc = cvx_conv_gemm_launch(cp, st);
   } else if (force_tile) {
-    CVX_CHECK(cvx_conv_tile_shape_ok(cp), "shape outside the row-band kernel (3x3 stride 1, cin % 8, cin >= 32)");
+    CVX_CHECK(cvx_conv_tile_shape_ok(cp), "shape outside the row-band kernel (3x3 pad 1, stride 1 or 2, cin % 8, cin >= 32, cout % 8)");
     cp.clk = g_cvx_clk;
     rc = cvx_conv_tile_launch(cp, st);
   } else if (force_dma) {
@@ -2362,6 +2462,26 @@
     cp.no_tile = no_tile ? 1 : 0;
     rc = cvx_conv_igemm_launch(cp, st);
   }
+  (void)hipStreamSynchronize(st);
+  return rc;
+}
+
+extern "C" int cvx_conv2d_dgrad_mode_nhwc(const void* dy_f16, int32_t batch, int32_t ih, int32_t iw, int32_t cin, const void* wt_f16, int32_t cout,
+                                          int32_t k, int32_t stride, int32_t pad, int32_t dil, int32_t mode, void* dx_f16, void* hip_stream) {
+  CVX_CHECK(dy_f16 && wt_f16 && dx_f16 && k * k <= CVX_MAX_TAPS && stride >= 1 && stride <= 4, "bad arguments");
+  CVX_CHECK(mode == 0x2000 || mode == 0x2001, "dgrad mode: 0x2000 (the row-band kernel's four-phase launch), | 1 to accumulate into dx");
+  hipStream_t st = (hipStream_t)hip_stream;
+  const int oh = cvx_conv_out_size(ih, k, stride, pad, dil), ow = cvx_conv_out_size(iw, k, stride, pad, dil);
+  DevTemps tmp;
+  const ConvTap* dt = nullptr;
+  const half_t* zeros = nullptr;
+  CVX_TRY(tmp.taps(cvx_conv_ps_window_taps(), &dt, &zeros));
+  ConvParams cp;
+  CVX_CHECK(fill_conv_tile_dg(ConvGeom{batch, ih, iw, cin, oh, ow, cout, stride, k * k}, k, pad, dil, dense_view(dy_f16, (long long)oh * ow, cout),
+                              dense_view(dx_f16, (long long)ih * iw, cin), (const half_t*)wt_f16, zeros, mode & 1, &cp) &&
+                cvx_conv_tile_shape_ok(cp),
+            "shape outside the row-band kernel's data gradient (3x3 / stride 2 / pad 1, cout % 8, cout >= 32, cin % 8)");
+  const int rc = cvx_conv_igemm_launch(cp, st);
   (void)hipStreamSynchronize(st);
   return rc;
 }
diff --git a/include/cvx_engine.h b/include/cvx_engine.h
--- a/include/cvx_engine.h
+++ b/include/cvx_engine.h
@@ -5,7 +5,7 @@
 extern "C" {
 #endif
 
-#define CVX_ABI_VERSION 5
+#define CVX_ABI_VERSION 6
 
 const char* cvx_last_error(void);
 int cvx_abi_version(void);
@@ -94,6 +94,8 @@
 int cvx_debug_clock_buffer(void* buf);
 
 int cvx_debug_conv_tile_plan(int32_t batch, int32_t h, int32_t w, int32_t cin, int32_t cout, int32_t* out8);
+int cvx_debug_conv_tile_s2_plan(int32_t batch, int32_t ih, int32_t iw, int32_t cin, int32_t cout, int32_t dgrad, int32_t* out12);
+int cvx_debug_conv_tile_rows(int32_t rows);
 int cvx_debug_conv_dma_plan(int64_t pixels, int32_t cin, int32_t cout, int32_t ntaps, int32_t* out4);
 int cvx_debug_conv_halo_plan(int32_t batch, int32_t h, int32_t w, int32_t cin, int32_t cout, int32_t* out4);
 int cvx_debug_conv_pw_plan(int64_t pixels, int32_t cin, int32_t cout, int32_t* out4);
@@ -187,6 +189,8 @@
                     void* hip_stream);
 int cvx_conv2d_dgrad_nhwc(const void* dy_f16, int32_t batch, int32_t ih, int32_t iw, int32_t cin, const void* wt_f16, int32_t cout,
                           int32_t k, int32_t stride, int32_t pad, int32_t dil, void* dx_f16, void* hip_stream);
+int cvx_conv2d_dgrad_mode_nhwc(const void* dy_f16, int32_t batch, int32_t ih, int32_t iw, int32_t cin, const void* wt_f16, int32_t cout,
+                               int32_t k, int32_t stride, int32_t pad, int32_t dil, int32_t mode, void* dx_f16, void* hip_stream);
 int64_t cvx_conv2d_wgrad_workspace_bytes(int32_t batch, int32_t oh, int32_t ow, int32_t cin, int32_t cout, int32_t k);
 int cvx_conv2d_wgrad_nhwc(const void* x_f16, const void* dy_f16, int32_t batch, int32_t ih, int32_t iw, int32_t cin, int32_t cout,
                           int32_t k, int32_t stride, int32_t pad, int32_t dil, float* dw, void* workspace, int64_t workspace_bytes,
```

Measured after the change: 5658 images/sec. About the same (-0.0%).
